# xingyizhou/CenterTrack

Measured on AMD Instinct MI355X. Metric: frames/sec (DLA-34 + DCNv2 CenterTrack hot path: H2D of the frame + forward + decode + D2H + track association), higher is better.
Workload: dtype f32; 1 GPU; mot17_512: mot heads, DLA-34, 512x512, 1 stream(s)/GPU, K=100, flip_test=False, seeded random-init weights; one step = 64 consecutive frames of every stream, each frame uploaded from pinned host memory inside the step (frame t+1 on a copy stream while frame t runs); global_batch=1, parallelism=streams sharded dp1, all-gather of packed detections, hip_graph=True

## Files before the change

### centertrack_amd/_lib.py

```python
import ctypes
import os

_PKG = os.path.dirname(os.path.abspath(__file__))
LIB_PATH = os.environ.get('CENTERTRACK_LIB') or os.path.join(_PKG, 'libcentertrack_hip.so')

c_float_p = ctypes.c_void_p
NUM_HEADS = 11
(HEAD_REG, HEAD_WH, HEAD_TRACKING, HEAD_LTRB, HEAD_LTRB_AMODAL, HEAD_DEP, HEAD_ROT, HEAD_DIM,
 HEAD_AMODEL_OFFSET, HEAD_NUSCENES_ATT, HEAD_VELOCITY) = range(NUM_HEADS)
HEAD_INDEX = {'reg': HEAD_REG, 'wh': HEAD_WH, 'tracking': HEAD_TRACKING, 'ltrb': HEAD_LTRB,
              'ltrb_amodal': HEAD_LTRB_AMODAL, 'dep': HEAD_DEP, 'rot': HEAD_ROT, 'dim': HEAD_DIM,
              'amodel_offset': HEAD_AMODEL_OFFSET, 'nuscenes_att': HEAD_NUSCENES_ATT,
              'velocity': HEAD_VELOCITY}
HEAD_CH = {'reg': 2, 'wh': 2, 'tracking': 2, 'ltrb': 4, 'ltrb_amodal': 4, 'dep': 1, 'rot': 8, 'dim': 3,
           'amodel_offset': 2, 'nuscenes_att': 8, 'velocity': 3}

CT_RELU = 1
CT_OUT_NCHW = 2
CT_DCN_MAIN, CT_DCN_FINISH, CT_DCN_OFFSETS = 1, 2, 4
CT_OK, CT_ERR_ARG, CT_ERR_LAUNCH, CT_ERR_WORKSPACE = 0, 1, 2, 3


class ConvDesc(ctypes.Structure):
    _fields_ = [('x', ctypes.c_void_p), ('N', ctypes.c_int), ('H', ctypes.c_int), ('W', ctypes.c_int),
                ('Cin', ctypes.c_int), ('ldx', ctypes.c_int),
                ('w_packed', ctypes.c_void_p), ('Cout', ctypes.c_int), ('ks', ctypes.c_int),
                ('stride', ctypes.c_int),
                ('scale', ctypes.c_void_p), ('shift', ctypes.c_void_p),
                ('res', ctypes.c_void_p), ('ldr', ctypes.c_int),
                ('y', ctypes.c_void_p), ('ldy', ctypes.c_int),
                ('flags', ctypes.c_int),
                ('sig_lo', ctypes.c_int), ('sig_hi', ctypes.c_int),
                ('dep_lo', ctypes.c_int), ('dep_hi', ctypes.c_int), ('depth_scale', ctypes.c_float),
                ('workspace', ctypes.c_void_p), ('workspace_bytes', ctypes.c_size_t),
                ('split_k', ctypes.c_int), ('algo', ctypes.c_int), ('w_winograd', ctypes.c_void_p),
                ('pool_y', ctypes.c_void_p), ('pool_ld', ctypes.c_int),
                ('proj_w_packed', ctypes.c_void_p), ('proj_scale', ctypes.c_void_p), ('proj_shift', ctypes.c_void_p),
                ('proj_y', ctypes.c_void_p), ('proj_ldy', ctypes.c_int)]


class DcnDesc(ctypes.Structure):
    _fields_ = [('x', ctypes.c_void_p), ('N', ctypes.c_int), ('H', ctypes.c_int), ('W', ctypes.c_int),
                ('Cin', ctypes.c_int), ('ldx', ctypes.c_int),
                ('om', ctypes.c_void_p), ('ldom', ctypes.c_int),
                ('w_packed', ctypes.c_void_p), ('Cout', ctypes.c_int),
                ('scale', ctypes.c_void_p), ('shift', ctypes.c_void_p),
                ('y', ctypes.c_void_p), ('ldy', ctypes.c_int),
                ('flags', ctypes.c_int),
                ('workspace', ctypes.c_void_p), ('workspace_bytes', ctypes.c_size_t),
                ('split_k', ctypes.c_int), ('algo', ctypes.c_int), ('fuse_offset', ctypes.c_int),
                ('w_off_packed', ctypes.c_void_p), ('b_off', ctypes.c_void_p),
                ('up_w', ctypes.c_void_p), ('up_f', ctypes.c_int), ('up_skip', ctypes.c_void_p), ('up_lds', ctypes.c_int),
                ('up_y', ctypes.c_void_p), ('up_ldy', ctypes.c_int),
                ('om_partial', ctypes.c_void_p), ('om_partial_bytes', ctypes.c_size_t),
                ('w_off_winograd', ctypes.c_void_p)]


CT_DCN_BWD_INPUT, CT_DCN_BWD_OFFSET_MASK, CT_DCN_BWD_WEIGHT = 1, 2, 4


class DcnBwdDesc(ctypes.Structure):
    _fields_ = [('x', ctypes.c_void_p), ('N', ctypes.c_int), ('H', ctypes.c_int), ('W', ctypes.c_int),
                ('Cin', ctypes.c_int), ('ldx', ctypes.c_int),
                ('om', ctypes.c_void_p), ('ldom', ctypes.c_int),
                ('gy', ctypes.c_void_p), ('Cout', ctypes.c_int), ('ldgy', ctypes.c_int),
                ('wT_packed', ctypes.c_void_p),
                ('gx', ctypes.c_void_p), ('ldgx', ctypes.c_int),
                ('gom', ctypes.c_void_p), ('ldgom', ctypes.c_int),
                ('gw', ctypes.c_void_p), ('gb', ctypes.c_void_p),
                ('workspace', ctypes.c_void_p), ('workspace_bytes', ctypes.c_size_t),
                ('flags', ctypes.c_int)]


CT_MAX_FUSED_HEADS = 8


class HeadsDesc(ctypes.Structure):
    _fields_ = [('x', ctypes.c_void_p), ('N', ctypes.c_int), ('H', ctypes.c_int), ('W', ctypes.c_int),
                ('Cin', ctypes.c_int), ('ldx', ctypes.c_int),
                ('w0_winograd', ctypes.c_void_p), ('b0', ctypes.c_void_p), ('nheads', ctypes.c_int),
                ('w2', ctypes.c_void_p), ('b2', ctypes.c_void_p),
                ('cout', ctypes.c_int * CT_MAX_FUSED_HEADS), ('coff', ctypes.c_int * CT_MAX_FUSED_HEADS),
                ('out', ctypes.c_void_p), ('ctot', ctypes.c_int),
                ('sig_lo', ctypes.c_int), ('sig_hi', ctypes.c_int), ('dep_lo', ctypes.c_int), ('dep_hi', ctypes.c_int),
                ('depth_scale', ctypes.c_float)]


class SparseHeadsDesc(ctypes.Structure):
    _fields_ = [('feat', ctypes.c_void_p), ('ldf', ctypes.c_int), ('nheads', ctypes.c_int),
                ('head', ctypes.c_int * NUM_HEADS),
                ('w1', ctypes.c_void_p * NUM_HEADS), ('b1', ctypes.c_void_p * NUM_HEADS),
                ('w2', ctypes.c_void_p * NUM_HEADS), ('b2', ctypes.c_void_p * NUM_HEADS),
                ('depth_scale', ctypes.c_float), ('zero_tracking', ctypes.c_int),
                ('flip_B', ctypes.c_int), ('flip_mode', ctypes.c_int * NUM_HEADS)]


class DecodeDesc(ctypes.Structure):
    _fields_ = [('hm', ctypes.c_void_p), ('B', ctypes.c_int), ('C', ctypes.c_int), ('h', ctypes.c_int),
                ('w', ctypes.c_int), ('K', ctypes.c_int),
                ('heads', ctypes.c_void_p * NUM_HEADS),
                ('out', ctypes.c_void_p), ('inds', ctypes.c_void_p),
                ('workspace', ctypes.c_void_p), ('workspace_bytes', ctypes.c_size_t),
                ('hm_batch_stride', ctypes.c_size_t), ('head_batch_stride', ctypes.c_size_t * NUM_HEADS),
                ('out_stride', ctypes.c_int),
                ('host_out', ctypes.c_void_p), ('done_flag', ctypes.c_void_p), ('done_counter', ctypes.c_void_p),
                ('sparse', ctypes.POINTER(SparseHeadsDesc))]


class PoseDesc(ctypes.Structure):
    _fields_ = [('rows', ctypes.c_void_p), ('row_floats', ctypes.c_int), ('box_col', ctypes.c_int),
                ('inds', ctypes.c_void_p),
                ('B', ctypes.c_int), ('h', ctypes.c_int), ('w', ctypes.c_int), ('K', ctypes.c_int),
                ('num_joints', ctypes.c_int),
                ('hps', ctypes.c_void_p), ('hm_hp', ctypes.c_void_p), ('hp_offset', ctypes.c_void_p),
                ('hps_batch_stride', ctypes.c_size_t), ('hm_hp_batch_stride', ctypes.c_size_t),
                ('hp_offset_batch_stride', ctypes.c_size_t),
                ('out', ctypes.c_void_p), ('out_stride', ctypes.c_int),
                ('workspace', ctypes.c_void_p), ('workspace_bytes', ctypes.c_size_t),
                ('box_wh', ctypes.c_void_p), ('box_reg', ctypes.c_void_p), ('box_ltrb', ctypes.c_void_p),
                ('box_wh_batch_stride', ctypes.c_size_t), ('box_reg_batch_stride', ctypes.c_size_t),
                ('box_ltrb_batch_stride', ctypes.c_size_t)]


class FlipHead(ctypes.Structure):
    _fields_ = [('src', ctypes.c_void_p), ('dst', ctypes.c_void_p), ('src_batch_stride', ctypes.c_size_t),
                ('C', ctypes.c_int), ('mode', ctypes.c_int)]


CT_FLIP_AVG, CT_FLIP_NEG_EVEN, CT_FLIP_JOINTS, CT_FLIP_JOINT_OFFSETS = range(4)


class RowLayout(ctypes.Structure):
    _fields_ = [(n, ctypes.c_int) for n in ('score', 'cls', 'cts', 'tracking', 'bbox', 'amodel_offset')]


class Track(ctypes.Structure):
    _fields_ = [('score', ctypes.c_float), ('cls', ctypes.c_int), ('ct', ctypes.c_float * 2),
                ('tracking', ctypes.c_float * 2), ('bbox', ctypes.c_float * 4),
                ('tracking_id', ctypes.c_int), ('age', ctypes.c_int), ('active', ctypes.c_int),
                ('row', ctypes.c_int)]


class PrestageDesc(ctypes.Structure):
    _fields_ = [('enabled', ctypes.c_int), ('N', ctypes.c_int), ('H', ctypes.c_int), ('W', ctypes.c_int),
                ('w_x', ctypes.c_void_p), ('w_img', ctypes.c_void_p), ('scale3', ctypes.c_void_p), ('shift3', ctypes.c_void_p),
                ('partial', ctypes.c_void_p * 3), ('ldp', ctypes.c_int), ('flip_B', ctypes.c_int)]


class FrameLoopDesc(ctypes.Structure):
    _fields_ = [('B', ctypes.c_int), ('K', ctypes.c_int), ('F', ctypes.c_int),
                ('trackers', ctypes.POINTER(ctypes.c_void_p)),
                ('layout', RowLayout),
                ('out_thresh', ctypes.c_float), ('pre_thresh', ctypes.c_float),
                ('inp_w', ctypes.c_int), ('inp_h', ctypes.c_int),
                ('host_rows', ctypes.c_void_p), ('rows_keep', ctypes.c_void_p),
                ('blob_params', ctypes.c_void_p), ('blob_counts', ctypes.c_void_p), ('blob_cap', ctypes.c_int),
                ('nslots', ctypes.c_int),
                ('graphs', ctypes.c_void_p * 3), ('frames', ctypes.c_void_p * 3),
                ('frame_bytes', ctypes.c_size_t),
                ('stream', ctypes.c_void_p),
                ('results', ctypes.c_void_p), ('results_cap', ctypes.c_int), ('done_flag', ctypes.c_void_p),
                ('pre', PrestageDesc)]


class FrameStepArgs(ctypes.Structure):
    _fields_ = [('slot', ctypes.c_int), ('frame_kind', ctypes.c_int),
                ('frame', ctypes.c_void_p), ('next_frame', ctypes.c_void_p),
                ('trans_input', ctypes.c_void_p), ('trans_inv', ctypes.c_void_p)]


CT_FRAME_DEVICE, CT_FRAME_HOST, CT_FRAME_IN_PLACE, CT_FRAME_UPLOADED = range(4)


ABI_VERSION = 103

EXPORTS = ['ct_last_error', 'ct_version', 'ct_set_tuning', 'ct_packed_weight_elems', 'ct_pack_conv_weight',
           'ct_packed_winograd_elems', 'ct_pack_winograd_weight', 'ct_conv2d',
           'ct_conv2d_workspace_bytes', 'ct_heads_fused', 'ct_dcn_v2', 'ct_dcn_v2_workspace_bytes', 'ct_dcn_v2_offsets_bytes', 'ct_dcn_v2_group', 'ct_dcn_v2_group_workspace_bytes', 'ct_dcn_v2_group_plan',
           'ct_dcn_v2_backward', 'ct_dcn_v2_backward_workspace_bytes', 'ct_packed_dcn_weight_t_elems', 'ct_pack_dcn_weight_t', 'ct_stem_forward',
           'ct_maxpool2x2', 'ct_upsample_add', 'ct_nchw_to_nhwc', 'ct_nhwc_to_nchw',
           'ct_decode_row_floats', 'ct_decode_workspace_bytes', 'ct_decode', 'ct_decode_pose_workspace_bytes',
           'ct_decode_pose', 'ct_render_pre_hm',
           'ct_tracker_create', 'ct_tracker_destroy', 'ct_tracker_reset', 'ct_tracker_num_tracks',
           'ct_tracker_id_count', 'ct_tracker_get_tracks', 'ct_tracker_step', 'ct_tracker_prehm_params', 'ct_linear_assignment', 'ct_tracker_set_mode', 'ct_tracker_init_tracks',
           'ct_tracker_step_public', 'ct_tracker_step_dets', 'ct_transform_points',
           'ct_preprocess_image', 'ct_preprocess_lut', 'ct_preprocess_device', 'ct_graph_begin', 'ct_graph_end', 'ct_graph_launch', 'ct_graph_destroy',
           'ct_memcpy_async', 'ct_memset_async', 'ct_stream_synchronize', 'ct_flip_merge', 'ct_flip_images',
           'ct_frame_loop_create', 'ct_frame_loop_destroy', 'ct_frame_loop_submit', 'ct_frame_loop_wait', 'ct_frame_loop_finish',
           'ct_frame_loop_finish_submit', 'ct_frame_loop_upload', 'ct_frame_loop_pending_slot', 'ct_frame_loop_in_flight',
           'ct_frame_loop_forget_upload', 'ct_frame_loop_prestage', 'ct_stem_forward_parts', 'ct_signal_host']

_lib = None


class CTError(RuntimeError):
    pass


def load():
    global _lib
    if _lib is not None:
        return _lib
    if not os.path.exists(LIB_PATH):
        raise CTError('%s not found: build it with `python -c "import __graft_entry__ as g; g.build()"` '
                      '(hipcc --offload-arch=gfx950); there is no CPU fallback' % LIB_PATH)
    import torch
    lib = ctypes.CDLL(LIB_PATH)
    i, p, sz = ctypes.c_int, ctypes.c_void_p, ctypes.c_size_t
    lib.ct_last_error.restype = ctypes.c_char_p
    lib.ct_version.restype = i
    if lib.ct_version() != ABI_VERSION:
        raise CTError('%s is ABI version %d, this binding was written against %d: rebuild it (python -m '
                      'centertrack_amd.build)' % (LIB_PATH, lib.ct_version(), ABI_VERSION))
    lib.ct_set_tuning.argtypes = [ctypes.c_char_p, i]
    lib.ct_packed_weight_elems.restype = sz
    lib.ct_packed_weight_elems.argtypes = [i, i, i]
    lib.ct_pack_conv_weight.argtypes = [p, p, i, i, i, p]
    lib.ct_packed_winograd_elems.restype = sz
    lib.ct_packed_winograd_elems.argtypes = [i, i]
    lib.ct_pack_winograd_weight.argtypes = [p, p, i, i, p]
    lib.ct_conv2d.argtypes = [ctypes.POINTER(ConvDesc), p]
    lib.ct_conv2d_workspace_bytes.restype = sz
    lib.ct_conv2d_workspace_bytes.argtypes = [ctypes.POINTER(ConvDesc)]
    lib.ct_heads_fused.argtypes = [ctypes.POINTER(HeadsDesc), p]
    lib.ct_dcn_v2.argtypes = [ctypes.POINTER(DcnDesc), p]
    lib.ct_dcn_v2_workspace_bytes.restype = sz
    lib.ct_dcn_v2_workspace_bytes.argtypes = [ctypes.POINTER(DcnDesc)]
    lib.ct_dcn_v2_offsets_bytes.restype = sz
    lib.ct_dcn_v2_offsets_bytes.argtypes = [ctypes.POINTER(DcnDesc)]
    lib.ct_dcn_v2_group.argtypes = [ctypes.POINTER(DcnDesc), i, i, p]
    lib.ct_dcn_v2_group_workspace_bytes.restype = sz
    lib.ct_dcn_v2_group_workspace_bytes.argtypes = [ctypes.POINTER(DcnDesc)]
    lib.ct_dcn_v2_group_plan.argtypes = [ctypes.POINTER(DcnDesc), ctypes.POINTER(ctypes.c_size_t), ctypes.POINTER(ctypes.c_int)]
    lib.ct_dcn_v2_backward.argtypes = [ctypes.POINTER(DcnBwdDesc), p]
    lib.ct_dcn_v2_backward_workspace_bytes.restype = sz
    lib.ct_dcn_v2_backward_workspace_bytes.argtypes = [ctypes.POINTER(DcnBwdDesc)]
    lib.ct_packed_dcn_weight_t_elems.restype = sz
    lib.ct_packed_dcn_weight_t_elems.argtypes = [i, i]
    lib.ct_pack_dcn_weight_t.argtypes = [p, p, i, i, p]
    lib.ct_stem_forward.argtypes = [p, p, p, i, i, i, p, p, p, p, p, p, i, p]
    lib.ct_stem_forward_parts.argtypes = [p, p, p, p, i, i, i, i, p, p, p, p, p, p, i, p]
    lib.ct_maxpool2x2.argtypes = [p, i, i, i, i, i, p, i, p]
    lib.ct_upsample_add.argtypes = [p, i, i, i, i, i, p, i, p, i, p, i, p]
    lib.ct_nchw_to_nhwc.argtypes = [p, i, i, i, i, p, i, p]
    lib.ct_nhwc_to_nchw.argtypes = [p, i, i, i, i, i, p, p]
    lib.ct_decode_row_floats.argtypes = [ctypes.POINTER(DecodeDesc)]
    lib.ct_decode_workspace_bytes.restype = sz
    lib.ct_decode_workspace_bytes.argtypes = [ctypes.POINTER(DecodeDesc)]
    lib.ct_decode.argtypes = [ctypes.POINTER(DecodeDesc), p]
    lib.ct_decode_pose_workspace_bytes.restype = sz
    lib.ct_decode_pose_workspace_bytes.argtypes = [ctypes.POINTER(PoseDesc)]
    lib.ct_decode_pose.argtypes = [ctypes.POINTER(PoseDesc), p]
    lib.ct_render_pre_hm.argtypes = [p, p, i, i, i, i, p, i, p]
    lib.ct_tracker_create.restype = p
    lib.ct_tracker_create.argtypes = [ctypes.c_float, i]
    lib.ct_tracker_destroy.restype = None
    lib.ct_tracker_destroy.argtypes = [p]
    lib.ct_tracker_reset.restype = None
    lib.ct_tracker_reset.argtypes = [p]
    lib.ct_tracker_num_tracks.argtypes = [p]
    lib.ct_tracker_id_count.argtypes = [p]
    lib.ct_tracker_get_tracks.argtypes = [p, p, i]
    lib.ct_tracker_step.argtypes = [p, p, i, i, ctypes.POINTER(RowLayout), ctypes.c_float, p, p, i]
    lib.ct_tracker_prehm_params.argtypes = [p, ctypes.c_float, p, i, i, p, i]
    lib.ct_linear_assignment.argtypes = [p, i, i, p, p]
    lib.ct_tracker_set_mode.argtypes = [p, i, i]
    lib.ct_tracker_init_tracks.argtypes = [p, p, i]
    lib.ct_tracker_step_public.argtypes = [p, p, i, i, ctypes.POINTER(RowLayout), ctypes.c_float, p, p, i, p, i]
    lib.ct_tracker_step_dets.argtypes = [p, p, i, p, i, p, i]
    lib.ct_transform_points.argtypes = [p, p, i, p]
    lib.ct_preprocess_image.argtypes = [p, i, i, i, i, p, i, i, p, p, p, i]
    lib.ct_preprocess_lut.argtypes = [p, p, i, p]
    lib.ct_preprocess_device.argtypes = [p, i, i, i, i, p, i, i, p, p, p, p]
    lib.ct_graph_begin.argtypes = [p]
    lib.ct_graph_end.restype = p
    lib.ct_graph_end.argtypes = [p]
    lib.ct_graph_launch.argtypes = [p, p]
    lib.ct_graph_destroy.restype = None
    lib.ct_graph_destroy.argtypes = [p]
    lib.ct_memcpy_async.argtypes = [p, p, sz, i, p]
    lib.ct_stream_synchronize.argtypes = [p]
    lib.ct_memset_async.argtypes = [p, i, sz, p]
    lib.ct_signal_host.argtypes = [p, i, p]
    lib.ct_flip_merge.argtypes = [ctypes.POINTER(FlipHead), i, p, i, i, i, i, p]
    lib.ct_flip_images.argtypes = [p, p, sz, i, p]
    lib.ct_frame_loop_create.restype = p
    lib.ct_frame_loop_create.argtypes = [ctypes.POINTER(FrameLoopDesc)]
    lib.ct_frame_loop_destroy.restype = None
    lib.ct_frame_loop_destroy.argtypes = [p]
    lib.ct_frame_loop_submit.argtypes = [p, ctypes.POINTER(FrameStepArgs)]
    lib.ct_frame_loop_wait.argtypes = [p]
    lib.ct_frame_loop_finish.argtypes = [p, ctypes.POINTER(FrameStepArgs), p]
    lib.ct_frame_loop_finish_submit.argtypes = [p, ctypes.POINTER(FrameStepArgs), p, ctypes.POINTER(FrameStepArgs)]
    lib.ct_frame_loop_upload.argtypes = [p, i, p]
    lib.ct_frame_loop_pending_slot.argtypes = [p]
    lib.ct_frame_loop_prestage.argtypes = [p, i]
    lib.ct_frame_loop_in_flight.argtypes = [p]
    lib.ct_frame_loop_forget_upload.restype = None
    lib.ct_frame_loop_forget_upload.argtypes = [p]
    for kv in filter(None, os.environ.get('CENTERTRACK_TUNE', '').split(',')):
        k, _, v = kv.partition('=')
        if lib.ct_set_tuning(k.strip().encode(), int(v)) != 0:
            raise CTError('CENTERTRACK_TUNE: %s' % lib.ct_last_error().decode())
    _lib = lib
    return lib


def check(rc, what=''):
    if rc != 0:
        raise CTError('%s failed (code %d): %s' % (what or 'libcentertrack_hip call', rc,
                                                  load().ct_last_error().decode()))


def stream_ptr():
    import torch
    return ctypes.c_void_p(torch.cuda.current_stream().cuda_stream)


import contextlib as _contextlib


@_contextlib.contextmanager
def capture_guard(collect=True):
    import gc
    if os.environ.get('CT_NO_CAPTURE_GUARD') == '1':
        yield
        return
    if collect:
        gc.collect()
    was = gc.isenabled()
    gc.disable()
    try:
        yield
    finally:
        if was:
            gc.enable()
```

### centertrack_amd/build.py

```python
import os
import subprocess
import sys

PKG = os.path.dirname(os.path.abspath(__file__))
ROOT = os.path.dirname(PKG)
CSRC = os.path.join(PKG, 'csrc')
LIB = os.path.join(PKG, 'libcentertrack_hip.so')
SOURCES = ['api.cpp', 'runtime.hip', 'conv_mfma.hip', 'wino_mfma.hip', 'dcn_mfma.hip', 'dcn_bwd.hip', 'stem.hip', 'elementwise.hip', 'decode.hip', 'pose.hip', 'host_track.cpp', 'host_preprocess.cpp', 'preprocess.hip', 'flip.hip', 'frame_loop.hip']
FLAGS = ['--offload-arch=gfx950', '-O3', '-std=c++17', '-fPIC', '-I' + os.path.join(ROOT, 'include'), '-I' + CSRC,
         '-Wno-unused-result']


def _stale(target, deps):
    if not os.path.exists(target):
        return True
    t = os.path.getmtime(target)
    return any(os.path.getmtime(d) > t for d in deps)


def build(force=False, verbose=False):
    hipcc = os.environ.get('HIPCC', '/opt/rocm/bin/hipcc')
    objdir = os.path.join(PKG, 'build')
    os.makedirs(objdir, exist_ok=True)
    headers = [os.path.join(CSRC, 'ct_common.h'), os.path.join(CSRC, 'ksplit_core.h'),
               os.path.join(ROOT, 'include', 'centertrack_hip.h')]
    objs = []
    procs = []
    for src in SOURCES:
        sp = os.path.join(CSRC, src)
        if not os.path.exists(sp):
            continue
        obj = os.path.join(objdir, src.rsplit('.', 1)[0] + '.o')
        objs.append(obj)
        if force or _stale(obj, [sp] + headers):
            extra = ['-x', 'hip'] if src.endswith('.hip') else ['-ffp-contract=off']
            cmd = [hipcc] + FLAGS + extra + ['-c', sp, '-o', obj]
            if verbose:
                print(' '.join(cmd))
            procs.append((src, subprocess.Popen(cmd)))
    for src, p in procs:
        if p.wait() != 0:
            raise RuntimeError('hipcc failed on %s' % src)
    if force or _stale(LIB, objs):
        cmd = [hipcc, '--offload-arch=gfx950', '-shared', '-fPIC', '-pthread', '-o', LIB] + objs
        if verbose:
            print(' '.join(cmd))
        subprocess.check_call(cmd)
    return LIB


if __name__ == '__main__':
    print(build(force='--force' in sys.argv, verbose=True))
```

### centertrack_amd/csrc/decode.hip

```cpp
#include "ct_common.h"

namespace {
CT_DEFINE_STAMPS(decode)

constexpr int SEG_MAX = 1024;
constexpr int MAXK = 512;

__device__ __forceinline__ unsigned f2ord(float f)
{
    const unsigned u = __float_as_uint(f);
    return (u & 0x80000000u) ? ~u : (u | 0x80000000u);
}
__device__ __forceinline__ float ord2f(unsigned o)
{
    return __uint_as_float((o & 0x80000000u) ? (o & 0x7fffffffu) : ~o);
}

__device__ __forceinline__ void hist_add(unsigned *hist, unsigned digit, bool active)
{
    unsigned long long todo = __ballot(active);
    const int lane = threadIdx.x & 63;
#pragma unroll 1
    for (int it = 0; it < 4 && todo; ++it) {
        const int leader = __ffsll((long long)todo) - 1;
        const unsigned d0 = __shfl(digit, leader);
        const unsigned long long same = __ballot(active && digit == d0) & todo;
        if (lane == leader) atomicAdd(&hist[d0], (unsigned)__popcll(same));
        todo &= ~same;
    }
    if (active && ((todo >> lane) & 1ull)) atomicAdd(&hist[digit], 1u);
}

template <typename Get>
__device__ unsigned long long radix_select_kth(Get get, int n, int K, unsigned *hist ,
                                               unsigned long long *bcast )
{
    __shared__ int scan_tmp[256];
    __shared__ int wsum[4];
    unsigned long long prefix = 0ull;
    int need = K;
    for (int d = 7; d >= 0; --d) {
        for (int i = threadIdx.x; i < 256; i += blockDim.x) hist[i] = 0u;
        __syncthreads();
        const int sh = d * 8;
        const unsigned long long himask = (d == 7) ? 0ull : (~0ull << (sh + 8));
        const int nround = (n + blockDim.x - 1) / blockDim.x * blockDim.x;
        for (int i = threadIdx.x; i < nround; i += blockDim.x) {
            const unsigned long long k = (i < n) ? get(i) : 0ull;
            hist_add(hist, (unsigned)(k >> sh) & 255u, k != 0ull && (k & himask) == prefix);
        }
        __syncthreads();
        if (threadIdx.x < 256) {
            const int b = threadIdx.x, ln = b & 63;
            const int c = (int)hist[b];
            int suf = c;
#pragma unroll
            for (int o = 1; o < 64; o <<= 1) {
                const int t = __shfl_down(suf, o);
                if (ln + o < 64) suf += t;
            }
            if (ln == 0) wsum[b >> 6] = suf;
            scan_tmp[b] = suf;
        }
        __syncthreads();
        if (threadIdx.x < 256) {
            const int b = threadIdx.x;
            int hi = 0;
            for (int wv = (b >> 6) + 1; wv < 4; ++wv) hi += wsum[wv];
            const int incl = scan_tmp[b] + hi;
            const int above = incl - (int)hist[b];
            if (above < need && incl >= need) {
                bcast[0] = (unsigned long long)b;
                bcast[1] = (incl - above == need - above) ? ~0ull : (unsigned long long)(need - above);
            }
        }
        __syncthreads();
        prefix |= bcast[0] << sh;
        const unsigned long long nd = bcast[1];
        __syncthreads();
        if (nd == ~0ull) break;
        need = (int)nd;
    }
    return prefix;
}

struct Stage1Args {
    const float *hm;
    unsigned long long *cand;
    int B, C, h, w, K, nseg, seg;
    size_t hm_bs;
};

__global__ __launch_bounds__(256) void decode_stage1_kernel(Stage1Args a)
{
    extern __shared__ __attribute__((aligned(16))) unsigned char smem[];
    unsigned long long *keys = reinterpret_cast<unsigned long long *>(smem);
    float *rows = reinterpret_cast<float *>(smem + SEG_MAX * sizeof(unsigned long long));
    __shared__ int npos;

    int bid = blockIdx.x;
    const int seg = bid % a.nseg; bid /= a.nseg;
    const int c = bid % a.C;
    const int b = bid / a.C;
    const int HW = a.h * a.w;
    const int p_lo = seg * a.seg;
    const int p_hi = min(HW, p_lo + a.seg);
    const int nloc = p_hi - p_lo;
    const float *map = a.hm + (size_t)b * a.hm_bs + (size_t)c * HW;

    const int y_lo = p_lo / a.w, y_hi = (p_hi - 1) / a.w;
    const int r_lo = max(0, y_lo - 1), r_hi = min(a.h - 1, y_hi + 1);
    const int nstage = (r_hi - r_lo + 1) * a.w;
    for (int i = threadIdx.x; i < nstage; i += 256) rows[i] = map[r_lo * a.w + i];
    if (threadIdx.x == 0) npos = 0;
    __syncthreads();

    const int lane = threadIdx.x & 63;
    const int nround = (nloc + 255) / 256 * 256;
    for (int i = threadIdx.x; i < nround; i += 256) {
        bool pos = false;
        unsigned long long key = 0ull;
        if (i < nloc) {
            const int p = p_lo + i;
            const int y = p / a.w, x = p - y * a.w;
            const float v = rows[(y - r_lo) * a.w + x];
            float m = v;
#pragma unroll
            for (int dy = -1; dy <= 1; ++dy) {
                const int yy = y + dy;
                if (yy < 0 || yy >= a.h) continue;
#pragma unroll
                for (int dx = -1; dx <= 1; ++dx) {
                    const int xx = x + dx;
                    if (xx < 0 || xx >= a.w) continue;
                    m = fmaxf(m, rows[(yy - r_lo) * a.w + xx]);
                }
            }
            const float s = (m == v) ? v : v * 0.0f;
            pos = s > 0.0f;
            key = ((unsigned long long)f2ord(s) << 32) | (unsigned long long)(0xFFFFFFFFu - (unsigned)p);
        }
        const unsigned long long mask = __ballot(pos);
        int base = 0;
        if (lane == 0 && mask) base = atomicAdd(&npos, (int)__popcll(mask));
        base = __shfl(base, 0);
        if (pos) keys[base + (int)__popcll(mask & ((1ull << lane) - 1ull))] = key;
    }
    __syncthreads();

    const int n = npos;
    unsigned long long *out = a.cand + (size_t)blockIdx.x * a.K;
    if (n <= a.K) {
        for (int i = threadIdx.x; i < a.K; i += 256) out[i] = (i < n) ? keys[i] : 0ull;
    } else {
        for (int i = threadIdx.x; i < n; i += 256) {
            const unsigned long long k = keys[i];
            int r = 0;
            for (int j = 0; j < n; ++j) r += (keys[j] > k) ? 1 : 0;
            if (r < a.K) out[r] = k;
        }
    }
}

struct Stage2Args {
    const unsigned long long *cand;
    const float *hm;
    const float *heads[CT_NUM_HEADS];
    int head_ch[CT_NUM_HEADS];
    size_t head_bs[CT_NUM_HEADS];
    size_t hm_bs;
    float *out;
    long long *inds;
    int B, C, h, w, K, nseg, F;
    int M2;
    int keys_final;
    float *host_out;
    int *done_flag;
    unsigned *done_counter;
    unsigned long long *winners;
    unsigned present;
};

template <typename HV>
__device__ __forceinline__ void emit_row(float *row, float *hrow, unsigned present, float score, int cls, float xs0,
                                         float ys0, HV hv)
{
    constexpr int HCH[CT_NUM_HEADS] = {2, 2, 2, 4, 4, 1, 8, 3, 2, 8, 3};
    auto has = [&](int hd) { return (present >> hd) & 1u; };
    int f = 0;
    auto put = [&](float v) { row[f] = v; if (hrow) hrow[f] = v; ++f; };
    put(score); put((float)cls); put(xs0); put(ys0);
    float xs = xs0 + 0.5f, ys = ys0 + 0.5f;
    if (has(CT_HEAD_REG)) { xs = xs0 + hv(CT_HEAD_REG, 0); ys = ys0 + hv(CT_HEAD_REG, 1); }
    const bool has_box = has(CT_HEAD_WH) || has(CT_HEAD_LTRB) || has(CT_HEAD_LTRB_AMODAL);
    float bb[4] = {0.f, 0.f, 0.f, 0.f};
    if (has(CT_HEAD_WH)) {
        float ww = hv(CT_HEAD_WH, 0), hh = hv(CT_HEAD_WH, 1);
        if (ww < 0.f) ww = 0.f;
        if (hh < 0.f) hh = 0.f;
        bb[0] = xs - ww / 2; bb[1] = ys - hh / 2; bb[2] = xs + ww / 2; bb[3] = ys + hh / 2;
    }
    if (has(CT_HEAD_LTRB)) {
        bb[0] = xs0 + hv(CT_HEAD_LTRB, 0); bb[1] = ys0 + hv(CT_HEAD_LTRB, 1);
        bb[2] = xs0 + hv(CT_HEAD_LTRB, 2); bb[3] = ys0 + hv(CT_HEAD_LTRB, 3);
    }
    float am[4] = {0.f, 0.f, 0.f, 0.f};
    if (has(CT_HEAD_LTRB_AMODAL)) {
        am[0] = xs0 + hv(CT_HEAD_LTRB_AMODAL, 0); am[1] = ys0 + hv(CT_HEAD_LTRB_AMODAL, 1);
        am[2] = xs0 + hv(CT_HEAD_LTRB_AMODAL, 2); am[3] = ys0 + hv(CT_HEAD_LTRB_AMODAL, 3);
        for (int i = 0; i < 4; ++i) bb[i] = am[i];
    }
    if (has_box) for (int i = 0; i < 4; ++i) put(bb[i]);
    if (has(CT_HEAD_LTRB_AMODAL)) for (int i = 0; i < 4; ++i) put(am[i]);
    const int rest[7] = {CT_HEAD_TRACKING, CT_HEAD_DEP, CT_HEAD_ROT, CT_HEAD_DIM, CT_HEAD_AMODEL_OFFSET,
                         CT_HEAD_NUSCENES_ATT, CT_HEAD_VELOCITY};
#pragma unroll
    for (int q = 0; q < 7; ++q) {
        const int hd = rest[q];
        if (!has(hd)) continue;
#pragma unroll
        for (int ch = 0; ch < HCH[hd]; ++ch) put(hv(hd, ch));
    }
}

__device__ __forceinline__ void raise_done_flag(int *done_flag, unsigned *done_counter, int nwg)
{
    __threadfence_system();
    __syncthreads();
    if (threadIdx.x == 0 && nwg == 1) {
        __hip_atomic_store(done_flag, 1, __ATOMIC_RELEASE, __HIP_MEMORY_SCOPE_SYSTEM);
    } else if (threadIdx.x == 0) {
        const unsigned prev = __hip_atomic_fetch_add(done_counter, 1u, __ATOMIC_ACQ_REL, __HIP_MEMORY_SCOPE_SYSTEM);
        if (prev == (unsigned)nwg - 1u) {
            *done_counter = 0u;
            __hip_atomic_store(done_flag, 1, __ATOMIC_RELEASE, __HIP_MEMORY_SCOPE_SYSTEM);
        }
    }
}

__device__ __forceinline__ unsigned long long key_from_map(const float *hm_b, int C, int h, int w, unsigned f)
{
    const int HW = h * w;
    const int cls = (int)(f / (unsigned)HW);
    const int p = (int)(f - (unsigned)cls * (unsigned)HW);
    const int y = p / w, x = p - y * w;
    const float *map = hm_b + (size_t)cls * HW;
    const float v = map[p];
    float m = v;
    for (int dy = -1; dy <= 1; ++dy) {
        const int yy = y + dy;
        if (yy < 0 || yy >= h) continue;
        for (int dx = -1; dx <= 1; ++dx) {
            const int xx = x + dx;
            if (xx < 0 || xx >= w) continue;
            m = fmaxf(m, map[yy * w + xx]);
        }
    }
    const float s = (m == v) ? v : v * 0.0f;
    return ((unsigned long long)f2ord(s) << 32) | (unsigned long long)(0xFFFFFFFFu - f);
}

template <typename F>
__device__ __forceinline__ void scan_cands(const unsigned long long *cand, int M2, int tid, int NT, F f)
{
    constexpr int U = 8;
    for (int i0 = tid; i0 - tid < M2; i0 += NT * U) {
        unsigned long long raw[U];
#pragma unroll
        for (int u = 0; u < U; ++u) {
            const int i = i0 + u * NT;
            raw[u] = (i < M2) ? cand[i] : 0ull;
        }
#pragma unroll
        for (int u = 0; u < U; ++u) f(i0 + u * NT, raw[u]);
    }
}

constexpr int FCAP = 4096;
constexpr int SLICE = 8192;

__device__ __forceinline__ void bitonic_desc(unsigned long long *v, int n, int tid, int NT)
{
    for (int size = 2; size <= n; size <<= 1) {
        for (int stride = size >> 1; stride > 0; stride >>= 1) {
            for (int i = tid; i < (n >> 1); i += NT) {
                const int lo = 2 * i - (i & (stride - 1));
                const int hi = lo + stride;
                const bool desc = ((lo & size) == 0);
                const unsigned long long x = v[lo], y = v[hi];
                if ((x < y) == desc) { v[lo] = y; v[hi] = x; }
            }
            __syncthreads();
        }
    }
}


constexpr int SEL_U = 8;
constexpr int SEL_BINS = 1024;
constexpr int TIECAP = 1024;

struct SelShared {
    unsigned hist[SEL_BINS];
    int wsum[16];
    unsigned long long tie[TIECAP];
    int bstar, need, total, nwin, ntie;
};

__device__ __forceinline__ int sel_bin(unsigned long long k)
{
    const float sc = ord2f((unsigned)(k >> 32));
    const int b = (int)(sc * (float)SEL_BINS);
    return b < 0 ? 0 : (b > SEL_BINS - 1 ? SEL_BINS - 1 : b);
}

__device__ __forceinline__ int select_topk_regs(const unsigned long long (&keys)[SEL_U], int K, SelShared &sh,
                                                unsigned long long *win, bool keep_all)
{
    const int tid = threadIdx.x, lane = tid & 63, wave = tid >> 6;
    sh.hist[tid] = 0u;
    if (tid == 0) { sh.bstar = -1; sh.need = 0; sh.total = 0; sh.nwin = 0; sh.ntie = 0; }
    __syncthreads();
    int bins[SEL_U];
#pragma unroll
    for (int u = 0; u < SEL_U; ++u) {
        bins[u] = sel_bin(keys[u]);
        if (keys[u] != 0ull) atomicAdd(&sh.hist[bins[u]], 1u);
    }
    __syncthreads();
    const int c = (int)sh.hist[tid];
    int suf = c;
#pragma unroll
    for (int o = 1; o < 64; o <<= 1) {
        const int t = __shfl_down(suf, o);
        if (lane + o < 64) suf += t;
    }
    if (lane == 0) sh.wsum[wave] = suf;
    __syncthreads();
    int hi = 0;
    for (int w = wave + 1; w < 16; ++w) hi += sh.wsum[w];
    const int incl = suf + hi, above = incl - c;
    if (tid == 0) sh.total = incl;
    if (above < K && incl >= K) { sh.bstar = tid; sh.need = K - above; }
    __syncthreads();
    const int total = sh.total;
    if (total < K) {
        if (keep_all) {
#pragma unroll
            for (int u = 0; u < SEL_U; ++u) {
                const bool hit = keys[u] != 0ull;
                const unsigned long long mask = __ballot(hit);
                int base = 0;
                if (mask) {
                    const int leader = __ffsll((long long)mask) - 1;
                    if (lane == leader) base = atomicAdd(&sh.nwin, (int)__popcll(mask));
                    base = __shfl(base, leader);
                }
                if (hit) win[base + (int)__popcll(mask & ((1ull << lane) - 1ull))] = keys[u];
            }
            __syncthreads();
        }
        return -1;
    }
    const int bstar = sh.bstar, need = sh.need;
    unsigned hitm = 0u, tiem = 0u;
#pragma unroll
    for (int u = 0; u < SEL_U; ++u) {
        const bool live = keys[u] != 0ull;
        hitm |= (live && bins[u] > bstar) ? (1u << u) : 0u;
        tiem |= (live && bins[u] == bstar) ? (1u << u) : 0u;
    }
    const int packed = __popc(hitm) | (__popc(tiem) << 16);
    int pre = packed;
#pragma unroll
    for (int o = 1; o < 64; o <<= 1) {
        const int t = __shfl_up(pre, o);
        if (lane >= o) pre += t;
    }
    const int tot = __shfl(pre, 63);
    int bh = 0, bt = 0;
    if (lane == 63) {
        if (tot & 0xffff) bh = atomicAdd(&sh.nwin, tot & 0xffff);
        if (tot >> 16) bt = atomicAdd(&sh.ntie, tot >> 16);
    }
    int sw = __shfl(bh, 63) + ((pre - packed) & 0xffff);
    int st = __shfl(bt, 63) + ((pre - packed) >> 16);
#pragma unroll
    for (int u = 0; u < SEL_U; ++u) {
        if ((hitm >> u) & 1u) win[sw++] = keys[u];
        if ((tiem >> u) & 1u) {
            if (st < TIECAP) sh.tie[st] = keys[u];
            ++st;
        }
    }
    __syncthreads();
    const int m = sh.ntie;
    if (m > TIECAP) return -2;
    const int first = K - need;
    for (int i = tid; i < m; i += 1024) {
        const unsigned long long k = sh.tie[i];
        int r = 0;
        for (int j = 0; j < m; ++j) r += (sh.tie[j] > k) ? 1 : 0;
        if (r < need) win[first + r] = k;
    }
    __syncthreads();
    return K;
}

struct Stage2aArgs {
    const unsigned long long *cand;
    unsigned long long *cand2;
    int M2, G, K, per_class, HW;
};

__global__ __launch_bounds__(1024) void decode_stage2a_kernel(Stage2aArgs a)
{
    __shared__ SelShared sh;
    __shared__ unsigned long long win[MAXK];
    __shared__ unsigned rhist[256];
    __shared__ unsigned long long rbcast[2];
    __shared__ int rslot;
    const int b = blockIdx.x / a.G, g = blockIdx.x - b * a.G;
    const int tid = threadIdx.x, NT = blockDim.x;
    const int lo = g * SLICE, n = min(SLICE, a.M2 - lo);
    const unsigned long long *cand = a.cand + (size_t)b * a.M2 + lo;
    unsigned long long keys[SEL_U];
#pragma unroll
    for (int u = 0; u < SEL_U; ++u) {
        const int i = tid + u * NT;
        unsigned long long k = (i < n) ? cand[i] : 0ull;
        if (k != 0ull) {
            const unsigned cls = (unsigned)((lo + i) / a.per_class);
            const unsigned p = 0xFFFFFFFFu - (unsigned)(k & 0xFFFFFFFFull);
            k = (k & 0xFFFFFFFF00000000ull) | (unsigned long long)(0xFFFFFFFFu - (cls * (unsigned)a.HW + p));
        }
        keys[u] = k;
    }
    for (int i = tid; i < a.K; i += NT) win[i] = 0ull;
    __syncthreads();
    unsigned long long *out = a.cand2 + ((size_t)b * a.G + g) * a.K;
    const int rc = select_topk_regs(keys, a.K, sh, win, true);
    if (rc != -2) {
        for (int i = tid; i < a.K; i += NT) out[i] = win[i];
        return;
    }
    auto get = [&](int i) -> unsigned long long {
        unsigned long long k = cand[i];
        if (k != 0ull) {
            const unsigned cls = (unsigned)((lo + i) / a.per_class);
            const unsigned p = 0xFFFFFFFFu - (unsigned)(k & 0xFFFFFFFFull);
            k = (k & 0xFFFFFFFF00000000ull) | (unsigned long long)(0xFFFFFFFFu - (cls * (unsigned)a.HW + p));
        }
        return k;
    };
    if (tid == 0) rslot = 0;
    __syncthreads();
    const unsigned long long T = radix_select_kth(get, n, a.K, rhist, rbcast);
#pragma unroll
    for (int u = 0; u < SEL_U; ++u)
        if (keys[u] >= T && keys[u] != 0ull) {
            const int sl = atomicAdd(&rslot, 1);
            if (sl < a.K) out[sl] = keys[u];
        }
}

__global__ __launch_bounds__(1024) void decode_stage2_kernel(Stage2Args a)
{
    __shared__ unsigned hist[256];
    __shared__ unsigned long long bcast[2];
    __shared__ unsigned long long win[MAXK];
    __shared__ unsigned long long lmax[1024];
    __shared__ unsigned long long filt[FCAP];
    __shared__ SelShared sel;
    __shared__ unsigned long long Lsh;
    __shared__ int slot, total, nf;
    const int b = blockIdx.x;
    const int tid = threadIdx.x, NT = blockDim.x, lane = tid & 63;
    const int HW = a.h * a.w;
    const int M2 = a.M2;
    CT_STAMP_RT(0);
    CT_STAMP(1);
    const unsigned long long *cand = a.cand + (size_t)b * M2;
    const int per_class = a.nseg * a.K;

    auto key2 = [&](int i, unsigned long long k) -> unsigned long long {
        if (k == 0ull || a.keys_final) return k;
        const unsigned cls = (unsigned)(i / per_class);
        const unsigned p = 0xFFFFFFFFu - (unsigned)(k & 0xFFFFFFFFull);
        return (k & 0xFFFFFFFF00000000ull) | (unsigned long long)(0xFFFFFFFFu - (cls * (unsigned)HW + p));
    };
    auto get = [&](int i) -> unsigned long long { return key2(i, cand[i]); };
    const bool in_regs = M2 <= SEL_U * 1024 && NT == 1024;
    unsigned long long keys[SEL_U];
    if (in_regs) {
#pragma unroll
        for (int u = 0; u < SEL_U; ++u) {
            const int i = tid + u * NT;
            keys[u] = (i < M2) ? cand[i] : 0ull;
        }
    }
    int KP = 1;
    while (KP < a.K) KP <<= 1;
    for (int i = tid; i < KP; i += NT) win[i] = 0ull;
    if (tid == 0) { slot = 0; total = 0; nf = 0; Lsh = 1ull; }
    __syncthreads();
    bool need_sort = true;
    bool selected = false;
    if (in_regs) {
#pragma unroll
        for (int u = 0; u < SEL_U; ++u) keys[u] = key2(tid + u * NT, keys[u]);
        CT_STAMP(2);
        const int rc = select_topk_regs(keys, a.K, sel, filt, false);
        CT_STAMP(3);
        if (rc == a.K) {
            for (int i0 = 0; i0 < a.K; i0 += NT / 8) {
                const int i = i0 + (tid >> 3), part = tid & 7;
                const unsigned long long k = (i < a.K) ? filt[i] : 0ull;
                int r = 0;
                for (int j = part; j < a.K; j += 8) r += (filt[j] > k) ? 1 : 0;
                r += __shfl_xor(r, 1);
                r += __shfl_xor(r, 2);
                r += __shfl_xor(r, 4);
                if (i < a.K && part == 0) win[r] = k;
            }
            need_sort = false;
            selected = true;
        } else if (rc == -1) {
            if (tid == 0) total = sel.total;
            selected = true;
        }
        __syncthreads();
    }
    if (!selected) {
    scan_cands(cand, M2, tid, NT, [&](int i, unsigned long long raw) {
        const unsigned long long k = key2(i, raw);
        const bool hit = k != 0ull;
        const unsigned long long mask = __ballot(hit);
        int base = 0;
        if (mask) {
            const int leader = __ffsll((long long)mask) - 1;
            if (lane == leader) base = atomicAdd(&total, (int)__popcll(mask));
            base = __shfl(base, leader);
        }
        if (hit) {
            const int sl = base + (int)__popcll(mask & ((1ull << lane) - 1ull));
            if (sl < FCAP) filt[sl] = k;
        }
    });
    __syncthreads();
    }
    if (selected && need_sort == false) {
    } else if (!selected && total >= a.K && total <= FCAP) {
        int NP = KP;
        while (NP < total) NP <<= 1;
        for (int i = total + tid; i < NP; i += NT) filt[i] = 0ull;
        __syncthreads();
        bitonic_desc(filt, NP, tid, NT);
        for (int i = tid; i < a.K; i += NT) win[i] = filt[i];
        need_sort = false;
    } else if (!selected && total >= a.K) {
        {
            unsigned long long mx = 0ull;
            scan_cands(cand, M2, tid, NT, [&](int i, unsigned long long raw) {
                const unsigned long long k = key2(i, raw);
                mx = (k > mx) ? k : mx;
            });
            lmax[tid] = mx;
        }
        __syncthreads();
        if (tid < 256) {
            const int G = NT < 256 ? NT : 256;
            const unsigned long long my = lmax[tid];
            int r = 0;
            for (int j = 0; j < G; ++j) r += (lmax[j] > my) ? 1 : 0;
            if (my != 0ull && r == a.K - 1) Lsh = my;
        }
        __syncthreads();
        const unsigned long long L = Lsh;
        scan_cands(cand, M2, tid, NT, [&](int i, unsigned long long raw) {
            const unsigned long long k = key2(i, raw);
            const bool hit = k >= L && k != 0ull;
            const unsigned long long mask = __ballot(hit);
            int base = 0;
            if (mask) {
                const int leader = __ffsll((long long)mask) - 1;
                if (lane == leader) base = atomicAdd(&nf, (int)__popcll(mask));
                base = __shfl(base, leader);
            }
            if (hit) {
                const int sl = base + (int)__popcll(mask & ((1ull << lane) - 1ull));
                if (sl < FCAP) filt[sl] = k;
            }
        });
        __syncthreads();
        const int n = nf;
        if (n <= FCAP) {
            for (int i = tid; i < n; i += NT) {
                const unsigned long long k = filt[i];
                int r = 0;
                for (int j = 0; j < n; ++j) r += (filt[j] > k) ? 1 : 0;
                if (r < a.K) win[r] = k;
            }
            need_sort = false;
        } else {
            const unsigned long long T = radix_select_kth(get, M2, a.K, hist, bcast);
            for (int i = tid; i < M2; i += NT) {
                const unsigned long long k = get(i);
                if (k >= T && k != 0ull) {
                    const int s = atomicAdd(&slot, 1);
                    if (s < a.K) win[s] = k;
                }
            }
        }
    } else {
        const float *hm_b = a.hm + (size_t)b * a.hm_bs;
        const int NALL = a.C * HW;
        auto getall = [&](int i) -> unsigned long long { return key_from_map(hm_b, a.C, a.h, a.w, (unsigned)i); };
        const unsigned long long T = radix_select_kth(getall, NALL, a.K, hist, bcast);
        for (int i = tid; i < NALL; i += NT) {
            const unsigned long long k = getall(i);
            if (k >= T) {
                const int s = atomicAdd(&slot, 1);
                if (s < a.K) win[s] = k;
            }
        }
    }
    __syncthreads();
    CT_STAMP(4);
    if (need_sort) bitonic_desc(win, KP, tid, NT);
    if (a.winners) {
        for (int r = threadIdx.x; r < a.K; r += blockDim.x) {
            const unsigned long long k = win[r];
            a.winners[(size_t)b * a.K + r] = k;
            if (a.inds) a.inds[(size_t)b * a.K + r] = (int)((0xFFFFFFFFu - (unsigned)(k & 0xFFFFFFFFull)) % (unsigned)HW);
        }
        CT_STAMP(5);
        CT_STAMP(6);
        CT_STAMP(7);
        CT_STAMP_RT(8);
        return;
    }
    for (int r = threadIdx.x; r < a.K; r += blockDim.x) {
        const unsigned long long k = win[r];
        const float score = ord2f((unsigned)(k >> 32));
        const unsigned flat = 0xFFFFFFFFu - (unsigned)(k & 0xFFFFFFFFull);
        const int cls = (int)(flat / (unsigned)HW);
        const int p = (int)(flat - (unsigned)cls * (unsigned)HW);
        const float ys0 = (float)(p / a.w), xs0 = (float)(p % a.w);
        float *row = a.out + ((size_t)b * a.K + r) * a.F;
        float *hrow = a.host_out ? a.host_out + ((size_t)b * a.K + r) * a.F : nullptr;
        if (a.inds) a.inds[(size_t)b * a.K + r] = p;
        constexpr int HCH[CT_NUM_HEADS] = {2, 2, 2, 4, 4, 1, 8, 3, 2, 8, 3};
        float hval[CT_NUM_HEADS][8];
#pragma unroll
        for (int hd = 0; hd < CT_NUM_HEADS; ++hd) {
            const float *hp = a.heads[hd];
            const bool on = hp != nullptr;
            const float *base = on ? hp + (size_t)b * a.head_bs[hd] + p : a.hm;
#pragma unroll
            for (int ch = 0; ch < HCH[hd]; ++ch) hval[hd][ch] = base[on ? (size_t)ch * HW : 0];
        }
        emit_row(row, hrow, a.present, score, cls, xs0, ys0, [&](int hd, int ch) { return hval[hd][ch]; });
    }
    CT_STAMP(5);
    if (a.done_flag) {
        raise_done_flag(a.done_flag, a.done_counter, a.B);
        CT_STAMP(6);
    }
    CT_STAMP(7);
    CT_STAMP_RT(8);
}

constexpr int SP_HID = 256;

struct SparseArgs {
    const float *feat; int ldf; size_t feat_bs;
    int nheads;
    int head[CT_NUM_HEADS];
    const float *w1[CT_NUM_HEADS], *b1[CT_NUM_HEADS], *w2[CT_NUM_HEADS], *b2[CT_NUM_HEADS];
    float depth_scale;
    int zero_tracking;
    int flip_B;
    int flip_mode[CT_NUM_HEADS];
    const unsigned long long *winners;
    float *partial;
    float *out, *host_out;
    int *done_flag; unsigned *done_counter;
    int B, h, w, K, F, tiles;
    unsigned present;
};

__global__ __launch_bounds__(256) __attribute__((amdgpu_waves_per_eu(2, 2))) void sparse_heads_kernel(SparseArgs a)
{
    __shared__ __attribute__((aligned(16))) float A[36 * 256];
    __shared__ __attribute__((aligned(16))) float Hd[16 * 68];
    __shared__ int wy[16], wx[16];
    constexpr int HCH[CT_NUM_HEADS] = {2, 2, 2, 4, 4, 1, 8, 3, 2, 8, 3};
    const int tid = threadIdx.x, lane = tid & 63;
    const int wave = __builtin_amdgcn_readfirstlane(tid >> 6);
    int bid = blockIdx.x;
    const int quarter = bid & 3; bid >>= 2;
    const int hi = bid % a.nheads; bid /= a.nheads;
    const int tile = bid;
    const int b = tile / a.tiles, t = tile - b * a.tiles;
    const int HW = a.h * a.w;
    const int hd = a.head[hi];
    const int cout = HCH[hd];
    const float *wp = a.w1[hi] + ((size_t)(quarter * 4 + wave) << 8) + (lane << 2);
    f32x4 bq[36];
#pragma unroll
    for (int st = 0; st < 36; ++st) bq[st] = *reinterpret_cast<const f32x4 *>(wp + (size_t)st * (16 << 8));
    const int li = lane & 15, lg = lane >> 4;
    const float bias1 = a.b1[hi][quarter * 64 + wave * 16 + li];
    if (tid < 16) {
        const int r = t * 16 + tid;
        int y = -4, x = -4;
        if (r < a.K) {
            const unsigned long long k = a.winners[(size_t)b * a.K + r];
            const unsigned flat = 0xFFFFFFFFu - (unsigned)(k & 0xFFFFFFFFull);
            const int p = (int)(flat % (unsigned)HW);
            y = p / a.w; x = p - y * a.w;
        }
        wy[tid] = y; wx[tid] = x;
    }
    __syncthreads();
    const int npass = (a.flip_B > 0 && a.flip_mode[hi] != 0) ? 2 : 1;
    for (int pass = 0; pass < npass; ++pass) {
    {
        const float *fb = a.feat + (size_t)(pass ? a.flip_B + b : b) * a.feat_bs;
        f32x4 pv[9];
#pragma unroll
        for (int j = 0; j < 9; ++j) {
            const int it = tid + 256 * j;
            const int m = it / 144, rem = it - m * 144;
            const int tap = rem >> 4, q = rem & 15;
            const int cx = pass ? a.w - 1 - wx[m] : wx[m];
            const int y = wy[m] + tap / 3 - 1, x = cx + tap % 3 - 1;
            const bool ok = y >= 0 && y < a.h && x >= 0 && x < a.w && wy[m] >= 0;
            const f32x4 v = *reinterpret_cast<const f32x4 *>(fb + (ok ? ((size_t)y * a.w + x) * a.ldf + q * 4 : 0));
            pv[j] = ok ? v : f32x4{0.f, 0.f, 0.f, 0.f};
        }
        if (pass) __syncthreads();
#pragma unroll
        for (int j = 0; j < 9; ++j) {
            const int it = tid + 256 * j;
            const int m = it / 144, rem = it - m * 144;
            const int tap = rem >> 4, q = rem & 15;
            *reinterpret_cast<f32x4 *>(A + (tap * 4 + (q >> 2)) * 256 + m * 16 + (((q & 3) ^ ((m >> 1) & 2)) << 2)) = pv[j];
        }
    }
    __syncthreads();
    {
        const int aoff = li * 16 + ((lg ^ ((li >> 1) & 2)) << 2);
        f32x4 acc = f32x4{0.f, 0.f, 0.f, 0.f};
#pragma unroll
        for (int st = 0; st < 36; ++st) {
            const f32x4 af = *reinterpret_cast<const f32x4 *>(A + st * 256 + aoff);
#pragma unroll
            for (int e = 0; e < 4; ++e) acc = __builtin_amdgcn_mfma_f32_16x16x4f32(af[e], bq[st][e], acc, 0, 0, 0);
        }
#pragma unroll
        for (int e = 0; e < 4; ++e) Hd[(lg * 4 + e) * 68 + wave * 16 + li] = fmaxf(acc[e] + bias1, 0.0f);
    }
    __syncthreads();
    {
        const int pair = tid >> 1, part = tid & 1;
        const int m = pair >> 3, c = pair & 7;
        float sum = 0.f;
        if (c < cout) {
            const float *w2 = a.w2[hi] + c * SP_HID + quarter * 64 + part * 32;
            const float *hh = Hd + m * 68 + part * 32;
#pragma unroll
            for (int j = 0; j < 32; ++j) sum += hh[j] * w2[j];
        }
        sum += __shfl_xor(sum, 1);
        if (part == 0) a.partial[(((((size_t)tile * a.nheads + hi) * 2 + pass) * 4 + quarter) * 16 + m) * 8 + c] = sum;
    }
    }
}

__global__ __launch_bounds__(128) void sparse_rows_kernel(SparseArgs a)
{
    constexpr int HCH[CT_NUM_HEADS] = {2, 2, 2, 4, 4, 1, 8, 3, 2, 8, 3};
    const int b = blockIdx.x;
    const int HW = a.h * a.w;
    for (int r = threadIdx.x; r < a.K; r += blockDim.x) {
        const unsigned long long k = a.winners[(size_t)b * a.K + r];
        const unsigned flat = 0xFFFFFFFFu - (unsigned)(k & 0xFFFFFFFFull);
        const int cls = (int)(flat / (unsigned)HW);
        const int p = (int)(flat - (unsigned)cls * (unsigned)HW);
        const int y = p / a.w, x = p - y * a.w;
        const float score = ord2f((unsigned)(k >> 32));
        const int tile = b * a.tiles + (r >> 4), m = r & 15;
        float V[CT_NUM_HEADS][8];
#pragma unroll
        for (int hd = 0; hd < CT_NUM_HEADS; ++hd)
#pragma unroll
            for (int c = 0; c < 8; ++c) V[hd][c] = 0.f;
        for (int h2 = 0; h2 < a.nheads; ++h2) {
            const int hd2 = a.head[h2];
            const bool both = a.flip_B > 0 && a.flip_mode[h2] != 0;
#pragma unroll
            for (int c = 0; c < 8; ++c) {
                if (c >= HCH[hd2]) continue;
                auto value = [&](int pass) {
                    const float *pp = a.partial + ((((size_t)tile * a.nheads + h2) * 2 + pass) * 4 * 16 + m) * 8 + c;
                    float v = pp[0];
                    v += pp[128];
                    v += pp[256];
                    v += pp[384];
                    v += a.b2[h2][c];
                    if (hd2 == CT_HEAD_DEP) v = (1.0f / (1.0f / (1.0f + expf(-v)) + 1e-6f) - 1.0f) * a.depth_scale;
                    return v;
                };
                float v = value(0);
                if (both) {
                    const float v1 = value(1);
                    v = (v + ((a.flip_mode[h2] == 2 && !(c & 1)) ? -v1 : v1)) / 2;
                }
                if (hd2 == CT_HEAD_TRACKING && a.zero_tracking) v = 0.0f;
#pragma unroll
                for (int hd = 0; hd < CT_NUM_HEADS; ++hd)
                    if (hd == hd2) V[hd][c] = v;
            }
        }
        float *row = a.out + ((size_t)b * a.K + r) * a.F;
        float *hrow = a.host_out ? a.host_out + ((size_t)b * a.K + r) * a.F : nullptr;
        emit_row(row, hrow, a.present, score, cls, (float)x, (float)y, [&](int hd3, int ch) { return V[hd3][ch]; });
    }
    if (a.done_flag) raise_done_flag(a.done_flag, a.done_counter, a.B);
}

const int kHeadCh[CT_NUM_HEADS] = {2, 2, 2, 4, 4, 1, 8, 3, 2, 8, 3};

int check(const ct_decode_desc *d, const char *who)
{
    if (!d || !d->hm) CT_FAIL_ARG("%s: null heat-map", who);
    if (d->B <= 0 || d->C <= 0 || d->h <= 0 || d->w <= 0) CT_FAIL_ARG("%s: bad shape", who);
    if (d->K <= 0 || d->K > MAXK) CT_FAIL_ARG("%s: K=%d out of range (1..%d)", who, d->K, MAXK);
    if ((long)d->h * d->w < d->K) CT_FAIL_ARG("%s: h*w=%ld < K=%d (torch.topk would raise too)", who, (long)d->h * d->w, d->K);
    if ((double)d->C * d->h * d->w >= 4294967295.0) CT_FAIL_ARG("%s: C*h*w too large", who);
    if (const ct_sparse_heads_desc *sp = d->sparse) {
        if (sp->nheads < 1 || sp->nheads > CT_NUM_HEADS || !sp->feat || sp->ldf < 64 || (sp->ldf & 3) || ((uintptr_t)sp->feat & 15))
            CT_FAIL_ARG("%s: sparse heads need 1..%d heads and a 16-byte aligned NHWC feature view of >= 64 channels", who, CT_NUM_HEADS);
        for (int i = 0; i < sp->nheads; ++i) {
            if (sp->head[i] < 0 || sp->head[i] >= CT_NUM_HEADS || !sp->w1[i] || !sp->b1[i] || !sp->w2[i] || !sp->b2[i])
                CT_FAIL_ARG("%s: sparse head %d is incomplete", who, i);
            if (d->heads[sp->head[i]]) CT_FAIL_ARG("%s: head %d is both dense and sparse", who, sp->head[i]);
        }
        if (sp->flip_B < 0 || (sp->flip_B > 0 && sp->flip_B != d->B)) CT_FAIL_ARG("%s: sparse flip_B must be 0 or B (feat then holds 2 * B images)", who);
    }
    return CT_OK;
}

}

static unsigned present_mask(const ct_decode_desc *d)
{
    unsigned m = 0;
    for (int i = 0; i < CT_NUM_HEADS; ++i)
        if (d->heads[i]) m |= 1u << i;
    if (d->sparse)
        for (int i = 0; i < d->sparse->nheads && i < CT_NUM_HEADS; ++i)
            if (d->sparse->head[i] >= 0 && d->sparse->head[i] < CT_NUM_HEADS) m |= 1u << d->sparse->head[i];
    return m;
}

extern "C" int ct_decode_row_floats(const ct_decode_desc *d)
{
    if (!d) return 0;
    if (d->sparse && (d->sparse->nheads < 1 || d->sparse->nheads > CT_NUM_HEADS)) {
        ct_set_error("ct_decode_row_floats: sparse nheads=%d out of range (1..%d)", d->sparse->nheads, CT_NUM_HEADS);
        return 0;
    }
    const unsigned m = present_mask(d);
    auto has = [&](int hd) { return (m >> hd) & 1u; };
    int f = 4;
    if (has(CT_HEAD_WH) || has(CT_HEAD_LTRB) || has(CT_HEAD_LTRB_AMODAL)) f += 4;
    if (has(CT_HEAD_LTRB_AMODAL)) f += 4;
    const int rest[7] = {CT_HEAD_TRACKING, CT_HEAD_DEP, CT_HEAD_ROT, CT_HEAD_DIM, CT_HEAD_AMODEL_OFFSET,
                         CT_HEAD_NUSCENES_ATT, CT_HEAD_VELOCITY};
    for (int q = 0; q < 7; ++q)
        if (has(rest[q])) f += kHeadCh[rest[q]];
    return f;
}

static int pick_seg(const ct_decode_desc *d)
{
    const long HW = (long)d->h * d->w;
    int seg = SEG_MAX;
    while (seg > 256 && (long)d->B * d->C * ((HW + seg - 1) / seg) < 256) seg >>= 1;
    return seg;
}

static int pick_groups(const ct_decode_desc *d, int seg, int nseg)
{
    const long M2 = (long)d->C * nseg * d->K;
    (void)seg;
    if (M2 <= SLICE) return 0;
    const long G = (M2 + SLICE - 1) / SLICE;
    return (int)G;
}

static size_t sparse_bytes(const ct_decode_desc *d)
{
    if (!d->sparse) return 0;
    const size_t tiles = (size_t)d->B * ct_cdiv(d->K, 16);
    return (size_t)d->B * d->K * 8 + tiles * (size_t)d->sparse->nheads * 2 * 4 * 16 * 8 * sizeof(float);
}

extern "C" size_t ct_decode_workspace_bytes(const ct_decode_desc *d)
{
    if (check(d, "ct_decode_workspace_bytes") != CT_OK) return 0;
    const int seg = pick_seg(d);
    const int nseg = ct_cdiv(d->h * d->w, seg);
    const long M2 = (long)d->C * nseg * d->K;
    return ((size_t)d->B * M2 + (size_t)d->B * pick_groups(d, seg, nseg) * d->K) * sizeof(unsigned long long) + sparse_bytes(d);
}

extern "C" int ct_decode(const ct_decode_desc *d, void *stream)
{
    int rc = check(d, "ct_decode");
    if (rc != CT_OK) return rc;
    if (!d->out) CT_FAIL_ARG("ct_decode: null output");
    if (d->done_flag && (!d->done_counter || !d->host_out)) CT_FAIL_ARG("ct_decode: done_flag needs host_out and done_counter");
    const int seg = pick_seg(d);
    const int nseg = ct_cdiv(d->h * d->w, seg);
    const long M2 = (long)d->C * nseg * d->K;
    const int G = pick_groups(d, seg, nseg);
    const size_t need = ((size_t)d->B * M2 + (size_t)d->B * G * d->K) * sizeof(unsigned long long) + sparse_bytes(d);
    const ct_sparse_heads_desc *sp = d->sparse;
    if (!d->workspace || d->workspace_bytes < need) {
        ct_set_error("ct_decode: needs %zu workspace bytes, got %zu", need, d->workspace_bytes);
        return CT_ERR_WORKSPACE;
    }
    if (d->w > 4096) CT_FAIL_ARG("ct_decode: w=%d > 4096 unsupported", d->w);
    hipStream_t s = (hipStream_t)stream;
    Stage1Args a1;
    a1.hm = d->hm; a1.cand = (unsigned long long *)d->workspace;
    a1.B = d->B; a1.C = d->C; a1.h = d->h; a1.w = d->w; a1.K = d->K; a1.nseg = nseg; a1.seg = seg;
    const size_t HWs = (size_t)d->h * d->w;
    a1.hm_bs = d->hm_batch_stride ? (size_t)d->hm_batch_stride : (size_t)d->C * HWs;
    const int max_rows = ct_cdiv(seg, d->w) + 3;
    const size_t lds1 = SEG_MAX * sizeof(unsigned long long) + (size_t)max_rows * d->w * sizeof(float);
    static bool attr_set = false;
    if (!attr_set) {
        (void)hipFuncSetAttribute(reinterpret_cast<const void *>(decode_stage1_kernel),
                                  hipFuncAttributeMaxDynamicSharedMemorySize, 96 * 1024);
        attr_set = true;
    }
    if (lds1 > 96 * 1024) CT_FAIL_ARG("ct_decode: stage-1 LDS %zu too large", lds1);
    hipLaunchKernelGGL(decode_stage1_kernel, dim3((unsigned)(d->B * d->C * nseg)), dim3(256), lds1, s, a1);
    CT_CHECK_LAUNCH("ct_decode(stage 1)");
    Stage2Args a2;
    a2.cand = a1.cand; a2.hm = d->hm;
    for (int i = 0; i < CT_NUM_HEADS; ++i) {
        a2.heads[i] = d->heads[i]; a2.head_ch[i] = kHeadCh[i];
        a2.head_bs[i] = d->head_batch_stride[i] ? (size_t)d->head_batch_stride[i] : (size_t)kHeadCh[i] * HWs;
    }
    a2.hm_bs = a1.hm_bs;
    a2.out = d->out; a2.inds = (long long *)d->inds;
    a2.B = d->B; a2.C = d->C; a2.h = d->h; a2.w = d->w; a2.K = d->K; a2.nseg = nseg;
    a2.F = d->out_stride ? d->out_stride : ct_decode_row_floats(d);
    if (a2.F < ct_decode_row_floats(d)) CT_FAIL_ARG("ct_decode: out_stride %d < row floats", d->out_stride);
    a2.M2 = (int)M2; a2.keys_final = 0;
    a2.host_out = d->host_out; a2.done_flag = d->done_flag; a2.done_counter = d->done_counter;
    a2.present = present_mask(d);
    a2.winners = sp ? (unsigned long long *)d->workspace + (size_t)d->B * M2 + (size_t)d->B * G * d->K : nullptr;
    if (G > 0) {
        Stage2aArgs aa;
        aa.cand = a1.cand; aa.cand2 = a1.cand + (size_t)d->B * M2;
        aa.M2 = (int)M2; aa.G = G; aa.K = d->K; aa.per_class = nseg * d->K; aa.HW = d->h * d->w;
        hipLaunchKernelGGL(decode_stage2a_kernel, dim3((unsigned)(d->B * G)), dim3(1024), 0, s, aa);
        CT_CHECK_LAUNCH("ct_decode(stage 2a)");
        a2.cand = aa.cand2; a2.M2 = G * d->K; a2.keys_final = 1;
    }
    hipLaunchKernelGGL(decode_stage2_kernel, dim3((unsigned)d->B), dim3(1024), 0, s, a2);
    CT_CHECK_LAUNCH("ct_decode(stage 2)");
    if (sp) {
        SparseArgs sa;
        sa.feat = sp->feat; sa.ldf = sp->ldf; sa.feat_bs = (size_t)d->h * d->w * sp->ldf;
        sa.nheads = sp->nheads;
        for (int i = 0; i < CT_NUM_HEADS; ++i) {
            const bool on = i < sp->nheads;
            sa.head[i] = on ? sp->head[i] : 0;
            sa.w1[i] = on ? sp->w1[i] : nullptr; sa.b1[i] = on ? sp->b1[i] : nullptr;
            sa.w2[i] = on ? sp->w2[i] : nullptr; sa.b2[i] = on ? sp->b2[i] : nullptr;
        }
        sa.depth_scale = sp->depth_scale; sa.zero_tracking = sp->zero_tracking;
        sa.flip_B = sp->flip_B;
        for (int i = 0; i < CT_NUM_HEADS; ++i) sa.flip_mode[i] = (i < sp->nheads) ? sp->flip_mode[i] : 0;
        sa.partial = (float *)(a2.winners + (size_t)d->B * d->K);
        sa.winners = a2.winners; sa.out = d->out; sa.host_out = d->host_out;
        sa.done_flag = d->done_flag; sa.done_counter = d->done_counter;
        sa.B = d->B; sa.h = d->h; sa.w = d->w; sa.K = d->K; sa.F = a2.F; sa.tiles = ct_cdiv(d->K, 16);
        sa.present = a2.present;
        hipLaunchKernelGGL(sparse_heads_kernel, dim3((unsigned)(d->B * sa.tiles * sp->nheads * 4)), dim3(256), 0, s, sa);
        CT_CHECK_LAUNCH("ct_decode(sparse heads)");
        hipLaunchKernelGGL(sparse_rows_kernel, dim3((unsigned)d->B), dim3(128), 0, s, sa);
        CT_CHECK_LAUNCH("ct_decode(sparse rows)");
    }
    return CT_OK;
}
```

### centertrack_amd/csrc/elementwise.hip

```cpp
#include "ct_common.h"

namespace {

__global__ __launch_bounds__(256) void maxpool2x2_kernel(const float *x, int N, int H, int W, int C, int ldx,
                                                         float *y, int ldy)
{
    const int Ho = H >> 1, Wo = W >> 1, C4 = C >> 2;
    const size_t total = (size_t)N * Ho * Wo * C4;
    for (size_t idx = (size_t)blockIdx.x * 256 + threadIdx.x; idx < total; idx += (size_t)gridDim.x * 256) {
        const int c4 = (int)(idx % C4);
        size_t p = idx / C4;
        const int ox = (int)(p % Wo); p /= Wo;
        const int oy = (int)(p % Ho);
        const int n = (int)(p / Ho);
        const float *src = x + (((size_t)n * H + 2 * oy) * W + 2 * ox) * ldx + c4 * 4;
        const f32x4 a = *reinterpret_cast<const f32x4 *>(src);
        const f32x4 b = *reinterpret_cast<const f32x4 *>(src + ldx);
        const f32x4 c = *reinterpret_cast<const f32x4 *>(src + (size_t)W * ldx);
        const f32x4 d = *reinterpret_cast<const f32x4 *>(src + (size_t)W * ldx + ldx);
        f32x4 m;
#pragma unroll
        for (int i = 0; i < 4; ++i) m[i] = fmaxf(fmaxf(a[i], b[i]), fmaxf(c[i], d[i]));
        *reinterpret_cast<f32x4 *>(y + (((size_t)n * Ho + oy) * Wo + ox) * ldy + c4 * 4) = m;
    }
}

__global__ __launch_bounds__(256) void upsample_add_kernel(const float *x, int N, int H, int W, int C, int ldx,
                                                           const float *w, int f, const float *skip, int lds,
                                                           float *y, int ldy)
{
    const int Ho = H * f, Wo = W * f, C4 = C >> 2, kw = 2 * f, p = f >> 1;
    const size_t total = (size_t)N * Ho * Wo * C4;
    for (size_t idx = (size_t)blockIdx.x * 256 + threadIdx.x; idx < total; idx += (size_t)gridDim.x * 256) {
        const int c = (int)(idx % C4) * 4;
        size_t q = idx / C4;
        const int ox = (int)(q % Wo); q /= Wo;
        const int oy = (int)(q % Ho);
        const int n = (int)(q / Ho);
        const int iy = (oy + p) / f, ky = (oy + p) - iy * f;
        const int ix = (ox + p) / f, kx = (ox + p) - ix * f;
        const size_t opix = ((size_t)n * Ho + oy) * Wo + ox;
        f32x4 acc = *reinterpret_cast<const f32x4 *>(skip + opix * lds + c);
#pragma unroll
        for (int jy = 0; jy < 2; ++jy) {
            const int yy = iy - jy;
            if (yy < 0 || yy >= H) continue;
#pragma unroll
            for (int jx = 0; jx < 2; ++jx) {
                const int xx = ix - jx;
                if (xx < 0 || xx >= W) continue;
                const f32x4 v = *reinterpret_cast<const f32x4 *>(x + (((size_t)n * H + yy) * W + xx) * ldx + c);
                const int widx = (ky + f * jy) * kw + (kx + f * jx);
                const f32x4 wv = *reinterpret_cast<const f32x4 *>(w + (size_t)widx * C + c);
#pragma unroll
                for (int i = 0; i < 4; ++i) acc[i] += v[i] * wv[i];
            }
        }
        *reinterpret_cast<f32x4 *>(y + opix * ldy + c) = acc;
    }
}

__global__ __launch_bounds__(256) void nchw_to_nhwc_kernel(const float *x, int C, int HW, float *y, int ldy)
{
    __shared__ float tile[32][33];
    const int n = blockIdx.z;
    const int c0 = blockIdx.y * 32, p0 = blockIdx.x * 32;
    const int tx = threadIdx.x & 31, ty = threadIdx.x >> 5;
    const float *src = x + (size_t)n * C * HW;
    float *dst = y + (size_t)n * HW * ldy;
    for (int r = ty; r < 32; r += 8) {
        const int c = c0 + r, p = p0 + tx;
        tile[r][tx] = (c < C && p < HW) ? src[(size_t)c * HW + p] : 0.0f;
    }
    __syncthreads();
    for (int r = ty; r < 32; r += 8) {
        const int p = p0 + r, c = c0 + tx;
        if (p < HW && c < C) dst[(size_t)p * ldy + c] = tile[tx][r];
    }
}

__global__ __launch_bounds__(256) void nhwc_to_nchw_kernel(const float *x, int C, int HW, int ldx, float *y)
{
    __shared__ float tile[32][33];
    const int n = blockIdx.z;
    const int c0 = blockIdx.y * 32, p0 = blockIdx.x * 32;
    const int tx = threadIdx.x & 31, ty = threadIdx.x >> 5;
    const float *src = x + (size_t)n * HW * ldx;
    float *dst = y + (size_t)n * C * HW;
    for (int r = ty; r < 32; r += 8) {
        const int p = p0 + r, c = c0 + tx;
        tile[r][tx] = (p < HW && c < C) ? src[(size_t)p * ldx + c] : 0.0f;
    }
    __syncthreads();
    for (int r = ty; r < 32; r += 8) {
        const int c = c0 + r, p = p0 + tx;
        if (c < C && p < HW) dst[(size_t)c * HW + p] = tile[tx][r];
    }
}

constexpr int PHM_TW = 32, PHM_TH = 8, PHM_CAP = 256;
__global__ __launch_bounds__(256) void render_pre_hm_kernel(const int *params, const int *counts, int cap, int B,
                                                            int H, int W, float *out, int also_flipped)
{
    __shared__ int blob[PHM_CAP * 3];
    __shared__ int nblob;
    const int tilesX = (W + PHM_TW - 1) / PHM_TW, tilesY = (H + PHM_TH - 1) / PHM_TH;
    int bid = blockIdx.x;
    const int tx = bid % tilesX; bid /= tilesX;
    const int ty = bid % tilesY;
    const int b = bid / tilesY;
    const int x0 = tx * PHM_TW, y0 = ty * PHM_TH;
    const int n = min(counts[b], cap);
    const int *p = params + (size_t)b * cap * 3;
    const int lane = threadIdx.x & 63;
    const int x = x0 + (threadIdx.x & (PHM_TW - 1)), y = y0 + (threadIdx.x / PHM_TW);
    float v = 0.0f;
    for (int c0 = 0; c0 == 0 || c0 < n; c0 += PHM_CAP) {
        const int c1 = min(n, c0 + PHM_CAP);
        if (threadIdx.x == 0) nblob = 0;
        __syncthreads();
        for (int i0 = c0; i0 < c1; i0 += 256) {
            const int i = i0 + threadIdx.x;
            int cx = 0, cy = 0, r = -1;
            if (i < c1) { cx = p[3 * i]; cy = p[3 * i + 1]; r = p[3 * i + 2]; }
            const bool hit = i < c1 && r >= 0 && cx + r >= x0 && cx - r < x0 + PHM_TW && cy + r >= y0 && cy - r < y0 + PHM_TH;
            const unsigned long long mask = __ballot(hit);
            int base = 0;
            if (mask) {
                const int leader = __ffsll((long long)mask) - 1;
                if (lane == leader) base = atomicAdd(&nblob, (int)__popcll(mask));
                base = __shfl(base, leader);
            }
            if (hit) {
                const int s = base + (int)__popcll(mask & ((1ull << lane) - 1ull));
                blob[3 * s] = cx; blob[3 * s + 1] = cy; blob[3 * s + 2] = r;
            }
        }
        __syncthreads();
        const int m = nblob;
        for (int i = 0; i < m; ++i) {
            const int cx = blob[3 * i], cy = blob[3 * i + 1], r = blob[3 * i + 2];
            const int dx = x - cx, dy = y - cy;
            if (dx < -r || dx > r || dy < -r || dy > r) continue;
            const double sigma = (double)(2 * r + 1) / 6.0;
            const double g = exp(-(double)(dx * dx + dy * dy) / (2.0 * sigma * sigma));
            v = fmaxf(v, (float)g);
        }
        __syncthreads();
    }
    if (x >= W || y >= H) return;
    out[((size_t)b * H + y) * W + x] = v;
    if (also_flipped) out[((size_t)(B + b) * H + y) * W + (W - 1 - x)] = v;
}

unsigned grid_for(size_t total)
{
    size_t b = (total + 255) / 256;
    if (b > 256 * 16) b = 256 * 16;
    if (b < 1) b = 1;
    return (unsigned)b;
}

}

extern "C" int ct_maxpool2x2(const float *x, int N, int H, int W, int C, int ldx, float *y, int ldy, void *stream)
{
    if (!x || !y) CT_FAIL_ARG("ct_maxpool2x2: null pointer");
    if (C % 4 || ldx % 4 || ldy % 4 || ((uintptr_t)x & 15) || ((uintptr_t)y & 15))
        CT_FAIL_ARG("ct_maxpool2x2: C/ld must be multiples of 4 and pointers 16-byte aligned");
    if (H < 2 || W < 2 || N <= 0) CT_FAIL_ARG("ct_maxpool2x2: bad shape");
    const size_t total = (size_t)N * (H / 2) * (W / 2) * (C / 4);
    hipLaunchKernelGGL(maxpool2x2_kernel, dim3(grid_for(total)), dim3(256), 0, (hipStream_t)stream, x, N, H, W, C, ldx,
                       y, ldy);
    CT_CHECK_LAUNCH("ct_maxpool2x2");
    return CT_OK;
}

extern "C" int ct_upsample_add(const float *x, int N, int H, int W, int C, int ldx, const float *w, int f,
                               const float *skip, int lds, float *y, int ldy, void *stream)
{
    if (!x || !w || !skip || !y) CT_FAIL_ARG("ct_upsample_add: null pointer");
    if (f != 2 && f != 4 && f != 8) CT_FAIL_ARG("ct_upsample_add: f=%d unsupported", f);
    if (C % 4 || ldx % 4 || lds % 4 || ldy % 4 || ((uintptr_t)x & 15) || ((uintptr_t)skip & 15) || ((uintptr_t)y & 15))
        CT_FAIL_ARG("ct_upsample_add: C/ld must be multiples of 4 and pointers 16-byte aligned");
    const size_t total = (size_t)N * H * f * W * f * (C / 4);
    hipLaunchKernelGGL(upsample_add_kernel, dim3(grid_for(total)), dim3(256), 0, (hipStream_t)stream, x, N, H, W, C,
                       ldx, w, f, skip, lds, y, ldy);
    CT_CHECK_LAUNCH("ct_upsample_add");
    return CT_OK;
}

extern "C" int ct_nchw_to_nhwc(const float *x, int N, int C, int H, int W, float *y, int ldy, void *stream)
{
    if (!x || !y || ldy < C) CT_FAIL_ARG("ct_nchw_to_nhwc: bad arguments");
    const int HW = H * W;
    hipLaunchKernelGGL(nchw_to_nhwc_kernel, dim3(ct_cdiv(HW, 32), ct_cdiv(C, 32), N), dim3(256), 0,
                       (hipStream_t)stream, x, C, HW, y, ldy);
    CT_CHECK_LAUNCH("ct_nchw_to_nhwc");
    return CT_OK;
}

extern "C" int ct_nhwc_to_nchw(const float *x, int N, int C, int H, int W, int ldx, float *y, void *stream)
{
    if (!x || !y || ldx < C) CT_FAIL_ARG("ct_nhwc_to_nchw: bad arguments");
    const int HW = H * W;
    hipLaunchKernelGGL(nhwc_to_nchw_kernel, dim3(ct_cdiv(HW, 32), ct_cdiv(C, 32), N), dim3(256), 0,
                       (hipStream_t)stream, x, C, HW, ldx, y);
    CT_CHECK_LAUNCH("ct_nhwc_to_nchw");
    return CT_OK;
}

extern "C" int ct_render_pre_hm(const int *params, const int *counts, int cap, int B, int H, int W, float *out,
                                int also_flipped, void *stream)
{
    if (!params || !counts || !out || cap <= 0 || B <= 0 || H <= 0 || W <= 0) CT_FAIL_ARG("ct_render_pre_hm: bad arguments");
    const long blocks = (long)B * ((H + PHM_TH - 1) / PHM_TH) * ((W + PHM_TW - 1) / PHM_TW);
    hipLaunchKernelGGL(render_pre_hm_kernel, dim3((unsigned)blocks), dim3(256), 0, (hipStream_t)stream, params, counts,
                       cap, B, H, W, out, also_flipped);
    CT_CHECK_LAUNCH("ct_render_pre_hm");
    return CT_OK;
}
```

### centertrack_amd/csrc/stem.hip

```cpp
#include "ct_common.h"

namespace {

constexpr int ST_TW = 32;
constexpr int ST_PW = 40;
template <int TH> struct StCfg {
    static constexpr int PH = TH + 6;
    static constexpr int PS = PH * ST_PW;
    static constexpr int NPV = (3 * PH * 38 + 255) / 256;
    static constexpr int HALVES = TH / 8;
};
__host__ __device__ constexpr int st_k4(int s) { return s == 2 ? 52 : 148; }
__host__ __device__ constexpr int st_koff(int s) { return s * 148; }
constexpr int ST_KTOT = 348;
constexpr int ST_WLP = 16;

CT_DEFINE_STAMPS(stem)

struct StemArgs {
    const float *in[3];
    const float *w[3];
    const float *scale;
    const float *shift;
    const float *add;
    float *y;
    int N, H, W, ldy, ldadd, tilesX, tilesY;
};

constexpr int ST_NWV = 10;

template <int TH>
__attribute__((amdgpu_waves_per_eu(TH == 16 ? 2 : 1)))
__global__ __launch_bounds__(256) void stem_kernel(StemArgs a)
{
    using SC = StCfg<TH>;
    constexpr int ST_TH = TH, ST_PH = SC::PH, ST_PS = SC::PS, ST_NPV = SC::NPV, MT = 4, HV = SC::HALVES;
    __shared__ __attribute__((aligned(16))) float planes[7 * ST_PS];
    __shared__ __attribute__((aligned(16))) float wl[ST_KTOT * ST_WLP];
    __shared__ int tab[ST_KTOT];
    CT_STAMP_RT(0);
    CT_STAMP(1);
    CT_STAMP_HW(8);

    const int tid = threadIdx.x;
    const int lane = tid & 63, wave = __builtin_amdgcn_readfirstlane(tid >> 6);
    const int li = lane & 15, lg = lane >> 4;
    int bid = blockIdx.x;
    const int tx = bid % a.tilesX; bid /= a.tilesX;
    const int ty = bid % a.tilesY; bid /= a.tilesY;
    const int n = bid;
    const int oy0 = ty * ST_TH, ox0 = tx * ST_TW;
    const size_t HW = (size_t)a.H * a.W;

    for (int k = tid; k < ST_KTOT; k += 256) {
        const int s = (k >= 296) ? 2 : ((k >= 148) ? 1 : 0);
        const int kk = k - st_koff(s);
        const int cin = (s == 2) ? 1 : 3;
        int off = 0;
        if (kk < cin * 49) {
            const int c = kk / 49, r = kk - c * 49;
            off = (3 * s + c) * ST_PS + (r / 7) * ST_PW + (r % 7);
        }
        tab[k] = off;
    }

    float pv[ST_NPV], wv[ST_NWV];
    auto stage_load = [&](int s) {
        const int cin = (s == 2) ? 1 : 3;
        const int K = cin * 49;
        const float *src = a.in[s] + (size_t)n * cin * HW;
        const float *w = a.w[s];
        const int np = cin * ST_PH * 38, nw = st_k4(s) * 16;
#pragma unroll
        for (int i = 0; i < ST_NPV; ++i) {
            const int it = tid + 256 * i;
            const int c = it / (ST_PH * 38);
            const int r = it - c * (ST_PH * 38);
            const int py = r / 38, px = r - py * 38;
            const int iy = oy0 - 3 + py, ix = ox0 - 3 + px;
            const bool ok = it < np && iy >= 0 && iy < a.H && ix >= 0 && ix < a.W;
            const float v = src[ok ? ((size_t)c * HW + (size_t)iy * a.W + ix) : 0];
            pv[i] = ok ? v : 0.0f;
        }
#pragma unroll
        for (int i = 0; i < ST_NWV; ++i) {
            const int it = tid + 256 * i;
            const int k = it >> 4, j = it & 15;
            const bool ok = it < nw && k < K;
            const float v = w[ok ? (j * K + k) : 0];
            wv[i] = ok ? v : 0.0f;
        }
    };
    auto stage_store = [&](int s) {
        const int cin = (s == 2) ? 1 : 3;
        const int np = cin * ST_PH * 38, nw = st_k4(s) * 16;
#pragma unroll
        for (int i = 0; i < ST_NPV; ++i) {
            const int it = tid + 256 * i;
            if (it < np) {
                const int c = it / (ST_PH * 38);
                const int r = it - c * (ST_PH * 38);
                const int py = r / 38, px = r - py * 38;
                planes[(3 * s + c) * ST_PS + py * ST_PW + px] = pv[i];
            }
        }
#pragma unroll
        for (int i = 0; i < ST_NWV; ++i) {
            const int it = tid + 256 * i;
            if (it < nw) wl[st_koff(s) * 16 + it] = wv[i];
        }
    };

    int pbase[MT];
#pragma unroll
    for (int mt = 0; mt < MT; ++mt) pbase[mt] = (2 * wave + (mt >> 1)) * ST_PW + (mt & 1) * 16 + li;

    f32x4 out[HV][MT];
#pragma unroll
    for (int h = 0; h < HV; ++h)
#pragma unroll
    for (int mt = 0; mt < MT; ++mt) {
        out[h][mt] = f32x4{0.f, 0.f, 0.f, 0.f};
        if (a.add) {
            const int oy = oy0 + 8 * h + 2 * wave + (mt >> 1);
#pragma unroll
            for (int e = 0; e < 4; ++e) {
                const int ox = ox0 + (mt & 1) * 16 + lg * 4 + e;
                if (oy < a.H && ox < a.W) out[h][mt][e] = a.add[(((size_t)n * a.H + oy) * a.W + ox) * a.ldadd + li];
            }
        }
    }

    const int first = a.in[0] ? 0 : (a.in[1] ? 1 : 2);
    stage_load(first);
    CT_STAMP(2);
    stage_store(first);
    __syncthreads();
    CT_STAMP(3);
#pragma unroll
    for (int s = 0; s < 3; ++s) {
        if (s < first) continue;
        const int nxt = (s < 1 && a.in[1]) ? 1 : ((s < 2 && a.in[2]) ? 2 : 3);
        const bool have_next = a.in[s] != nullptr && nxt < 3;
        if (have_next) stage_load(nxt);
        if (a.in[s]) {
            const float sc = a.scale[s * 16 + li], sh = a.shift[s * 16 + li];
#pragma unroll
            for (int h = 0; h < HV; ++h) {
                f32x4 acc[MT];
#pragma unroll
                for (int mt = 0; mt < MT; ++mt) acc[mt] = f32x4{0.f, 0.f, 0.f, 0.f};
                const int nsteps = st_k4(s) / 4;
#pragma unroll 4
                for (int st = 0; st < nsteps; ++st) {
                    const int k = st_koff(s) + 4 * st + lg;
                    const int off = tab[k] + 8 * h * ST_PW;
                    const float b = wl[k * ST_WLP + li];
#pragma unroll
                    for (int mt = 0; mt < MT; ++mt)
                        acc[mt] = __builtin_amdgcn_mfma_f32_16x16x4f32(planes[off + pbase[mt]], b, acc[mt], 0, 0, 0);
                }
#pragma unroll
                for (int mt = 0; mt < MT; ++mt)
#pragma unroll
                    for (int e = 0; e < 4; ++e) out[h][mt][e] += fmaxf(acc[mt][e] * sc + sh, 0.0f);
            }
        }
        if (have_next) stage_store(nxt);
        if (s < 2) __syncthreads();
        if (s == 0) CT_STAMP(4);
        if (s == 1) CT_STAMP(5);
    }
    CT_STAMP(9);

#pragma unroll
    for (int h = 0; h < HV; ++h)
#pragma unroll
    for (int mt = 0; mt < MT; ++mt) {
        const int oy = oy0 + 8 * h + 2 * wave + (mt >> 1);
        if (oy >= a.H) continue;
#pragma unroll
        for (int e = 0; e < 4; ++e) {
            const int ox = ox0 + (mt & 1) * 16 + lg * 4 + e;
            if (ox < a.W) a.y[(((size_t)n * a.H + oy) * a.W + ox) * a.ldy + li] = out[h][mt][e];
        }
    }
    CT_STAMP(6);
    CT_STAMP_RT(7);
}

}

extern "C" int ct_stem_forward(const float *x, const float *pre_img, const float *pre_hm, int N, int H, int W,
                               const float *w_x, const float *w_img, const float *w_hm, const float *scale3,
                               const float *shift3, float *y, int ldy, void *stream)
{
    if (!x) CT_FAIL_ARG("ct_stem_forward: null pointer");
    return ct_stem_forward_parts(x, pre_img, pre_hm, nullptr, 0, N, H, W, w_x, w_img, w_hm, scale3, shift3, y, ldy, stream);
}

extern "C" int ct_stem_forward_parts(const float *x, const float *pre_img, const float *pre_hm, const float *add, int ldadd,
                                     int N, int H, int W, const float *w_x, const float *w_img, const float *w_hm,
                                     const float *scale3, const float *shift3, float *y, int ldy, void *stream)
{
    if (!scale3 || !shift3 || !y) CT_FAIL_ARG("ct_stem_forward: null pointer");
    if (!x && !pre_img && !pre_hm) CT_FAIL_ARG("ct_stem_forward_parts: no stem selected");
    if ((x && !w_x) || (pre_img && !w_img) || (pre_hm && !w_hm)) CT_FAIL_ARG("ct_stem_forward: input given without its weights");
    if (N <= 0 || H <= 0 || W <= 0 || ldy < 16 || (add && ldadd < 16)) CT_FAIL_ARG("ct_stem_forward: bad shape");
    StemArgs a;
    a.in[0] = x; a.in[1] = pre_img; a.in[2] = pre_hm;
    a.w[0] = w_x; a.w[1] = w_img; a.w[2] = w_hm;
    a.scale = scale3; a.shift = shift3; a.y = y; a.add = add; a.ldadd = ldadd;
    a.N = N; a.H = H; a.W = W; a.ldy = ldy;
    a.tilesX = ct_cdiv(W, ST_TW);
    const long blocks8 = (long)N * a.tilesX * ct_cdiv(H, 8);
    const int want = ct_tune_get(CT_TUNE_STEM_ROWS);
    const bool rows16 = want == 16 || (want == 0 && blocks8 > 768 && blocks8 <= 1536);
    a.tilesY = ct_cdiv(H, rows16 ? 16 : 8);
    const long blocks = (long)N * a.tilesX * a.tilesY;
    if (blocks > 0x7fffffffL) CT_FAIL_ARG("ct_stem_forward: grid too large");
    if (rows16) hipLaunchKernelGGL(stem_kernel<16>, dim3((unsigned)blocks), dim3(256), 0, (hipStream_t)stream, a);
    else hipLaunchKernelGGL(stem_kernel<8>, dim3((unsigned)blocks), dim3(256), 0, (hipStream_t)stream, a);
    CT_CHECK_LAUNCH("ct_stem_forward");
    return CT_OK;
}
```

### centertrack_amd/detector.py

```python
import ctypes
import math
import os
import time

import numpy as np
import torch

from . import _lib, fast_track, ops
NATIVE_LOOP = os.environ.get('CENTERTRACK_NATIVE_LOOP', '1') != '0'
SPLIT_STEM_MAX = int(os.environ.get('CENTERTRACK_SPLIT_STEM_MAX', '0'))
HOST_FLAG = os.environ.get('CENTERTRACK_HOST_FLAG', '1') != '0'
HOST_ROWS = os.environ.get('CENTERTRACK_HOST_ROWS', '1') != '0'
from .image import (affine_transform, draw_umich_gaussian, gaussian_radius, get_affine_transform, make_meta)
from .model import create_model, load_model
from .post_process import generic_post_process
from .tracker import Tracker

MEAN = np.array([0.40789654, 0.44719302, 0.47026115], dtype=np.float32).reshape(1, 1, 3)
STD = np.array([0.28863828, 0.27408164, 0.27809835], dtype=np.float32).reshape(1, 1, 3)
REST_FOCAL_LENGTH = {'nuscenes': 1200, 'kitti': 721.5377, 'kitti_tracking': 721.5377}
AVERAGE_FLIPS = ('hm', 'wh', 'dep', 'dim')
NEG_AVERAGE_FLIPS = ('amodel_offset',)
COCO_FLIP_IDX = [[1, 2], [3, 4], [5, 6], [7, 8], [9, 10], [11, 12], [13, 14], [15, 16]]


def trans_bbox(bbox, trans, width, height):
    bbox = np.array(bbox, dtype=np.float32).copy()
    bbox[:2] = affine_transform(bbox[:2], trans)
    bbox[2:] = affine_transform(bbox[2:], trans)
    bbox[[0, 2]] = np.clip(bbox[[0, 2]], 0, width - 1)
    bbox[[1, 3]] = np.clip(bbox[[1, 3]], 0, height - 1)
    return bbox


def render_pre_hm(tracks, meta, pre_thresh, out=None, with_hm=True):
    inp_w, inp_h = meta['inp_width'], meta['inp_height']
    out_w, out_h = meta['out_width'], meta['out_height']
    hm = np.zeros((inp_h, inp_w), np.float32) if out is None else out
    if out is not None:
        hm[...] = 0
    inds = []
    for det in tracks:
        if det['score'] < pre_thresh or det['active'] == 0:
            continue
        bbox = trans_bbox(det['bbox'], meta['trans_input'], inp_w, inp_h)
        bbox_out = trans_bbox(det['bbox'], meta['trans_output'], out_w, out_h)
        h, w = bbox[3] - bbox[1], bbox[2] - bbox[0]
        if h > 0 and w > 0:
            radius = max(0, int(gaussian_radius((math.ceil(h), math.ceil(w)))))
            ct = np.array([(bbox[0] + bbox[2]) / 2, (bbox[1] + bbox[3]) / 2], dtype=np.float32)
            if with_hm:
                draw_umich_gaussian(hm, ct.astype(np.int32), radius)
            ct_out = np.array([(bbox_out[0] + bbox_out[2]) / 2, (bbox_out[1] + bbox_out[3]) / 2], dtype=np.int32)
            inds.append(int(ct_out[1] * out_w + ct_out[0]))
    return hm, inds


def imread_bgr(path):
    try:
        import cv2
        img = cv2.imread(str(path))
        if img is None:
            raise _lib.CTError('cannot read image %r' % (path,))
        return img
    except ImportError:
        pass
    try:
        from PIL import Image
    except ImportError:
        raise _lib.CTError('reading image files needs cv2 or Pillow; pass the decoded uint8 BGR array instead')
    from PIL import ImageOps
    with Image.open(path) as im:
        im = ImageOps.exif_transpose(im)
        return np.ascontiguousarray(np.asarray(im.convert('RGB'))[:, :, ::-1])


class _HipGraph(object):

    def __init__(self, fn, collect=True):
        lib = _lib.load()
        side = torch.cuda.Stream()
        side.wait_stream(torch.cuda.current_stream())
        sp = ctypes.c_void_p(side.cuda_stream)
        with _lib.capture_guard(collect=collect), torch.cuda.stream(side):
            _lib.check(lib.ct_graph_begin(sp), 'ct_graph_begin')
            try:
                fn()
            finally:
                self.exec = lib.ct_graph_end(sp)
        torch.cuda.current_stream().wait_stream(side)
        if not self.exec:
            raise _lib.CTError('ct_graph_end failed: %s' % lib.ct_last_error().decode())
        self._lib = lib

    def replay(self, sp=None):
        rc = self._lib.ct_graph_launch(self.exec, sp if sp is not None else _lib.stream_ptr())
        if rc:
            _lib.check(rc, 'ct_graph_launch')

    def __del__(self):
        try:
            self._lib.ct_graph_destroy(self.exec)
        except Exception:
            pass


class StreamDetector(object):
    supports_prefetch = True

    def __init__(self, opt, model=None, num_streams=1, use_graph=True, native_host=True):
        if not torch.cuda.is_available():
            raise _lib.CTError('centertrack_amd needs an MI355X (no CPU fallback)')
        _lib.load()
        self.opt = opt
        self.device = torch.device('cuda', torch.cuda.current_device())
        opt.device = self.device
        if model is None:
            model = create_model(opt.arch, opt.heads, opt.head_conv, opt=opt)
            if getattr(opt, 'load_model', ''):
                model = load_model(model, opt.load_model, opt)
        self.model = model.to(self.device).eval()
        self.B = num_streams
        self.flip = bool(getattr(opt, 'flip_test', False))
        self.sparse = bool(getattr(opt, 'sparse_heads', False)) and not ({'hps', 'hm_hp'} & set(opt.heads))
        self.use_graph = use_graph
        self.trackers = [Tracker(opt) for _ in range(self.B)]
        self.native = bool(native_host and getattr(opt, 'tracking', False) and 'tracking' in opt.heads
                           and not getattr(opt, 'zero_pre_hm', False))
        self.fast = [fast_track.FastTracker(opt.new_thresh, getattr(opt, 'max_age', -1), opt.K,
                                            hungarian=getattr(opt, 'hungarian', False),
                                            public_det=getattr(opt, 'public_det', False))
                     for _ in range(self.B)] if self.native else None
        self._last_dets = None
        self._prefetched = None
        self.started = [False] * self.B
        lut = np.empty((3, 256), np.float32)
        mean, std = np.ascontiguousarray(MEAN.reshape(-1)), np.ascontiguousarray(STD.reshape(-1))
        _lib.check(_lib.load().ct_preprocess_lut(mean.ctypes.data, std.ctypes.data, 3, lut.ctypes.data), 'ct_preprocess_lut')
        self._lut = torch.from_numpy(lut).to(self.device)
        self._raw_bufs = {}
        self._carried = {}
        self.gather_fn = None
        self._rows_free = None
        self._ctx = None

    def __del__(self):
        try:
            ctx = self._ctx
            if ctx is not None and ctx.get('loop') is not None:
                if os.environ.get('CT_NO_CAPTURE_GUARD') != '1' and torch.cuda.is_current_stream_capturing():
                    return
                torch.cuda.synchronize()
                _lib.load().ct_frame_loop_destroy(ctx['loop'])
                ctx['loop'] = None
        except Exception:
            pass

    def _context(self, H, W):
        if self._ctx is not None and self._ctx['hw'] == (H, W):
            return self._ctx
        if self._ctx is not None and self._ctx.get('loop') is not None:
            torch.cuda.synchronize()
            _lib.load().ct_frame_loop_destroy(self._ctx['loop'])
            self._ctx['loop'] = None
        opt = self.opt
        NB = self.B * (2 if self.flip else 1)
        with_img = bool(getattr(opt, 'tracking', False)) and bool(getattr(opt, 'pre_img', True))
        with_hm = bool(getattr(opt, 'tracking', False)) and bool(getattr(opt, 'pre_hm', False))
        plan = self.model.get_plan(NB, H, W, with_img, with_hm, True, self.sparse)
        x_in, img_in, hm_in = plan['inputs']
        outs = plan['outputs']
        ctx = {'hw': (H, W), 'plan': plan, 'NB': NB}
        if self.flip:
            modes = {'hps': _lib.CT_FLIP_JOINT_OFFSETS, 'hm_hp': _lib.CT_FLIP_JOINTS}
            modes.update({k: _lib.CT_FLIP_AVG for k in AVERAGE_FLIPS})
            modes.update({k: _lib.CT_FLIP_NEG_EVEN for k in NEG_AVERAGE_FLIPS})
            merged, fl = {}, []
            for k, v in outs.items():
                if k in modes:
                    merged[k] = torch.empty((self.B,) + tuple(v.shape[1:]), device=self.device)
                    fl.append((v, merged[k], modes[k]))
                else:
                    merged[k] = v[:self.B]
            heads_arr = (_lib.FlipHead * len(fl))()
            for i, (v, m, mode) in enumerate(fl):
                assert v.stride(3) == 1 and v.stride(2) == v.shape[3] and v.stride(1) == v.shape[2] * v.shape[3]
                heads_arr[i].src, heads_arr[i].dst = v.data_ptr(), m.data_ptr()
                heads_arr[i].src_batch_stride, heads_arr[i].C, heads_arr[i].mode = v.stride(0), v.shape[1], mode
            pairs = np.ascontiguousarray(getattr(opt, 'flip_idx', COCO_FLIP_IDX), np.int32).reshape(-1, 2)
            hm0 = outs['hm']
            ctx['flip_call'] = (heads_arr, len(fl), pairs, int(hm0.shape[2]), int(hm0.shape[3]))
        else:
            merged = outs
        ctx['merged'] = merged
        dec_heads = {k: v for k, v in merged.items() if k != 'hm'}
        ctx['done_flag'] = torch.zeros((16,), dtype=torch.int32).pin_memory()
        sparse = plan.get('sparse')
        if sparse is not None:
            sparse = dict(sparse, zero_tracking=bool(getattr(opt, 'zero_tracking', False)), flip=self.flip)
        F = ops.Decoder.row_floats(dec_heads, [n for n, *_ in sparse['heads']] if sparse else None)
        ctx['host_out'] = torch.zeros((merged['hm'].shape[0], opt.K, F), dtype=torch.float32).pin_memory()
        direct = HOST_FLAG and HOST_ROWS
        ctx['decoder'] = ops.Decoder(merged['hm'], dec_heads, opt.K, host_out=ctx['host_out'] if direct else None,
                                     done_flag=ctx['done_flag'] if direct else None, sparse=sparse)
        assert tuple(ctx['decoder'].out.shape) == tuple(ctx['host_out'].shape)
        ctx['host_rows'] = ctx['host_out'].numpy()
        ctx['host_hm'] = torch.zeros((NB, 1, H, W), dtype=torch.float32).pin_memory() if (with_hm and not self.native) else None
        render = self.native and with_hm
        if render:
            nblob = ctx['max_blobs'] = fast_track.max_blobs(opt.K)
            nprm = self.B * nblob * 3
            ctx['pc_host'] = torch.zeros((nprm + self.B,), dtype=torch.int32).pin_memory()
            ctx['pc_dev'] = torch.zeros((nprm + self.B,), dtype=torch.int32, device=self.device)
            ctx['prm_host'] = ctx['pc_host'][:nprm].view(self.B, nblob, 3)
            ctx['cnt_host'] = ctx['pc_host'][nprm:]
            ctx['prm_dev'] = ctx['pc_dev'][:nprm]
            ctx['cnt_dev'] = ctx['pc_dev'][nprm:]
        if self.native:
            ctx['row_layout'] = fast_track.row_layout(ctx['decoder'].layout)
        nslots = 3 if img_in is not None else 2
        ctx['nslots'] = nslots
        ctx['frames'] = [torch.zeros_like(x_in) for _ in range(nslots)]
        ctx['slot'] = 0
        ctx['graphs'] = [None] * nslots
        ctx['raw'] = False
        ctx['loop'] = None
        ctx['launched'] = None
        ctx['copy_stream'] = None
        split = img_in is not None and hm_in is not None and 0 < NB <= SPLIT_STEM_MAX
        ctx['partial'] = [ops.new_view(NB, H, W, 16, self.device) for _ in range(nslots)] if split else None

        def pre_stage(slot):
            if not split:
                return
            cur, prev = ctx['frames'][slot], ctx['frames'][(slot - 1) % nslots]
            if self.flip:
                _lib.check(_lib.load().ct_flip_images(cur.data_ptr(), cur[self.B:].data_ptr(), self.B * 3 * H, W,
                                                      _lib.stream_ptr()), 'ct_flip_images')
            self.model.run_stem_partial(cur, prev, ctx['partial'][slot])
        ctx['pre_stage'] = pre_stage

        def device_frame(slot=0, with_copies=False):
            cur = ctx['frames'][slot]
            prev = ctx['frames'][(slot - 1) % nslots] if img_in is not None else None
            if with_copies and render:
                _lib.check(_lib.load().ct_memcpy_async(ctx['pc_dev'].data_ptr(), ctx['pc_host'].data_ptr(),
                                                       ctx['pc_host'].numel() * 4, 1, _lib.stream_ptr()), 'H2D')
            lib = _lib.load()
            if render:
                _lib.check(lib.ct_render_pre_hm(ctx['prm_dev'].data_ptr(), ctx['cnt_dev'].data_ptr(),
                                                ctx['max_blobs'], self.B, H, W, hm_in.data_ptr(),
                                                1 if self.flip else 0, _lib.stream_ptr()), 'ct_render_pre_hm')
            if self.flip and not split:
                _lib.check(lib.ct_flip_images(cur.data_ptr(), cur[self.B:].data_ptr(), self.B * 3 * H, W,
                                              _lib.stream_ptr()), 'ct_flip_images')
            self.model._run_plan(plan, inputs=(cur, prev, hm_in), stem_partial=ctx['partial'][slot] if split else None)
            if self.flip:
                arr, n, pairs, h, w = ctx['flip_call']
                _lib.check(lib.ct_flip_merge(arr, n, pairs.ctypes.data, len(pairs), self.B, h, w, _lib.stream_ptr()),
                           'ct_flip_merge')
            if getattr(opt, 'zero_tracking', False) and 'tracking' in merged:
                t = merged['tracking']
                for b in range(t.shape[0]):
                    _lib.check(lib.ct_memset_async(t[b].data_ptr(), 0, t[b].numel() * 4, _lib.stream_ptr()), 'memset')
            ctx['decoder'].run()
            if with_copies and not ctx['decoder'].direct:
                _lib.check(_lib.load().ct_memcpy_async(ctx['host_out'].data_ptr(), ctx['decoder'].out.data_ptr(),
                                                       ctx['host_out'].numel() * 4, 2, _lib.stream_ptr()), 'D2H')
                if HOST_FLAG:
                    _lib.check(_lib.load().ct_signal_host(ctx['done_flag'].data_ptr(), 1, _lib.stream_ptr()), 'ct_signal_host')

        ctx['device_frame'] = device_frame
        if self.use_graph:
            try:
                torch.cuda.synchronize()
                side = torch.cuda.Stream()
                side.wait_stream(torch.cuda.current_stream())
                with torch.cuda.stream(side):
                    pre_stage(0)
                    device_frame(0)
                torch.cuda.current_stream().wait_stream(side)
                torch.cuda.synchronize()
                raw = os.environ.get('CENTERTRACK_RAW_GRAPH', '1') != '0'
                for sl in range(nslots):
                    if raw:
                        g = _HipGraph(lambda: device_frame(sl, True), collect=(sl == 0))
                    else:
                        g = torch.cuda.CUDAGraph()
                        with _lib.capture_guard(collect=False), torch.cuda.graph(g):
                            device_frame(sl)
                    ctx['graphs'][sl] = g
                ctx['raw'] = raw
            except Exception as e:
                if os.environ.get('CENTERTRACK_GRAPH_FALLBACK', '0') != '1':
                    raise _lib.CTError('HIP graph capture of the frame failed (%s); pass use_graph=False or set '
                                       'CENTERTRACK_GRAPH_FALLBACK=1 to run eager launches' % (e,))
                import warnings
                warnings.warn('centertrack_amd: HIP graph capture failed (%s); using eager launches' % (e,))
                ctx['graphs'] = [None] * nslots
                torch.cuda.synchronize()
        ctx['graph'] = ctx['graphs'][0]
        if ctx['raw'] and self.native and NATIVE_LOOP:
            self._make_loop(ctx, H, W, render)
        self._ctx = ctx
        return ctx

    def _make_loop(self, ctx, H, W, render):
        lib = _lib.load()
        B, K, F = ctx['decoder'].out.shape
        d = _lib.FrameLoopDesc()
        d.B, d.K, d.F = int(B), int(K), int(F)
        ctx['loop_trackers'] = (ctypes.c_void_p * self.B)(*[f.h for f in self.fast])
        d.trackers = ctypes.cast(ctx['loop_trackers'], ctypes.POINTER(ctypes.c_void_p))
        d.layout = ctx['row_layout']
        d.out_thresh, d.pre_thresh = float(self.opt.out_thresh), float(self.opt.pre_thresh)
        d.inp_w, d.inp_h = int(W), int(H)
        d.host_rows = ctx['host_out'].data_ptr()
        ctx['rows_keep'] = np.zeros(tuple(ctx['decoder'].out.shape), np.float32)
        d.rows_keep = ctx['rows_keep'].ctypes.data
        if render:
            d.blob_params, d.blob_counts = ctx['prm_host'].data_ptr(), ctx['cnt_host'].data_ptr()
            d.blob_cap = ctx['max_blobs']
        d.nslots = ctx['nslots']
        for i in range(ctx['nslots']):
            d.graphs[i] = ctx['graphs'][i].exec
            d.frames[i] = ctx['frames'][i].data_ptr()
        d.frame_bytes = self.B * 3 * H * W * 4
        ctx['loop_stream'] = torch.cuda.current_stream()
        d.stream = ctx['loop_stream'].cuda_stream
        if ctx['partial'] is not None:
            P = self.model._prepare()
            d.pre.enabled = 1
            d.pre.N, d.pre.H, d.pre.W = ctx['NB'], int(H), int(W)
            d.pre.w_x, d.pre.w_img = P['stem_w'][0].data_ptr(), P['stem_w'][1].data_ptr()
            d.pre.scale3, d.pre.shift3 = P['stem_scale'].data_ptr(), P['stem_shift'].data_ptr()
            for i in range(ctx['nslots']):
                d.pre.partial[i] = ctx['partial'][i].ptr
            d.pre.ldp = ctx['partial'][0].ld
            d.pre.flip_B = self.B if self.flip else 0
        ctx['res_cap'] = self.fast[0].cap
        ctx['res_buf'] = np.zeros((self.B, ctx['res_cap']), fast_track.TRACK_DTYPE)
        d.results, d.results_cap = ctx['res_buf'].ctypes.data, ctx['res_cap']
        d.done_flag = ctx['done_flag'].data_ptr() if HOST_FLAG else None
        h = lib.ct_frame_loop_create(ctypes.byref(d))
        if not h:
            raise _lib.CTError('ct_frame_loop_create: %s' % lib.ct_last_error().decode())
        ctx['loop'] = ctypes.c_void_p(h)
        ctx['loop_desc'] = d
        ctx['counts'] = np.zeros(self.B, np.int32)
        ctx['tin'] = np.zeros((self.B, 6), np.float64)
        ctx['tinv'] = np.zeros((self.B, 6), np.float32)
        ctx['args'] = [_lib.FrameStepArgs(), _lib.FrameStepArgs()]
        for a in ctx['args']:
            a.trans_input, a.trans_inv = ctx['tin'].ctypes.data, ctx['tinv'].ctypes.data

    def _warp_frame(self, s, image, meta, frames, H, W):
        lib = _lib.load()
        if image.dtype != np.uint8 or image.ndim != 3 or image.shape[2] != 3:
            raise _lib.CTError('raw frames must be uint8 HxWx3 (got %s %s)' % (image.dtype, image.shape))
        h, w, c = image.shape
        if (int(meta['inp_height']), int(meta['inp_width'])) != (H, W):
            raise _lib.CTError('all streams of a step must share the network input size')
        need = h * w * c
        bufs = self._raw_bufs.get(s)
        if bufs is None or bufs[0].numel() < need:
            bufs = (torch.empty(need, dtype=torch.uint8).pin_memory(),
                    torch.empty(need, dtype=torch.uint8, device=self.device))
            self._raw_bufs[s] = bufs
        host, dev = bufs
        host.numpy()[:need].reshape(h, w, c)[...] = image
        st = _lib.stream_ptr()
        _lib.check(lib.ct_memcpy_async(dev.data_ptr(), host.data_ptr(), need, 1, st), 'H2D')
        trans = np.ascontiguousarray(meta['trans_input'], np.float64)
        _lib.check(lib.ct_preprocess_device(dev.data_ptr(), h, w, w * c, c, trans.ctypes.data, W, H,
                                            self._lut.data_ptr(), frames[s].data_ptr(),
                                            frames[self.B + s].data_ptr() if self.flip else None, st),
                   'ct_preprocess_device')

    def _meta_transforms(self, m):
        cached = m.get('_trans_inv')
        c_, s_ = m['c'], m['s']
        ident = (float(c_[0]), float(c_[1]), float(s_) if np.ndim(s_) == 0 else tuple(np.ravel(s_).tolist()),
                 m['out_width'], m['out_height'])
        if cached is None or cached[0] != ident:
            tinv = np.ascontiguousarray(get_affine_transform(
                m['c'], m['s'], 0, (m['out_width'], m['out_height']), inv=1).astype(np.float32))
            m['_trans_inv'] = cached = (ident, tinv)
        return cached[1]

    def _checked_submit(self, ctx, rc, what):
        if rc == 0:
            return
        lib = _lib.load()
        msg = lib.ct_last_error().decode('utf-8', 'replace')
        lib.ct_frame_loop_wait(ctx['loop'])
        lib.ct_frame_loop_forget_upload(ctx['loop'])
        ctx['launched'] = None
        self._prefetched = None
        raise _lib.CTError('%s failed (%d): %s' % (what, rc, msg))

    def _drop_launched(self, ctx):
        if ctx.get('loop') is not None and ctx['launched'] is not None:
            _lib.check(_lib.load().ct_frame_loop_wait(ctx['loop']), 'ct_frame_loop_wait')
            _lib.load().ct_frame_loop_forget_upload(ctx['loop'])
            ctx['slot'] = (ctx['slot'] - 1) % ctx['nslots']
            ctx['launched'] = None

    def _step_native(self, ctx, images, metas, timers, prefetch, prefetch_metas):
        cs = torch.cuda.current_stream()
        ls = ctx['loop_stream']
        if cs != ls:
            ls.wait_stream(cs)
            try:
                with torch.cuda.stream(ls):
                    return self._step_native_on_loop_stream(ctx, images, metas, timers, prefetch, prefetch_metas)
            finally:
                cs.wait_stream(ls)
        return self._step_native_on_loop_stream(ctx, images, metas, timers, prefetch, prefetch_metas)

    def _step_native_on_loop_stream(self, ctx, images, metas, timers, prefetch, prefetch_metas):
        lib = _lib.load()
        t0 = time.time()
        B, n = self.B, ctx['nslots']
        loop = ctx['loop']
        launched = ctx['launched']
        ahead = launched is not None and launched[0] is images and launched[1] == images._version
        if launched is not None and not ahead:
            self._drop_launched(ctx)
        cur, nxt = ctx['args']
        if ahead:
            if any(a is not b for a, b in zip(launched[2], metas)) and [self._meta_transforms(m).tobytes() for m in metas] != launched[3]:
                raise _lib.CTError('step(): the metas of this frame differ from the prefetch_metas promised for it')
            ctx['launched'] = None
            slot = (ctx['slot'] - 1) % n
        else:
            slot = ctx['slot']
            tin, tinv = ctx['tin'], ctx['tinv']
            for s_ in range(B):
                tinv[s_] = self._meta_transforms(metas[s_]).reshape(-1)
                tin[s_] = np.asarray(metas[s_]['trans_input'], np.float64).reshape(-1)
            pf = self._prefetched
            self._prefetched = None
            cur.slot, cur.frame, cur.next_frame = slot, None, None
            if pf is not None and pf[0] is images and pf[1] == images._version and pf[2] == slot:
                cur.frame_kind = _lib.CT_FRAME_UPLOADED
            elif images.dtype == torch.float32 and images.is_contiguous():
                cur.frame_kind = _lib.CT_FRAME_DEVICE if images.device.type == 'cuda' else _lib.CT_FRAME_HOST
                cur.frame = images.data_ptr()
            else:
                if pf is not None:
                    lib.ct_frame_loop_forget_upload(loop)
                    pf = None
                ctx['frames'][slot][:B].copy_(images)
                cur.frame_kind = _lib.CT_FRAME_IN_PLACE
            if pf is not None and cur.frame_kind != _lib.CT_FRAME_UPLOADED:
                lib.ct_frame_loop_forget_upload(loop)
        can_prefetch = (prefetch is not None and torch.is_tensor(prefetch) and prefetch.device.type == 'cpu'
                        and prefetch.dtype == torch.float32 and prefetch.is_contiguous()
                        and tuple(prefetch.shape) == tuple(images.shape))
        t1 = time.time()
        if ahead:
            if can_prefetch:
                _lib.check(lib.ct_frame_loop_upload(loop, (slot + 1) % n, prefetch.data_ptr()), 'ct_frame_loop_upload')
        else:
            if can_prefetch:
                cur.next_frame = prefetch.data_ptr()
            if self._rows_free is not None:
                ctx['loop_stream'].wait_event(self._rows_free)
                self._rows_free = None
            self._checked_submit(ctx, lib.ct_frame_loop_submit(loop, ctypes.byref(cur)), 'ct_frame_loop_submit')
            ctx['slot'] = (slot + 1) % n
        if can_prefetch:
            self._prefetched = (prefetch, prefetch._version, (slot + 1) % n)
        if self.gather_fn is not None:
            ev = self.gather_fn(ctx['decoder'].out)
            if isinstance(ev, torch.cuda.Event):
                ctx['loop_stream'].wait_event(ev)
        counts = ctx['counts']
        early = (can_prefetch and prefetch_metas is not None
                 and all(a is b for a, b in zip(prefetch_metas, metas)))
        if early:
            nxt.slot, nxt.frame_kind, nxt.frame, nxt.next_frame = (slot + 1) % n, _lib.CT_FRAME_UPLOADED, None, None
            ctx['slot'] = (slot + 1) % n
            self._checked_submit(ctx, lib.ct_frame_loop_finish_submit(loop, ctypes.byref(cur), counts.ctypes.data,
                                                                      ctypes.byref(nxt)), 'ct_frame_loop_finish_submit')
            ctx['slot'] = (slot + 2) % n
            ctx['launched'] = (prefetch, prefetch._version, list(metas),
                               [self._meta_transforms(m).tobytes() for m in metas])
            self._prefetched = None
        else:
            _lib.check(lib.ct_frame_loop_finish(loop, ctypes.byref(cur), counts.ctypes.data), 'ct_frame_loop_finish')
        t2 = time.time()
        self._last_dets = None
        res, cap = ctx['res_buf'], ctx['res_cap']
        out = []
        for s_ in range(B):
            k = int(counts[s_])
            if k > cap:
                tmp = np.zeros(k, fast_track.TRACK_DTYPE)
                got = lib.ct_tracker_get_tracks(self.fast[s_].h, tmp.ctypes.data, k)
                out.append(tmp[:min(got, k)])
            else:
                out.append(res[s_, :k].copy())
        if timers is not None:
            timers.update({'pre': t1 - t0, 'net': t2 - t1, 'dec': 0.0, 'post': 0.0, 'merge': 0.0,
                           'track': time.time() - t2})
        return out

    def step(self, images, metas, timers=None, prefetch=None, prefetch_metas=None):
        opt = self.opt
        t0 = time.time()
        B = self.B
        raw_frames = isinstance(images, (list, tuple))
        if not raw_frames and self.flip and images.shape[0] == 2 * B:
            images = images[:B]
        assert len(images) == B and len(metas) == B
        if raw_frames:
            H, W = int(metas[0]['inp_height']), int(metas[0]['inp_width'])
        else:
            H, W = int(images.shape[2]), int(images.shape[3])
        ctx = self._context(H, W)
        x_in, img_in, hm_in = ctx['plan']['inputs']
        lib = _lib.load()
        if (ctx['loop'] is not None and not raw_frames and all(self.started) and tuple(images.shape) == (B, 3, H, W)
                and not getattr(opt, 'public_det', False) and not getattr(opt, 'zero_tracking', False)):
            return self._step_native(ctx, images, metas, timers, prefetch, prefetch_metas)
        self._drop_launched(ctx)
        cur = torch.cuda.current_stream()
        sp = ctypes.c_void_p(cur.cuda_stream)
        n = ctx['nslots']
        slot = ctx['slot']
        fr = ctx['frames'][slot]
        pf = self._prefetched
        self._prefetched = None
        if raw_frames:
            self._forget_upload(ctx, pf)
            for s in range(B):
                self._warp_frame(s, images[s], metas[s], fr, H, W)
        else:
            if tuple(images.shape) != (B, 3, H, W):
                raise _lib.CTError('step() expects [%d,3,%d,%d] frames, got %s' % (B, H, W, tuple(images.shape)))
            if pf is not None and pf[0] is images and pf[1] == images._version and pf[2] == slot:
                if ctx['loop'] is not None:
                    self._forget_upload(ctx, pf)
                else:
                    cur.wait_event(ctx['frame_ready'])
            else:
                self._forget_upload(ctx, pf)
                if images.dtype == torch.float32 and images.is_contiguous():
                    kind = 0 if images.device.type == 'cuda' else 1
                    _lib.check(lib.ct_memcpy_async(fr.data_ptr(), images.data_ptr(), images.numel() * 4, kind, sp),
                               'frame copy')
                else:
                    fr[:B].copy_(images)
        tracking = bool(getattr(opt, 'tracking', False))
        if tracking:
            for s in range(B):
                if not self.started[s]:
                    pre_dets = metas[s].get('pre_dets', [])
                    if self.native and len(pre_dets) > 0:
                        self.fast[s].init_tracks(pre_dets)
                    if not self.native:
                        self.trackers[s].init_track(pre_dets)
            if img_in is not None:
                prev = ctx['frames'][(slot - 1) % n]
                fresh = [s for s in range(B) if not self.started[s]]
                if fresh and self.flip:
                    _lib.check(lib.ct_flip_images(fr.data_ptr(), fr[B:].data_ptr(), B * 3 * H, W, sp), 'ct_flip_images')
                if len(fresh) == B:
                    prev.copy_(fr)
                else:
                    for s in fresh:
                        prev[s].copy_(fr[s])
                        if self.flip:
                            prev[B + s].copy_(fr[B + s])
            if hm_in is not None and self.native:
                ph, ch = ctx['prm_host'].numpy(), ctx['cnt_host'].numpy()
                for s in range(B):
                    m = metas[s]
                    ch[s], _ = self.fast[s].prehm_params(opt.pre_thresh, m['trans_input'], m['inp_width'],
                                                         m['inp_height'], out=ph[s])
                if not ctx['raw']:
                    ctx['pc_dev'].copy_(ctx['pc_host'], non_blocking=True)
            elif hm_in is not None:
                hh = ctx['host_hm']
                for s in range(B):
                    render_pre_hm(self.trackers[s].tracks, metas[s], opt.pre_thresh, out=hh[s, 0].numpy(),
                                  with_hm=not getattr(opt, 'zero_pre_hm', False))
                    if self.flip:
                        hh[B + s, 0].copy_(torch.flip(hh[s, 0], [1]))
                hm_in.copy_(hh, non_blocking=True)
            for s in range(B):
                self.started[s] = True
        t1 = time.time()
        if self._rows_free is not None:
            cur.wait_event(self._rows_free)
            self._rows_free = None
        if ctx['partial'] is not None:
            if ctx['loop'] is not None:
                _lib.check(lib.ct_frame_loop_prestage(ctx['loop'], slot), 'ct_frame_loop_prestage')
            else:
                ctx['pre_stage'](slot)
        if ctx['raw']:
            ctx['graphs'][slot].replay(sp)
        elif ctx['graphs'][slot] is not None:
            ctx['graphs'][slot].replay()
        else:
            ctx['device_frame'](slot)
        ctx['slot'] = (slot + 1) % n
        if (prefetch is not None and torch.is_tensor(prefetch) and prefetch.device.type == 'cpu'
                and prefetch.dtype == torch.float32 and prefetch.is_contiguous() and tuple(prefetch.shape) == (B, 3, H, W)):
            ns = (slot + 1) % n
            if ctx['loop'] is not None:
                _lib.check(lib.ct_frame_loop_upload(ctx['loop'], ns, prefetch.data_ptr()), 'ct_frame_loop_upload')
            else:
                if ctx['copy_stream'] is None:
                    ctx['copy_stream'] = torch.cuda.Stream(device=self.device)
                    ctx['frame_ready'] = torch.cuda.Event()
                    ctx['copy_sp'] = ctypes.c_void_p(ctx['copy_stream'].cuda_stream)
                _lib.check(lib.ct_memcpy_async(ctx['frames'][ns].data_ptr(), prefetch.data_ptr(), prefetch.numel() * 4, 1,
                                               ctx['copy_sp']), 'prefetch')
                ctx['frame_ready'].record(ctx['copy_stream'])
            self._prefetched = (prefetch, prefetch._version, ns)
        if self.gather_fn is not None:
            ev = self.gather_fn(ctx['decoder'].out)
            self._rows_free = ev if isinstance(ev, torch.cuda.Event) else None
        if ctx['raw']:
            _lib.check(lib.ct_stream_synchronize(sp), 'ct_stream_synchronize')
        else:
            ctx['host_out'].copy_(ctx['decoder'].out, non_blocking=True)
            cur.synchronize()
        t2 = time.time()
        rows = ctx['host_rows']
        if ctx.get('rows_keep') is not None:
            ctx['rows_keep'][...] = rows
        self._last_dets = None
        all_results = []
        t_post = t_track = 0.0
        if self.native:
            ta = time.time()
            for s in range(B):
                m = metas[s]
                tinv = self._meta_transforms(m)
                pub = m['cur_dets'] if getattr(opt, 'public_det', False) else None
                all_results.append(self.fast[s].step(rows[s], ctx['row_layout'], opt.out_thresh, tinv, pub).copy())
            t_track = time.time() - ta
        dets = None if self.native else self.last_dets
        for s in (range(B) if not self.native else []):
            ta = time.time()
            meta = metas[s]
            one = {k: v[s:s + 1] for k, v in dets.items()}
            res = generic_post_process(opt, one, [meta['c']], [meta['s']], meta['out_height'], meta['out_width'],
                                       opt.num_classes, [meta['calib']], meta['height'], meta['width'])[0]
            res = [r for r in res if r['score'] > opt.out_thresh]
            tb = time.time()
            if tracking:
                public_det = meta['cur_dets'] if getattr(opt, 'public_det', False) else None
                res = self.trackers[s].step(res, public_det)
            tc = time.time()
            t_post += tb - ta
            t_track += tc - tb
            all_results.append(res)
        if timers is not None:
            timers.update({'pre': t1 - t0, 'net': t2 - t1, 'dec': 0.0, 'post': t_post, 'merge': 0.0,
                           'track': t_track})
        return all_results

    def _forget_upload(self, ctx, pf):
        if pf is None:
            return
        if ctx['loop'] is not None:
            _lib.load().ct_frame_loop_forget_upload(ctx['loop'])
        if ctx['copy_stream'] is not None:
            ctx['copy_stream'].synchronize()

    @property
    def last_dets(self):
        if self._last_dets is None and self._ctx is not None:
            keep = self._ctx.get('rows_keep')
            self._last_dets = self._ctx['decoder'].unpack((keep if keep is not None else self._ctx['host_rows']).copy())
        return self._last_dets

    def reset_tracking(self, stream=None):
        if self._ctx is not None:
            self._drop_launched(self._ctx)
            self._forget_upload(self._ctx, self._prefetched)
        for s in (range(self.B) if stream is None else [stream]):
            self.trackers[s].reset()
            if self.fast is not None:
                self.fast[s].reset()
            self._carried.pop(s, None)
            self.started[s] = False
        self._prefetched = None

    def results_as_dicts(self, results, stream=0, meta=None):
        if isinstance(results, np.ndarray):
            carried = self._carried.setdefault(stream, {})
            tinv = meta['_trans_inv'][1] if (meta is not None and '_trans_inv' in meta) else None
            return fast_track.as_dicts(results, self.last_dets, stream, None if meta is None else meta.get('calib'),
                                       carried, tinv)
        return results


class Detector(object):

    def __init__(self, opt, model=None, use_graph=True, native_host=True):
        if not hasattr(opt, 'device'):
            opt.device = torch.device('cuda')
        self._init_host(opt)
        self.impl = StreamDetector(opt, model=model, num_streams=1, use_graph=use_graph, native_host=native_host)
        self.model = self.impl.model

    def _init_host(self, opt):
        scales = list(getattr(opt, 'test_scales', [1.0]))
        if len(scales) != 1:
            raise _lib.CTError('centertrack_amd.Detector supports one test scale (got test_scales=%s): multi-scale '
                               'testing (detector.py:78, merge_outputs) is not part of the accelerated path' % scales)
        self.opt = opt
        self.mean, self.std = MEAN, STD
        self.pause = not getattr(opt, 'no_pause', True)
        self.rest_focal_length = (REST_FOCAL_LENGTH.get(getattr(opt, 'dataset', ''), 1200)
                                  if getattr(opt, 'test_focal_length', -1) < 0 else opt.test_focal_length)
        self.cnt = 0

    @property
    def tracker(self):
        return self.impl.fast[0] if self.impl.native else self.impl.trackers[0]

    def pre_process(self, image, scale, input_meta={}):
        import ctypes
        opt = self.opt
        image = np.ascontiguousarray(image)
        height, width, ch = image.shape
        meta = self.frame_meta(image, input_meta)
        inp_h, inp_w = meta['inp_height'], meta['inp_width']
        flip = bool(getattr(opt, 'flip_test', False))
        out = np.empty((2 if flip else 1, ch, inp_h, inp_w), np.float32)
        trans = np.ascontiguousarray(meta['trans_input'], np.float64)
        mean = np.ascontiguousarray(self.mean.reshape(-1)[:ch], np.float32)
        std = np.ascontiguousarray(self.std.reshape(-1)[:ch], np.float32)
        _lib.check(_lib.load().ct_preprocess_image(
            image.ctypes.data_as(ctypes.c_void_p), height, width, image.strides[0], ch,
            trans.ctypes.data_as(ctypes.c_void_p), inp_w, inp_h, mean.ctypes.data_as(ctypes.c_void_p),
            std.ctypes.data_as(ctypes.c_void_p), out.ctypes.data_as(ctypes.c_void_p), 1 if flip else 0),
            'ct_preprocess_image')
        return torch.from_numpy(out), meta

    def frame_meta(self, image, input_meta={}):
        opt = self.opt
        if image.dtype != np.uint8 or image.ndim != 3:
            raise _lib.CTError('pre_process expects a uint8 HxWxC image (got %s %s)' % (image.dtype, image.shape))
        height, width = image.shape[:2]
        meta = make_meta(getattr(opt, 'input_h', -1), getattr(opt, 'input_w', -1), height, width,
                         down_ratio=getattr(opt, 'down_ratio', 4), calib=input_meta.get('calib'),
                         focal_length=self.rest_focal_length, fix_res=bool(getattr(opt, 'fix_res', True)),
                         fix_short=getattr(opt, 'fix_short', 0), pad=getattr(opt, 'pad', 31))
        if 'pre_dets' in input_meta:
            meta['pre_dets'] = input_meta['pre_dets']
        if 'cur_dets' in input_meta:
            meta['cur_dets'] = input_meta['cur_dets']
        return meta

    def run(self, image_or_path_or_tensor, meta={}):
        start = time.time()
        x = image_or_path_or_tensor
        if isinstance(x, dict):
            images, meta = self.parse_prefetched(x)
        elif torch.is_tensor(x):
            images = x
        elif isinstance(x, (str, os.PathLike)) or isinstance(x, np.ndarray):
            if not isinstance(x, np.ndarray):
                x = imread_bgr(x)
            if getattr(self.opt, 'device_pre_process', True) and x.ndim == 3 and x.shape[2] == 3:
                images, meta = [x], self.frame_meta(x, meta)
            else:
                images, meta = self.pre_process(x, 1.0, meta)
        else:
            raise _lib.CTError('run() takes an image path, a uint8 image array, a normalised tensor + meta, or a '
                               'pre-processed dict (got %s)' % type(x).__name__)
        loaded = time.time()
        timers = {}
        results = self.impl.results_as_dicts(self.impl.step(images, [meta], timers)[0], 0, meta)
        self.cnt += 1
        end = time.time()
        ret = {'results': results, 'tot': end - start, 'load': loaded - start, 'display': 0.0}
        ret.update(timers)
        return ret

    def parse_prefetched(self, x):
        scale = self.opt.test_scales[0] if hasattr(self.opt, 'test_scales') else 1.0
        images = x['images'][scale][0]
        meta = {k: (v.numpy()[0] if torch.is_tensor(v) else v) for k, v in x['meta'][scale].items()}
        for k in ('pre_dets', 'cur_dets'):
            if k in x['meta']:
                meta[k] = x['meta'][k]
        return images, meta

    def reset_tracking(self):
        self.impl.reset_tracking()


def default_opt(heads, **kw):
    import types
    o = types.SimpleNamespace(
        arch='dla_34', heads=heads, head_conv=256, dla_node='dcn', head_kernel=3, load_model='',
        tracking=True, pre_img=True, pre_hm=True, zero_pre_hm=False, flip_test=False, K=100,
        track_thresh=0.3, out_thresh=-1.0, pre_thresh=-1.0, new_thresh=0.3, max_age=-1, hungarian=False,
        public_det=False, zero_tracking=False, depth_scale=1.0, down_ratio=4, num_classes=heads['hm'],
        test_scales=[1.0], model_output_list=False, no_pause=True, dataset='', test_focal_length=-1,
        input_h=512, input_w=512, fix_res=True, fix_short=0, pad=31)
    for k, v in kw.items():
        setattr(o, k, v)
    if o.tracking:
        o.out_thresh = max(o.track_thresh, o.out_thresh)
        o.pre_thresh = max(o.track_thresh, o.pre_thresh)
        o.new_thresh = max(o.track_thresh, o.new_thresh)
    return o
```

### centertrack_amd/model.py

```python
import ctypes
import os
from collections import OrderedDict

import torch

from . import _lib, autotune, ops
from .ops import View
from .weights import CHANNELS, LEVELS, dla34_param_shapes

BN_EPS = 1e-5
SMALL_SLOT_WGS = 600
FUSE_OFFSET = os.environ.get('CENTERTRACK_FUSE_OFFSET', '1') != '0'
WINOGRAD = os.environ.get('CENTERTRACK_WINOGRAD', '1') != '0'
FUSE_HEADS = os.environ.get('CENTERTRACK_FUSE_HEADS', '1') != '0'
FOLD_POOL = os.environ.get('CENTERTRACK_FOLD_POOL', '1') != '0'
FUSE_PROJ = os.environ.get('CENTERTRACK_FUSE_PROJ', '1') != '0'


def _fold_bn(sd, p):
    scale = sd[p + '.weight'].double() / torch.sqrt(sd[p + '.running_var'].double() + BN_EPS)
    shift = sd[p + '.bias'].double() - sd[p + '.running_mean'].double() * scale
    return scale.float().contiguous(), shift.float().contiguous()


class _Launch(object):
    __slots__ = ('fn', 'args', 'name', 'keep', 'us', 'ws_need')

    def __init__(self, name, fn, args, keep=(), reads=(), writes=(), us=5.0, ws_need=0):
        self.name, self.fn, self.args, self.keep = name, fn, args, keep
        self.us, self.ws_need = us, ws_need


class _DcnLayer(object):
    __slots__ = ('name', 'x', 'cout', 'out', 'up', 'main', 'finish', 'desc', 'fused', 'splits', 'use_ws', 'nkk')

    def __init__(self, name, x, cout, out, up):
        self.name, self.x, self.cout, self.out, self.up = name, x, cout, out, up


class DLASegHIP(torch.nn.Module):

    def __init__(self, heads, head_conv=256, pre_img=True, pre_hm=True, depth_scale=1.0,
                 model_output_list=False):
        super().__init__()
        self.heads = OrderedDict(heads)
        if isinstance(head_conv, dict):
            vals = {tuple(v) if isinstance(v, (list, tuple)) else (v,) for v in head_conv.values()}
            assert len(vals) == 1 and len(next(iter(vals))) == 1, 'only one head-conv layer is supported'
            head_conv = next(iter(vals))[0]
        self.head_conv = head_conv
        self.pre_img, self.pre_hm = pre_img, pre_hm
        self.depth_scale = depth_scale
        self.model_output_list = model_output_list
        self._names = []
        for key, shape, kind in dla34_param_shapes(self.heads, head_conv, pre_img, pre_hm):
            if kind == 'bn':
                for suf, val in (('weight', 1.0), ('bias', 0.0), ('running_mean', 0.0), ('running_var', 1.0)):
                    self._reg(key + '.' + suf, torch.full(shape, val))
                self._reg(key + '.num_batches_tracked', torch.tensor(0, dtype=torch.long))
            else:
                self._reg(key, torch.zeros(shape))
        self._prepared = None
        self._plans = {}

    def _reg(self, name, t):
        self.register_buffer(name.replace('.', '__'), t)
        self._names.append(name)

    def state_dict(self, *a, **k):
        return OrderedDict((n, getattr(self, n.replace('.', '__'))) for n in self._names)

    def load_state_dict(self, sd, strict=True):
        missing = [n for n in self._names if n not in sd]
        unexpected = [k for k in sd if k not in set(self._names)]
        if strict and (missing or unexpected):
            raise RuntimeError('missing %s unexpected %s' % (missing[:5], unexpected[:5]))
        for n in self._names:
            if n in sd:
                buf = getattr(self, n.replace('.', '__'))
                if tuple(buf.shape) != tuple(sd[n].shape):
                    raise RuntimeError('shape mismatch for %s: %s vs %s' % (n, tuple(buf.shape), tuple(sd[n].shape)))
                buf.copy_(sd[n])
        self._prepared = None
        self._plans = {}
        return missing, unexpected

    def _prepare(self):
        if self._prepared is not None:
            return self._prepared
        dev = next(self.buffers()).device
        if dev.type != 'cuda':
            raise _lib.CTError('DLASegHIP runs on an MI355X only: call .to("cuda") first (no CPU fallback)')
        _lib.load()
        sd = {k: v.to(dev) for k, v in self.state_dict().items()}
        P = {}

        def wino(w):
            ok = WINOGRAD and w.shape[2] == 3 and w.shape[1] % 64 == 0
            return ops.pack_winograd(w) if ok else None

        def conv_bn(wkey, bnkey):
            sc, sh = _fold_bn(sd, bnkey)
            return ops.pack_weight(sd[wkey]), sc, sh, wino(sd[wkey])

        P['stem_w'] = [sd['base.base_layer.0.weight'].contiguous(),
                       sd['base.pre_img_layer.0.weight'].contiguous() if self.pre_img else None,
                       sd['base.pre_hm_layer.0.weight'].contiguous() if self.pre_hm else None]
        sc3 = torch.ones(3, 16, device=dev)
        sh3 = torch.zeros(3, 16, device=dev)
        for i, (name, on) in enumerate((('base_layer', True), ('pre_img_layer', self.pre_img),
                                        ('pre_hm_layer', self.pre_hm))):
            if on:
                sc3[i], sh3[i] = _fold_bn(sd, 'base.%s.1' % name)
        P['stem_scale'], P['stem_shift'] = sc3.contiguous(), sh3.contiguous()
        P['level0'] = conv_bn('base.level0.0.weight', 'base.level0.1')
        P['level1'] = conv_bn('base.level1.0.weight', 'base.level1.1')

        def leaf(p, cin, cout):
            d = {'c11': conv_bn(p + '.tree1.conv1.weight', p + '.tree1.bn1'),
                 'c12': conv_bn(p + '.tree1.conv2.weight', p + '.tree1.bn2'),
                 'c21': conv_bn(p + '.tree2.conv1.weight', p + '.tree2.bn1'),
                 'c22': conv_bn(p + '.tree2.conv2.weight', p + '.tree2.bn2'),
                 'root': conv_bn(p + '.root.conv.weight', p + '.root.bn')}
            if cin != cout:
                d['proj'] = conv_bn(p + '.project.0.weight', p + '.project.1')
            return d

        for i in range(2, 6):
            p = 'base.level%d' % i
            if LEVELS[i] == 1:
                P[p] = leaf(p, CHANNELS[i - 1], CHANNELS[i])
            else:
                P[p + '.tree1'] = leaf(p + '.tree1', CHANNELS[i - 1], CHANNELS[i])
                P[p + '.tree2'] = leaf(p + '.tree2', CHANNELS[i], CHANNELS[i])

        def deform(p):
            sc, sh = _fold_bn(sd, p + '.actf.0')
            sh = (sd[p + '.conv.bias'].double() * sc.double() + sh.double()).float().contiguous()
            return {'w': ops.pack_weight(sd[p + '.conv.weight']), 'scale': sc, 'shift': sh,
                    'w_off': ops.pack_weight(sd[p + '.conv.conv_offset_mask.weight']),
                    'w_off_wino': wino(sd[p + '.conv.conv_offset_mask.weight']),
                    'b_off': sd[p + '.conv.conv_offset_mask.bias'].contiguous()}

        for p, n in (('dla_up.ida_0', 1), ('dla_up.ida_1', 2), ('dla_up.ida_2', 3), ('ida_up', 2)):
            for k in range(1, n + 1):
                P['%s.proj_%d' % (p, k)] = deform('%s.proj_%d' % (p, k))
                P['%s.node_%d' % (p, k)] = deform('%s.node_%d' % (p, k))
                P['%s.up_%d' % (p, k)] = ops.upsample_weight(sd['%s.up_%d.weight' % (p, k)])
        hc = self.head_conv
        small = ([h for h, c in self.heads.items() if c <= 8 and h != 'hm_hp']
                 if (FUSE_HEADS and WINOGRAD and hc == 256) else [])
        small = small[:_lib.CT_MAX_FUSED_HEADS]
        P['heads_small'] = small
        def fused(names):
            w0s = torch.cat([sd[h + '.0.weight'] for h in names], 0)
            w2s = torch.zeros((len(names), 8, hc), device=dev)
            b2s = torch.zeros((len(names), 8), device=dev)
            for i, h in enumerate(names):
                c = self.heads[h]
                w2s[i, :c] = sd[h + '.2.weight'].reshape(c, hc)
                b2s[i, :c] = sd[h + '.2.bias']
            return (ops.pack_winograd(w0s), torch.cat([sd[h + '.0.bias'] for h in names], 0).contiguous(),
                    w2s.contiguous(), b2s.contiguous())

        if small:
            P['hs:' + ','.join(small)] = fused(small)
            if 'hm' in small and small != ['hm']:
                P['hs:hm'] = fused(['hm'])
        big = [h for h in self.heads if h not in small]
        P['heads_big'] = big
        if small and big:
            w0b = torch.cat([sd[h + '.0.weight'] for h in big], 0)
            P['hb_w'], P['hb_ww'] = ops.pack_weight(w0b), wino(w0b)
            P['hb_b'] = torch.cat([sd[h + '.0.bias'] for h in big], 0).contiguous()
        w0 = torch.cat([sd[h + '.0.weight'] for h in self.heads], 0)
        P['head0_w'] = ops.pack_weight(w0)
        P['head0_ww'] = wino(w0)
        P['head0_b'] = torch.cat([sd[h + '.0.bias'] for h in self.heads], 0).contiguous()
        hc = self.head_conv
        ctot = sum(self.heads.values())
        w2 = torch.zeros((ctot, hc * len(self.heads), 1, 1), device=dev)
        c0 = 0
        for j, (h, c) in enumerate(self.heads.items()):
            w2[c0:c0 + c, hc * j:hc * (j + 1)] = sd[h + '.2.weight']
            c0 += c
        P['head2_w'] = ops.pack_weight(w2)
        P['head2_b'] = torch.cat([sd[h + '.2.bias'] for h in self.heads], 0).contiguous()
        for h in self.heads:
            P[h + '.2'] = (ops.pack_weight(sd[h + '.2.weight']), sd[h + '.2.bias'].contiguous())
        if hc == 256:
            for h, c in self.heads.items():
                if h in _lib.HEAD_INDEX:
                    P['sparse.' + h] = (ops.pack_weight(sd[h + '.0.weight']), sd[h + '.0.bias'].contiguous(),
                                        sd[h + '.2.weight'].reshape(c, hc).contiguous(), sd[h + '.2.bias'].contiguous())
        self._prepared = P
        return P

    def _build_plan(self, N, H, W, with_img, with_hm, fuse_sigmoid, sparse_heads=False):
        P = self._prepare()
        lib = _lib.load()
        dev = next(self.buffers()).device
        if H % 32 or W % 32:
            raise _lib.CTError('input %dx%d must be a multiple of 32 (reference pads to 32 too, opts.py:297)' % (H, W))
        plan = {'launches': [], 'ws_need': 0}
        L = plan['launches']
        tune = autotune.enabled()

        def alloc(h, w, c):
            return ops.new_view(N, h, w, c, dev)

        def add_conv(name, x, pk, cout, ks, stride=1, relu=True, res=None, out=None, **kw):
            wp, sc, sh, ww = pk
            d = ops.make_conv_desc(x, wp, cout, ks, stride, scale=sc, shift=sh, res=res, relu=relu, out=out,
                                   w_wino=(ww if stride == 1 else None), **kw)
            us = autotune.tune_conv(d, dev)[2] if tune else 10.0
            L.append(_Launch(name, 'conv', d, (x, res, out, pk, kw.get('out_nchw'), kw.get('pool'), kw.get('proj')), reads=(x, res),
                             writes=(out, kw.get('out_nchw')), us=us,
                             ws_need=lib.ct_conv2d_workspace_bytes(ctypes.byref(d))))
            return out

        x_in = torch.zeros((N, 3, H, W), device=dev)
        img_in = torch.zeros((N, 3, H, W), device=dev) if with_img else None
        hm_in = torch.zeros((N, 1, H, W), device=dev) if with_hm else None
        plan['inputs'] = (x_in, img_in, hm_in)
        s0 = alloc(H, W, 16)
        L.append(_Launch('stem', 'stem', (x_in, img_in, hm_in, s0), (), reads=(x_in, img_in, hm_in), writes=(s0,), us=46.0))
        l0 = add_conv('level0', s0, P['level0'], 16, 3, out=alloc(H, W, 16))
        l1 = add_conv('level1', l0, P['level1'], 32, 3, stride=2, out=alloc(H // 2, W // 2, 32))

        def leaf(name, x, pk, cin, cout, stride, R, out, bottom=None, level_root=False, make_bottom=False):
            h, w = x.H // stride, x.W // stride
            fold = None
            fuse_proj = FUSE_PROJ and stride == 2 and cin != cout
            if stride > 1 and bottom is None:
                if level_root:
                    bottom = R.slice(2 * cout, cin)
                    make_bottom = True
                elif not fuse_proj:
                    bottom = alloc(h, w, cin)
                    make_bottom = True
            elif stride == 1:
                bottom = x
            if stride > 1 and make_bottom:
                if FOLD_POOL:
                    fold = bottom
                else:
                    L.append(_Launch(name + '.pool', 'pool', (x, bottom), reads=(x,), writes=(bottom,)))
            t = alloc(h, w, cout)
            x1 = R.slice(cout, cout)
            x2 = R.slice(0, cout)
            if fuse_proj:
                residual = alloc(h, w, cout)
                add_conv(name + '.t1.conv1+project', x, pk['c11'], cout, 3, stride=stride, out=t, pool=fold,
                         proj=(pk['proj'][0], pk['proj'][1], pk['proj'][2], residual))
            else:
                add_conv(name + '.t1.conv1', x, pk['c11'], cout, 3, stride=stride, out=t, pool=fold)
                if cin != cout:
                    residual = add_conv(name + '.project', bottom, pk['proj'], cout, 1, relu=False, out=alloc(h, w, cout))
                else:
                    residual = bottom
            add_conv(name + '.t1.conv2', t, pk['c12'], cout, 3, res=residual, out=x1)
            add_conv(name + '.t2.conv1', x1, pk['c21'], cout, 3, out=t)
            add_conv(name + '.t2.conv2', t, pk['c22'], cout, 3, res=x1, out=x2)
            add_conv(name + '.root', View(R.buf, R.c0, R.C), pk['root'], cout, 1, out=out)
            return out

        feats = [l0, l1]
        x = l1
        for i in range(2, 6):
            p = 'base.level%d' % i
            cin, cout = CHANNELS[i - 1], CHANNELS[i]
            h, w = x.H // 2, x.W // 2
            out = alloc(h, w, cout)
            level_root = i >= 3
            if LEVELS[i] == 1:
                R = alloc(h, w, 2 * cout + (cin if level_root else 0))
                leaf(p, x, P[p], cin, cout, 2, R, out, level_root=level_root)
            else:
                R2 = alloc(h, w, 3 * cout + cin)
                bottom = R2.slice(2 * cout, cin)
                x1 = R2.slice(2 * cout + cin, cout)
                R1 = alloc(h, w, 2 * cout)
                leaf(p + '.tree1', x, P[p + '.tree1'], cin, cout, 2, R1, x1, bottom=bottom, make_bottom=True)
                leaf(p + '.tree2', x1, P[p + '.tree2'], cout, cout, 1, R2, out)
            feats.append(out)
            x = out

        dcn_layers = []

        def deform(name, x, cout, out, up=None):
            dcn_layers.append(_DcnLayer(name, x, cout, out, up))
            return out

        def ida(p, layers, startp, endp, o, up_f):
            for i in range(startp + 1, endp):
                k = i - startp
                f = up_f[k]
                xi = layers[i]
                up = alloc(xi.H * f, xi.W * f, o)
                deform('%s.proj_%d' % (p, k), xi, o, alloc(xi.H, xi.W, o),
                       up=(P['%s.up_%d' % (p, k)], f, layers[i - 1], up))
                layers[i] = deform('%s.node_%d' % (p, k), up, o, alloc(up.H, up.W, o))

        layers = list(feats)
        outs = [layers[-1]]
        ida('dla_up.ida_0', layers, 4, 6, 256, [1, 2]); outs.insert(0, layers[-1])
        ida('dla_up.ida_1', layers, 3, 6, 128, [1, 2, 2]); outs.insert(0, layers[-1])
        ida('dla_up.ida_2', layers, 2, 6, 64, [1, 2, 2, 2]); outs.insert(0, layers[-1])
        y = [outs[0], outs[1], outs[2]]
        ida('ida_up', y, 0, 3, 64, [1, 2, 4])
        feat = y[-1]
        plan['feat'] = feat
        produced0 = {id(f_.buf): 0 for f_ in feats}
        knobs, dcn_launches = self._tune_dcn_schedule(dcn_layers, produced0, N, H, W, dev, tune)
        plan['dcn_knobs'] = knobs
        plan['dcn_layers'] = {ly.name: (ly.up[3] if ly.up is not None else ly.out) for ly in dcn_layers}
        L.extend(dcn_launches)

        small, big = P['heads_small'], P['heads_big']
        plan['sparse'] = None
        if sparse_heads:
            sp = [h for h in self.heads if ('sparse.' + h) in P]
            if {'ltrb', 'ltrb_amodal'} & set(self.heads):
                sp = [h for h in sp if h not in ('reg', 'wh')]
            if not sp or 'hm' not in self.heads or {'hps', 'hm_hp'} & set(self.heads) or not fuse_sigmoid:
                raise _lib.CTError('sparse heads need an hm head, regression heads with head_conv 256, no pose heads '
                                   'and the detector\'s fused epilogues')
            plan['sparse'] = {'feat': feat, 'heads': [(h,) + P['sparse.' + h] for h in sp], 'depth_scale': self.depth_scale}
            small = [h for h in small if ('sparse.' + h) not in P]
            if any(('sparse.' + h) in P for h in big):
                raise _lib.CTError('sparse heads: %s do not fit the fused-heads launch' % [h for h in big if ('sparse.' + h) in P])
        if small or plan['sparse'] is not None:
            outputs = self._plan_heads_fused(plan, L, P, feat, N, dev, tune, fuse_sigmoid, small, big)
        else:
            nh = len(self.heads)
            hc = self.head_conv
            mid = alloc(feat.H, feat.W, hc * nh)
            d = ops.make_conv_desc(feat, P['head0_w'], hc * nh, 3, 1, shift=P['head0_b'], relu=True, out=mid,
                                   w_wino=P['head0_ww'])
            us = autotune.tune_conv(d, dev)[2] if tune else 200.0
            L.append(_Launch('heads.0', 'conv', d, (feat, mid), reads=(feat,), writes=(mid,), us=us,
                             ws_need=lib.ct_conv2d_workspace_bytes(ctypes.byref(d))))
            ctot = sum(self.heads.values())
            comb = torch.empty((N, ctot, feat.H, feat.W), device=dev)
            sig, dep = (0, 0), (0, 0)
            c0 = 0
            outputs = OrderedDict()
            for hname, c in self.heads.items():
                if fuse_sigmoid and hname == 'hm':
                    sig = (c0, c0 + c)
                if fuse_sigmoid and hname == 'dep':
                    dep = (c0, c0 + c)
                outputs[hname] = comb[:, c0:c0 + c]
                c0 += c
            if ctot <= 32 and 'hm_hp' not in self.heads:
                d = ops.make_conv_desc(mid, P['head2_w'], ctot, 1, 1, shift=P['head2_b'], out_nchw=comb, sig=sig, dep=dep,
                                       depth_scale=self.depth_scale)
                us = autotune.tune_conv(d, dev)[2] if tune else 20.0
                L.append(_Launch('heads.2', 'conv', d, (mid, comb), reads=(mid,), writes=(comb,), us=us,
                                 ws_need=lib.ct_conv2d_workspace_bytes(ctypes.byref(d))))
            else:
                outputs = OrderedDict()
                for j, (hname, c) in enumerate(self.heads.items()):
                    o = torch.empty((N, c, feat.H, feat.W), device=dev)
                    wp, b = P[hname + '.2']
                    hsig = (0, c) if (fuse_sigmoid and hname in ('hm', 'hm_hp')) else (0, 0)
                    hdep = (0, c) if (fuse_sigmoid and hname == 'dep') else (0, 0)
                    d = ops.make_conv_desc(mid.slice(hc * j, hc), wp, c, 1, 1, shift=b, out_nchw=o, sig=hsig, dep=hdep,
                                           depth_scale=self.depth_scale)
                    us = autotune.tune_conv(d, dev)[2] if tune else 7.0
                    L.append(_Launch('heads.%s.2' % hname, 'conv', d, (mid, o), reads=(mid.slice(hc * j, hc),), writes=(o,),
                                     us=us, ws_need=lib.ct_conv2d_workspace_bytes(ctypes.byref(d))))
                    outputs[hname] = o
        plan['outputs'] = outputs
        need = max([l.ws_need for l in L if l.fn == 'conv'] + [16])
        ws = torch.empty(need // 4, dtype=torch.float32, device=dev)
        plan['ws'] = [ws]
        for l in L:
            if l.fn == 'conv':
                l.args.workspace, l.args.workspace_bytes = ws.data_ptr(), ws.numel() * 4
        plan['ws_need'] = ws.numel() * 4
        return plan

    def _plan_heads_fused(self, plan, L, P, feat, N, dev, tune, fuse_sigmoid, small, big):
        lib = _lib.load()
        hc = self.head_conv
        outputs = {}
        if small:
            ctot = sum(self.heads[h] for h in small)
            comb = torch.empty((N, ctot, feat.H, feat.W), device=dev)
            hd = _lib.HeadsDesc()
            hd.x, hd.N, hd.H, hd.W, hd.Cin, hd.ldx = feat.ptr, N, feat.H, feat.W, feat.C, feat.ld
            hs_w0, hs_b0, hs_w2, hs_b2 = P['hs:' + ','.join(small)]
            hd.w0_winograd, hd.b0, hd.nheads = hs_w0.data_ptr(), hs_b0.data_ptr(), len(small)
            hd.w2, hd.b2, hd.out, hd.ctot = hs_w2.data_ptr(), hs_b2.data_ptr(), comb.data_ptr(), ctot
            hd.depth_scale = self.depth_scale
            c0 = 0
            for i, h in enumerate(small):
                c = self.heads[h]
                hd.cout[i], hd.coff[i] = c, c0
                if fuse_sigmoid and h == 'hm':
                    hd.sig_lo, hd.sig_hi = c0, c0 + c
                if fuse_sigmoid and h == 'dep':
                    hd.dep_lo, hd.dep_hi = c0, c0 + c
                outputs[h] = comb[:, c0:c0 + c]
                c0 += c
            L.append(_Launch('heads.fused[%s]' % ' + '.join(small), 'heads', hd, (feat, comb, hs_w0, hs_b0, hs_w2, hs_b2),
                             us=100.0))
        if big:
            mid = ops.new_view(N, feat.H, feat.W, hc * len(big), dev)
            d = ops.make_conv_desc(feat, P['hb_w'], hc * len(big), 3, 1, shift=P['hb_b'], relu=True, out=mid, w_wino=P['hb_ww'])
            us = autotune.tune_conv(d, dev)[2] if tune else 100.0
            L.append(_Launch('heads.0', 'conv', d, (feat, mid), us=us, ws_need=lib.ct_conv2d_workspace_bytes(ctypes.byref(d))))
            for j, h in enumerate(big):
                c = self.heads[h]
                o = torch.empty((N, c, feat.H, feat.W), device=dev)
                wp, b = P[h + '.2']
                hsig = (0, c) if (fuse_sigmoid and h in ('hm', 'hm_hp')) else (0, 0)
                hdep = (0, c) if (fuse_sigmoid and h == 'dep') else (0, 0)
                d = ops.make_conv_desc(mid.slice(hc * j, hc), wp, c, 1, 1, shift=b, out_nchw=o, sig=hsig, dep=hdep,
                                       depth_scale=self.depth_scale)
                us = autotune.tune_conv(d, dev)[2] if tune else 7.0
                L.append(_Launch('heads.%s.2' % h, 'conv', d, (mid, o), us=us,
                                 ws_need=lib.ct_conv2d_workspace_bytes(ctypes.byref(d))))
                outputs[h] = o
        return OrderedDict((h, outputs[h]) for h in self.heads if h in outputs)

    def run_stem_partial(self, x, pre_img, out):
        P = self._prepare()
        lib = _lib.load()
        w = P['stem_w']
        rc = lib.ct_stem_forward_parts(x.data_ptr(), ops._p(pre_img), None, None, 0, x.shape[0], x.shape[2], x.shape[3],
                                       w[0].data_ptr(), ops._p(w[1]) if pre_img is not None else None, None,
                                       P['stem_scale'].data_ptr(), P['stem_shift'].data_ptr(), out.ptr, out.ld,
                                       _lib.stream_ptr())
        if rc != 0:
            _lib.check(rc, 'stem (x / pre_img terms)')

    def _run_plan(self, plan, inputs=None, stem_partial=None, launches=None):
        P = self._prepared
        lib = _lib.load()
        st = _lib.stream_ptr()
        for l in (plan['launches'] if launches is None else launches):
            if l.fn == 'conv':
                rc = lib.ct_conv2d(ctypes.byref(l.args), st)
            elif l.fn == 'dcn_group':
                arr, n, phases = l.args
                rc = lib.ct_dcn_v2_group(arr, n, phases, st)
            elif l.fn == 'heads':
                rc = lib.ct_heads_fused(ctypes.byref(l.args), st)
            elif l.fn == 'pool':
                x, y = l.args
                rc = lib.ct_maxpool2x2(x.ptr, x.N, x.H, x.W, x.C, x.ld, y.ptr, y.ld, st)
            elif l.fn == 'stem':
                x, img, hm, y = l.args
                if inputs is not None:
                    x, img, hm = inputs
                w = P['stem_w']
                if stem_partial is not None:
                    if hm is None:
                        raise _lib.CTError('a split stem needs the pre_hm input')
                    rc = lib.ct_stem_forward_parts(None, None, hm.data_ptr(), stem_partial.ptr, stem_partial.ld,
                                                   x.shape[0], x.shape[2], x.shape[3], None, None, w[2].data_ptr(),
                                                   P['stem_scale'].data_ptr(), P['stem_shift'].data_ptr(), y.ptr, y.ld, st)
                    if rc != 0:
                        _lib.check(rc, l.name)
                    continue
                rc = lib.ct_stem_forward(x.data_ptr(), ops._p(img), ops._p(hm), x.shape[0], x.shape[2], x.shape[3],
                                         w[0].data_ptr(), ops._p(w[1]) if img is not None else None,
                                         ops._p(w[2]) if hm is not None else None,
                                         P['stem_scale'].data_ptr(), P['stem_shift'].data_ptr(), y.ptr, y.ld, st)
            else:
                raise AssertionError(l.fn)
            if rc != 0:
                _lib.check(rc, l.name)

    def _schedule_dcn(self, layers, produced0, N, dev, knobs, tune=True):
        lib = _lib.load()
        P = self._prepared
        fuse_max_cin, cps, nkk = knobs[:3]
        split_offsets = knobs[3] if len(knobs) > 3 else 1
        cps_small = knobs[4] if len(knobs) > 4 else 0
        small_unfuse = knobs[5] if len(knobs) > 5 else 0
        persist = knobs[6] if len(knobs) > 6 else 0
        slot_cps = {}
        sizes, mains = self._dcn_slot_sizes(layers, produced0, N, cps, with_mains=True)
        if cps_small and cps_small < cps:
            for t, wgs in sizes.items():
                if wgs < SMALL_SLOT_WGS:
                    slot_cps[t] = cps_small
        unfuse_slots = set()
        if small_unfuse == 2:
            unfuse_slots = {m for ly, m in zip(layers, mains) if not (ly.x.C % 64 == 0 and ly.x.C <= fuse_max_cin and FUSE_OFFSET)}
        time_of = dict(produced0)

        def t_of(view):
            return time_of.get(id(view.buf), 0)

        slots = {}
        convs = {}
        offs = {}
        for ly in layers:
            pk = P[ly.name]
            nchunks = ly.x.C // 32
            ly.main = t_of(ly.x) // 2 + 1
            c = slot_cps.get(ly.main, cps)
            ly.fused = (ly.x.C % 64 == 0 and ly.x.C <= fuse_max_cin and FUSE_OFFSET
                        and not (small_unfuse and ly.main in slot_cps) and ly.main not in unfuse_slots)
            ly.nkk = 2 if (c == 1 or ly.x.C % 64) else nkk
            ly.splits = max(1, nchunks // c)
            om = part = None
            raw = False
            if not ly.fused and split_offsets == 2 and ly.x.C % 64 == 0 and pk['w_off_wino'] is not None:
                raw = True
                omv = ops.new_view(N, ly.x.H, ly.x.W, 32, dev)
                part = omv.buf
                d = ops.make_conv_desc(ly.x, pk['w_off'], 27, 3, 1, out=omv, w_wino=pk['w_off_wino'])
                if tune:
                    autotune.tune_conv(d, dev)
                convs.setdefault(ly.main, []).append(
                    _Launch(ly.name + '.offset', 'conv', d, (ly.x, omv, pk),
                            ws_need=lib.ct_conv2d_workspace_bytes(ctypes.byref(d))))
            elif not ly.fused and split_offsets and ly.x.C % 64 == 0:
                part = torch.empty((ly.x.C // 64) * N * ly.x.H * ly.x.W * 32, dtype=torch.float32, device=dev)
                offs.setdefault(ly.main, []).append(ly)
            elif not ly.fused:
                om = ops.new_view(N, ly.x.H, ly.x.W, 32, dev)
                d = ops.make_conv_desc(ly.x, pk['w_off'], 27, 3, 1, shift=pk['b_off'], out=om, sig=(18, 27))
                if tune:
                    autotune.tune_conv(d, dev)
                convs.setdefault(ly.main, []).append(
                    _Launch(ly.name + '.offset', 'conv', d, (ly.x, om, pk),
                            ws_need=lib.ct_conv2d_workspace_bytes(ctypes.byref(d))))
            own = ly.fused or part is not None
            dd = ops.make_dcn_desc(ly.x, om, pk['w'], ly.cout, pk['scale'], pk['shift'], True, ly.out, up=ly.up,
                                   split_k=ly.splits, algo=3264, om_partial=part, raw_offsets=raw,
                                   w_off=pk['w_off'] if own else None, b_off=pk['b_off'] if own else None,
                                   w_off_wino=pk['w_off_wino'] if (split_offsets == 3 and not ly.fused) else None)
            need_c = ctypes.c_size_t(0)
            _lib.check(lib.ct_dcn_v2_group_plan(ctypes.byref(dd), ctypes.byref(need_c), None), 'DCN layer ' + ly.name)
            need = need_c.value
            ly.use_ws = need > 0
            keep = [ly.x, om, part, ly.out, pk, ly.up]
            if need:
                ws = torch.empty(need // 4, dtype=torch.float32, device=dev)
                dd.workspace, dd.workspace_bytes = ws.data_ptr(), need
                keep.append(ws)
            ly.desc = (dd, keep)
            if ly.use_ws:
                ly.finish = max(ly.main, (t_of(ly.up[2]) + 1) // 2) if ly.up is not None else ly.main
                done = 2 * ly.finish + 1
            else:
                ly.finish = None
                done = 2 * ly.main
            time_of[id((ly.up[3] if ly.up is not None else ly.out).buf)] = done
            slots.setdefault(ly.main, {'main': [], 'finish': []})['main'].append(ly)
            if ly.finish is not None:
                slots.setdefault(ly.finish, {'main': [], 'finish': []})['finish'].append(ly)
        out = []

        def group(lys, phases, tag):
            if phases == _lib.CT_DCN_MAIN:
                lys = sorted(lys, key=lambda ly: -((ly.x.C // 32 + ly.splits - 1) // ly.splits))
            for i in range(0, len(lys), 4):
                part = lys[i:i + 4]
                arr = (_lib.DcnDesc * len(part))()
                keep = []
                def can_persist(ly):
                    cpsplit = -(-(ly.x.C // 32) // ly.splits)
                    return (not ly.fused and (ly.x.C // 32) % cpsplit == 0
                            and cpsplit % (4 if ly.nkk == 4 else 2) == 0)
                pers = bool(persist) and phases == _lib.CT_DCN_MAIN and all(can_persist(ly) for ly in part)
                for j, ly in enumerate(part):
                    ctypes.memmove(ctypes.byref(arr[j]), ctypes.byref(ly.desc[0]), ctypes.sizeof(_lib.DcnDesc))
                    arr[j].algo = (43264 if ly.nkk == 4 else 3264) + (20000 if pers and ly.nkk == 4 else 50000 if pers else 0)
                    keep.append(ly.desc[1])
                name = '%s[%s]' % (tag, ' + '.join(ly.name for ly in part))
                out.append(_Launch(name, 'dcn_group', (arr, len(part), phases), keep))

        for t in sorted(slots):
            out.extend(convs.get(t, []))
            if offs.get(t):
                group(offs[t], _lib.CT_DCN_OFFSETS, 'dcn.offsets')
            lys = slots[t]['main']
            if lys:
                group(lys, _lib.CT_DCN_MAIN, 'dcn')
            if slots[t]['finish']:
                group(slots[t]['finish'], _lib.CT_DCN_FINISH, 'dcn.finish')
        return out

    @staticmethod
    def _dcn_slot_sizes(layers, produced0, N, cps, with_mains=False):
        time_of = dict(produced0)
        sizes = {}
        mains = []
        for ly in layers:
            main = time_of.get(id(ly.x.buf), 0) // 2 + 1
            mains.append(main)
            splits = max(1, (ly.x.C // 32) // cps)
            use_ws = splits > 1 or ly.up is not None
            if use_ws:
                fin = max(main, (time_of.get(id(ly.up[2].buf), 0) + 1) // 2) if ly.up is not None else main
                done = 2 * fin + 1
            else:
                done = 2 * main
            time_of[id((ly.up[3] if ly.up is not None else ly.out).buf)] = done
            tiles = N * ((ly.x.H + 1) // 2) * ((ly.x.W + 15) // 16) * ((ly.cout + 63) // 64)
            sizes[main] = sizes.get(main, 0) + tiles * splits
        return (sizes, mains) if with_mains else sizes

    def _time_launches(self, launches, reps=10):
        plan = {'launches': launches}
        need = max([l.ws_need for l in launches if l.fn == 'conv'] + [16])
        dev = next(self.buffers()).device
        ws = torch.empty(need // 4, dtype=torch.float32, device=dev)
        for l in launches:
            if l.fn == 'conv':
                l.args.workspace, l.args.workspace_bytes = ws.data_ptr(), ws.numel() * 4
        side = torch.cuda.Stream()
        side.wait_stream(torch.cuda.current_stream())
        with torch.cuda.stream(side):
            self._run_plan(plan)
        torch.cuda.current_stream().wait_stream(side)
        torch.cuda.synchronize()
        g = torch.cuda.CUDAGraph()
        with _lib.capture_guard(collect=False), torch.cuda.graph(g):
            for _ in range(reps):
                self._run_plan(plan)
        g.replay()
        torch.cuda.synchronize()
        best = None
        e0, e1 = torch.cuda.Event(enable_timing=True), torch.cuda.Event(enable_timing=True)
        for _ in range(2):
            e0.record()
            g.replay()
            e1.record()
            torch.cuda.synchronize()
            t = e0.elapsed_time(e1) * 1e3 / reps
            best = t if best is None else min(best, t)
        del g
        return best

    def _tune_dcn_schedule(self, layers, produced0, N, H, W, dev, tune):
        env = os.environ.get('CENTERTRACK_DCN_KNOBS', '')
        if env:
            knobs = tuple(int(v) for v in env.split(','))
            return knobs, self._schedule_dcn(layers, produced0, N, dev, knobs, tune)
        default = (128, 4, 2, 1, 0, 0, 0)
        if not tune:
            return default, self._schedule_dcn(layers, produced0, N, dev, default, tune)
        key = 'dcnplan5:%d,%d,%d' % (N, H, W)
        key4 = 'dcnplan4:%d,%d,%d' % (N, H, W)
        key3 = 'dcnplan3:%d,%d,%d' % (N, H, W)
        autotune._load_file()
        retune = os.environ.get('CENTERTRACK_DCN_RETUNE', '0') == '1'
        if key in autotune._CACHE and not retune:
            knobs = tuple(int(v) for v in autotune._CACHE[key][:-1])
            return knobs, self._schedule_dcn(layers, produced0, N, dev, knobs)
        if key4 in autotune._CACHE and not retune:
            knobs = tuple(int(v) for v in autotune._CACHE[key4][:-1]) + (0,)
            return knobs, self._schedule_dcn(layers, produced0, N, dev, knobs)
        if key3 in autotune._CACHE and not retune:
            knobs = tuple(int(v) for v in autotune._CACHE[key3][:4]) + (0, 0, 0)
            return knobs, self._schedule_dcn(layers, produced0, N, dev, knobs)
        best = None
        tried = []
        for fuse_max in (0, 64, 128, 256):
            for cps in (2, 4, 8):
                for nkk in (2, 4):
                    for so in ((1, 2, 3) if fuse_max < 256 else (1,)):
                        small = [t for t, w in self._dcn_slot_sizes(layers, produced0, N, cps).items() if w < SMALL_SLOT_WGS]
                        for cs, un in (((0, 0), (0, 2)) + tuple((c, u) for c in (2, 1) if c < cps for u in (0, 1, 2)) if small
                                       else ((0, 0), (0, 2))):
                            knobs = (fuse_max, cps, nkk, so, cs, un, 0)
                            launches = self._schedule_dcn(layers, produced0, N, dev, knobs)
                            us = self._time_launches(launches)
                            if os.environ.get('CENTERTRACK_TUNE_VERBOSE'):
                                print('dcn schedule N=%d %dx%d knobs %s: %d launches, %.1f us' % (N, H, W, knobs, len(launches), us))
                            tried.append((us, knobs))
                            if best is None or us < best[0]:
                                best = (us, knobs)
                            del launches
        tried.sort()
        stage2 = os.environ.get('CENTERTRACK_DCN_TUNE_PERSIST', '0') == '1'
        for us0, k0 in (tried[:5] + [t for t in tried[5:] if t[1][0] == 0 and t[1][5] == 0]) if stage2 else ():
            knobs = k0[:6] + (1,)
            launches = self._schedule_dcn(layers, produced0, N, dev, knobs)
            if any(l.fn == 'dcn_group' and int(l.args[0][0].algo) >= 50000 for l in launches):
                us = self._time_launches(launches)
                if os.environ.get('CENTERTRACK_TUNE_VERBOSE'):
                    print('dcn schedule N=%d %dx%d knobs %s: %d launches, %.1f us (%.1f without)' % (N, H, W, knobs, len(launches), us, us0))
                if us < best[0]:
                    best = (us, knobs)
            del launches
        autotune._CACHE[key] = tuple(best[1]) + (round(best[0], 1),)
        autotune._save_file()
        return best[1], self._schedule_dcn(layers, produced0, N, dev, best[1])

    @staticmethod
    def plan_signature(plan):
        parts = ['dcn_knobs=%s' % (tuple(plan.get('dcn_knobs', ())),)]
        for l in plan['launches']:
            if l.fn == 'conv':
                parts.append('%s:conv:%d:%d' % (l.name, int(l.args.algo), int(l.args.split_k)))
            elif l.fn == 'dcn_group':
                arr, n, phases = l.args
                parts.append('%s:dcn:%d:%s' % (l.name, phases, ','.join(
                    '%d/%d/%d' % (int(arr[j].algo), int(arr[j].split_k), int(arr[j].fuse_offset)) for j in range(n))))
            else:
                parts.append('%s:%s' % (l.name, l.fn))
        return ';'.join(parts)

    def get_plan(self, N, H, W, with_img, with_hm, fuse_sigmoid=False, sparse_heads=False):
        key = (N, H, W, with_img, with_hm, fuse_sigmoid, sparse_heads)
        if key not in self._plans:
            self._plans[key] = self._build_plan(*key)
        return self._plans[key]

    def forward_plan(self, plan, x, pre_img=None, pre_hm=None):
        xi, ii, hi = plan['inputs']
        xi.copy_(x)
        if ii is not None:
            ii.copy_(pre_img)
        if hi is not None:
            hi.copy_(pre_hm)
        self._run_plan(plan)
        return plan['outputs']

    @torch.no_grad()
    def forward(self, x, pre_img=None, pre_hm=None, fuse_sigmoid=False):
        if pre_img is not None and not self.pre_img:
            raise _lib.CTError('model was built with pre_img=False')
        if pre_hm is not None and not self.pre_hm:
            raise _lib.CTError('model was built with pre_hm=False')
        N, _, H, W = x.shape
        plan = self.get_plan(N, H, W, pre_img is not None, pre_hm is not None, fuse_sigmoid)
        out = self.forward_plan(plan, x, pre_img, pre_hm)
        z = OrderedDict((k, v.clone()) for k, v in out.items())
        if self.model_output_list:
            return [[z[h] for h in sorted(self.heads)]]
        return [z]


def create_model(arch, head, head_conv, opt=None):
    if arch != 'dla_34':
        raise ValueError('centertrack_amd implements arch "dla_34" only (got %r)' % arch)
    if opt is not None and getattr(opt, 'dla_node', 'dcn') != 'dcn':
        raise ValueError('only dla_node="dcn" is implemented')
    if opt is not None and getattr(opt, 'head_kernel', 3) != 3:
        raise ValueError('only head_kernel=3 is implemented')
    return DLASegHIP(head, head_conv,
                     pre_img=getattr(opt, 'pre_img', True) if opt is not None else True,
                     pre_hm=getattr(opt, 'pre_hm', True) if opt is not None else True,
                     depth_scale=getattr(opt, 'depth_scale', 1.0) if opt is not None else 1.0,
                     model_output_list=getattr(opt, 'model_output_list', False) if opt is not None else False)


def load_model(model, model_path, opt=None, optimizer=None):
    ckpt = torch.load(model_path, map_location='cpu')
    sd_in = ckpt['state_dict'] if 'state_dict' in ckpt else ckpt
    if 'epoch' in ckpt:
        print('loaded {}, epoch {}'.format(model_path, ckpt['epoch']))
    sd = {}
    for k, v in sd_in.items():
        sd[k[7:] if k.startswith('module') and not k.startswith('module_list') else k] = v
    own = model.state_dict()
    reset_hm = bool(getattr(opt, 'reset_hm', False))
    reuse_hm = bool(getattr(opt, 'reuse_hm', False))
    keep = {}
    for k, v in sd.items():
        if k in own:
            mismatch = tuple(v.shape) != tuple(own[k].shape)
            if mismatch or (reset_hm and k.startswith('hm') and v.shape[0] in (80, 1)):
                if reuse_hm and tuple(v.shape[1:]) == tuple(own[k].shape[1:]):
                    print('Reusing parameter {}, required shape{}, loaded shape{}.'.format(
                        k, tuple(own[k].shape), tuple(v.shape)))
                    n = min(v.shape[0], own[k].shape[0])
                    merged = own[k].clone()
                    merged[:n] = v[:n]
                    keep[k] = merged
                else:
                    print('Skip loading parameter {}, required shape{}, loaded shape{}.'.format(
                        k, tuple(own[k].shape), tuple(v.shape)))
            else:
                keep[k] = v
        else:
            print('Drop parameter {}.'.format(k))
    for k in own:
        if k not in keep:
            print('No param {}.'.format(k))
    model.load_state_dict(keep, strict=False)
    return model
```

### include/centertrack_hip.h

```cpp
#ifndef CENTERTRACK_HIP_H
#define CENTERTRACK_HIP_H

#include <stddef.h>
#include <stdint.h>

#ifdef __cplusplus
extern "C" {
#endif

#define CT_OK 0
#define CT_ERR_ARG 1
#define CT_ERR_LAUNCH 2
#define CT_ERR_WORKSPACE 3

#define CT_RELU 1
#define CT_OUT_NCHW 2

#define CT_ABI_VERSION 103

const char *ct_last_error(void);
int ct_version(void);
int ct_set_tuning(const char *key, int value);

size_t ct_packed_weight_elems(int Cout, int Cin, int ks);
int ct_pack_conv_weight(const float *w_oihw, float *packed, int Cout, int Cin, int ks, void *stream);
size_t ct_packed_winograd_elems(int Cout, int Cin);
int ct_pack_winograd_weight(const float *w_oihw, float *packed, int Cout, int Cin, void *stream);

typedef struct ct_conv_desc {
    const float *x; int N, H, W, Cin, ldx;
    const float *w_packed; int Cout, ks, stride;
    const float *scale; const float *shift;
    const float *res; int ldr;
    float *y; int ldy;
    int flags;
    int sig_lo, sig_hi;
    int dep_lo, dep_hi; float depth_scale;
    float *workspace; size_t workspace_bytes;
    int split_k;
    int algo;
    const float *w_winograd;
    float *pool_y; int pool_ld;
    const float *proj_w_packed; const float *proj_scale; const float *proj_shift;
    float *proj_y; int proj_ldy;
} ct_conv_desc;
int ct_conv2d(const ct_conv_desc *d, void *stream);
size_t ct_conv2d_workspace_bytes(const ct_conv_desc *d);

#define CT_MAX_FUSED_HEADS 8
typedef struct ct_heads_desc {
    const float *x; int N, H, W, Cin, ldx;
    const float *w0_winograd; const float *b0;
    int nheads;
    const float *w2; const float *b2;
    int cout[CT_MAX_FUSED_HEADS], coff[CT_MAX_FUSED_HEADS];
    float *out; int ctot;
    int sig_lo, sig_hi, dep_lo, dep_hi; float depth_scale;
} ct_heads_desc;
int ct_heads_fused(const ct_heads_desc *d, void *stream);

typedef struct ct_dcn_desc {
    const float *x; int N, H, W, Cin, ldx;
    const float *om; int ldom;
    const float *w_packed; int Cout;
    const float *scale; const float *shift;
    float *y; int ldy;
    int flags;
    float *workspace; size_t workspace_bytes;
    int split_k;
    int algo;
    int fuse_offset;
    const float *w_off_packed; const float *b_off;
    const float *up_w; int up_f; const float *up_skip; int up_lds; float *up_y; int up_ldy;
    float *om_partial; size_t om_partial_bytes;
    const float *w_off_winograd;
} ct_dcn_desc;
int ct_dcn_v2(const ct_dcn_desc *d, void *stream);
size_t ct_dcn_v2_workspace_bytes(const ct_dcn_desc *d);
size_t ct_dcn_v2_offsets_bytes(const ct_dcn_desc *d);
enum { CT_DCN_MAIN = 1,
       CT_DCN_FINISH = 2,
       CT_DCN_OFFSETS = 4     };
int ct_dcn_v2_group(const ct_dcn_desc *descs, int n, int phases, void *stream);
size_t ct_dcn_v2_group_workspace_bytes(const ct_dcn_desc *d);
int ct_dcn_v2_group_plan(const ct_dcn_desc *d, size_t *workspace_bytes, int *splits);

#define CT_DCN_BWD_INPUT 1
#define CT_DCN_BWD_OFFSET_MASK 2
#define CT_DCN_BWD_WEIGHT 4
typedef struct ct_dcn_bwd_desc {
    const float *x; int N, H, W, Cin, ldx;
    const float *om; int ldom;
    const float *gy; int Cout, ldgy;
    const float *wT_packed;
    float *gx; int ldgx;
    float *gom; int ldgom;
    float *gw; float *gb;
    float *workspace; size_t workspace_bytes;
    int flags;
} ct_dcn_bwd_desc;
int ct_dcn_v2_backward(const ct_dcn_bwd_desc *d, void *stream);
size_t ct_dcn_v2_backward_workspace_bytes(const ct_dcn_bwd_desc *d);
size_t ct_packed_dcn_weight_t_elems(int Cout, int Cin);
int ct_pack_dcn_weight_t(const float *w_oihw, float *packed, int Cout, int Cin, void *stream);

int ct_stem_forward(const float *x, const float *pre_img, const float *pre_hm, int N, int H, int W,
                    const float *w_x, const float *w_img, const float *w_hm,
                    const float *scale3, const float *shift3,
                    float *y, int ldy, void *stream);
int ct_stem_forward_parts(const float *x, const float *pre_img, const float *pre_hm, const float *add, int ldadd,
                          int N, int H, int W, const float *w_x, const float *w_img, const float *w_hm,
                          const float *scale3, const float *shift3, float *y, int ldy, void *stream);

int ct_maxpool2x2(const float *x, int N, int H, int W, int C, int ldx, float *y, int ldy, void *stream);
int ct_upsample_add(const float *x, int N, int H, int W, int C, int ldx, const float *w, int f,
                    const float *skip, int lds, float *y, int ldy, void *stream);
int ct_nchw_to_nhwc(const float *x, int N, int C, int H, int W, float *y, int ldy, void *stream);
int ct_nhwc_to_nchw(const float *x, int N, int C, int H, int W, int ldx, float *y, void *stream);

enum { CT_HEAD_REG = 0, CT_HEAD_WH, CT_HEAD_TRACKING, CT_HEAD_LTRB, CT_HEAD_LTRB_AMODAL,
       CT_HEAD_DEP, CT_HEAD_ROT, CT_HEAD_DIM, CT_HEAD_AMODEL_OFFSET, CT_HEAD_NUSCENES_ATT,
       CT_HEAD_VELOCITY, CT_NUM_HEADS };
typedef struct ct_sparse_heads_desc {
    const float *feat; int ldf;
    int nheads;
    int head[CT_NUM_HEADS];
    const float *w1[CT_NUM_HEADS], *b1[CT_NUM_HEADS], *w2[CT_NUM_HEADS], *b2[CT_NUM_HEADS];
    float depth_scale;
    int zero_tracking;
    int flip_B;
    int flip_mode[CT_NUM_HEADS];
} ct_sparse_heads_desc;
typedef struct ct_decode_desc {
    const float *hm; int B, C, h, w, K;
    const float *heads[CT_NUM_HEADS];
    float *out;
    int64_t *inds;
    void *workspace; size_t workspace_bytes;
    size_t hm_batch_stride; size_t head_batch_stride[CT_NUM_HEADS];
    int out_stride;
    float *host_out; int *done_flag; unsigned *done_counter;
    const ct_sparse_heads_desc *sparse;
} ct_decode_desc;
int ct_decode_row_floats(const ct_decode_desc *d);
size_t ct_decode_workspace_bytes(const ct_decode_desc *d);
int ct_decode(const ct_decode_desc *d, void *stream);

typedef struct ct_pose_desc {
    const float *rows; int row_floats, box_col;
    const int64_t *inds;
    int B, h, w, K, num_joints;
    const float *hps, *hm_hp, *hp_offset;
    size_t hps_batch_stride, hm_hp_batch_stride, hp_offset_batch_stride;
    float *out; int out_stride;
    void *workspace; size_t workspace_bytes;
    const float *box_wh, *box_reg, *box_ltrb;
    size_t box_wh_batch_stride, box_reg_batch_stride, box_ltrb_batch_stride;
} ct_pose_desc;
size_t ct_decode_pose_workspace_bytes(const ct_pose_desc *d);
int ct_decode_pose(const ct_pose_desc *d, void *stream);

int ct_render_pre_hm(const int *params, const int *counts, int cap, int B, int H, int W, float *out,
                     int also_flipped, void *stream);

enum { CT_FLIP_AVG = 0,
       CT_FLIP_NEG_EVEN = 1,
       CT_FLIP_JOINTS = 2,
       CT_FLIP_JOINT_OFFSETS = 3    };
typedef struct ct_flip_head {
    const float *src; float *dst;
    size_t src_batch_stride;
    int C, mode;
} ct_flip_head;
int ct_flip_merge(const ct_flip_head *heads, int nheads, const int *flip_idx, int npairs, int B, int h, int w,
                  void *stream);
int ct_flip_images(const float *src, float *dst, size_t rows, int W, void *stream);

typedef struct ct_row_layout {
    int score, cls, cts, tracking, bbox, amodel_offset;
} ct_row_layout;
typedef struct ct_track {
    float score; int cls;
    float ct[2], tracking[2], bbox[4];
    int tracking_id, age, active;
    int row;
} ct_track;
void *ct_tracker_create(float new_thresh, int max_age);
void ct_tracker_destroy(void *tracker);
void ct_tracker_reset(void *tracker);
int ct_tracker_num_tracks(void *tracker);
int ct_tracker_id_count(void *tracker);
int ct_tracker_get_tracks(void *tracker, ct_track *out, int cap);
int ct_tracker_step(void *tracker, const float *rows, int K, int F, const ct_row_layout *lay, float out_thresh,
                    const float *trans_inv, ct_track *out, int cap);
int ct_tracker_set_mode(void *tracker, int hungarian, int public_det);
int ct_tracker_init_tracks(void *tracker, const ct_track *items, int n);
int ct_tracker_step_public(void *tracker, const float *rows, int K, int F, const ct_row_layout *lay, float out_thresh,
                           const float *trans_inv, const float *public_cts, int n_public, ct_track *out, int cap);
int ct_tracker_step_dets(void *tracker, const ct_track *dets, int n, const float *public_cts, int n_public,
                         ct_track *out, int cap);
int ct_transform_points(const float *trans_inv, const float *xy, int n, float *out);
int ct_tracker_prehm_params(void *tracker, float pre_thresh, const double *trans_input, int inp_w, int inp_h,
                            int *params, int cap);

int ct_linear_assignment(const double *cost, int nr, int nc, int *rows, int *cols);

int ct_graph_begin(void *stream);
void *ct_graph_end(void *stream);
int ct_graph_launch(void *graph_exec, void *stream);
void ct_graph_destroy(void *graph_exec);
int ct_memcpy_async(void *dst, const void *src, size_t bytes, int kind , void *stream);
int ct_memset_async(void *dst, int value, size_t bytes, void *stream);
int ct_stream_synchronize(void *stream);
int ct_signal_host(int *flag, int value, void *stream);
enum { CT_FRAME_DEVICE = 0, CT_FRAME_HOST = 1, CT_FRAME_IN_PLACE = 2, CT_FRAME_UPLOADED = 3 };
typedef struct ct_prestage_desc {
    int enabled;
    int N, H, W;
    const float *w_x, *w_img, *scale3, *shift3;
    float *partial[3]; int ldp;
    int flip_B;
} ct_prestage_desc;
typedef struct ct_frame_loop_desc {
    int B, K, F;
    void *const *trackers;
    ct_row_layout layout;
    float out_thresh, pre_thresh;
    int inp_w, inp_h;
    const float *host_rows;
    float *rows_keep;
    int *blob_params, *blob_counts;
    int blob_cap;
    int nslots;
    void *graphs[3];
    float *frames[3];
    size_t frame_bytes;
    void *stream;
    ct_track *results; int results_cap;
    int *done_flag;
    ct_prestage_desc pre;
} ct_frame_loop_desc;
typedef struct ct_frame_step_args {
    int slot, frame_kind;
    const float *frame;
    const float *next_frame;
    const double *trans_input;
    const float *trans_inv;
} ct_frame_step_args;
void *ct_frame_loop_create(const ct_frame_loop_desc *d);
void ct_frame_loop_destroy(void *loop);
int ct_frame_loop_submit(void *loop, const ct_frame_step_args *a);
int ct_frame_loop_wait(void *loop);
int ct_frame_loop_finish(void *loop, const ct_frame_step_args *a, int *counts);
int ct_frame_loop_finish_submit(void *loop, const ct_frame_step_args *cur, int *counts, const ct_frame_step_args *next);
int ct_frame_loop_upload(void *loop, int slot, const float *frame);
int ct_frame_loop_prestage(void *loop, int slot);
int ct_frame_loop_pending_slot(void *loop);
int ct_frame_loop_in_flight(void *loop);
void ct_frame_loop_forget_upload(void *loop);

int ct_preprocess_image(const uint8_t *img, int h, int w, int stride, int channels, const double *trans,
                        int dst_w, int dst_h, const float *mean, const float *stdv, float *out, int flip_copy);

int ct_preprocess_lut(const float *mean, const float *stdv, int channels, float *lut_host);
int ct_preprocess_device(const uint8_t *img, int h, int w, int stride, int channels, const double *trans,
                         int dst_w, int dst_h, const float *lut, float *out, float *out_flip, void *stream);

#ifdef __cplusplus
}
#endif
#endif
```

Before: 1152 frames/s.

## Fuse decode NMS into top-k kernel and optionally render pre_hm inside stem

When the heatmap fits in LDS, the decode runs 3x3 max-pool NMS and candidate compaction inside the stage-2 top-k kernel. This removes the separate stage-1 launch and its candidate buffer. Separately, it adds an opt-in stem variant that renders the previous-frame heatmap blobs directly from the pinned parameter table, skipping the render kernel and a host-to-device copy. The fused decode puts the whole NMS on one 1024-thread block per image, which may reduce parallelism compared with the multi-block stage 1.

```diff
diff --git a/centertrack_amd/_lib.py b/centertrack_amd/_lib.py
--- a/centertrack_amd/_lib.py
+++ b/centertrack_amd/_lib.py
@@ -188,7 +188,7 @@
            'ct_memcpy_async', 'ct_memset_async', 'ct_stream_synchronize', 'ct_flip_merge', 'ct_flip_images',
            'ct_frame_loop_create', 'ct_frame_loop_destroy', 'ct_frame_loop_submit', 'ct_frame_loop_wait', 'ct_frame_loop_finish',
            'ct_frame_loop_finish_submit', 'ct_frame_loop_upload', 'ct_frame_loop_pending_slot', 'ct_frame_loop_in_flight',
-           'ct_frame_loop_forget_upload', 'ct_frame_loop_prestage', 'ct_stem_forward_parts', 'ct_signal_host']
+           'ct_frame_loop_forget_upload', 'ct_frame_loop_prestage', 'ct_stem_forward_parts', 'ct_signal_host', 'ct_stem_forward_blobs']
 
 _lib = None
 
@@ -240,6 +240,7 @@
     lib.ct_pack_dcn_weight_t.argtypes = [p, p, i, i, p]
     lib.ct_stem_forward.argtypes = [p, p, p, i, i, i, p, p, p, p, p, p, i, p]
     lib.ct_stem_forward_parts.argtypes = [p, p, p, p, i, i, i, i, p, p, p, p, p, p, i, p]
+    lib.ct_stem_forward_blobs.argtypes = [p, p, p, p, i, i, i, p, i, i, i, i, p, p, p, p, p, p, i, p]
     lib.ct_maxpool2x2.argtypes = [p, i, i, i, i, i, p, i, p]
     lib.ct_upsample_add.argtypes = [p, i, i, i, i, i, p, i, p, i, p, i, p]
     lib.ct_nchw_to_nhwc.argtypes = [p, i, i, i, i, p, i, p]
diff --git a/centertrack_amd/build.py b/centertrack_amd/build.py
--- a/centertrack_amd/build.py
+++ b/centertrack_amd/build.py
@@ -22,7 +22,7 @@
     hipcc = os.environ.get('HIPCC', '/opt/rocm/bin/hipcc')
     objdir = os.path.join(PKG, 'build')
     os.makedirs(objdir, exist_ok=True)
-    headers = [os.path.join(CSRC, 'ct_common.h'), os.path.join(CSRC, 'ksplit_core.h'),
+    headers = [os.path.join(CSRC, 'ct_common.h'), os.path.join(CSRC, 'ksplit_core.h'), os.path.join(CSRC, 'pre_hm.h'),
                os.path.join(ROOT, 'include', 'centertrack_hip.h')]
     objs = []
     procs = []
diff --git a/centertrack_amd/csrc/decode.hip b/centertrack_amd/csrc/decode.hip
--- a/centertrack_amd/csrc/decode.hip
+++ b/centertrack_amd/csrc/decode.hip
@@ -1,4 +1,5 @@
 #include "ct_common.h"
+#include <stdlib.h>
 
 namespace {
 CT_DEFINE_STAMPS(decode)
@@ -464,8 +465,90 @@
         }
 }
 
+constexpr int NMS_PIX = 16 * 1024;
+constexpr size_t NMS_LDS = (size_t)NMS_PIX * sizeof(float);
+static_assert(NMS_LDS == (size_t)SEL_U * 1024 * sizeof(unsigned long long), "the key list takes the map's place");
+
+__device__ __forceinline__ int nms_front_end(const float *hm_b, int C, int h, int w, unsigned char *smem, int *count,
+                                             unsigned long long (&keys)[SEL_U])
+{
+    float *map = reinterpret_cast<float *>(smem);
+    unsigned long long *list = reinterpret_cast<unsigned long long *>(smem);
+    const int tid = threadIdx.x, lane = tid & 63;
+    const int HW = h * w, NPIX = C * HW, nstrip = NPIX >> 3;
+    for (int i = tid * 4; i < NPIX; i += 4096)
+        *reinterpret_cast<f32x4 *>(map + i) = *reinterpret_cast<const f32x4 *>(hm_b + i);
+    __syncthreads();
+    const float NINF = -__builtin_inff();
+    float sv[16];
+#pragma unroll
+    for (int u = 0; u < 2; ++u) {
+        const int st = tid + u * 1024;
+        const bool live = st < nstrip;
+        const int f0 = live ? st * 8 : 0;
+        const int cls = f0 / HW, p0 = f0 - cls * HW;
+        const int y = p0 / w, x0 = p0 - y * w;
+        float m[8], c[8];
+#pragma unroll
+        for (int r = -1; r <= 1; ++r) {
+            const int yy = y + r;
+            const bool ok = live && yy >= 0 && yy < h;
+            const float *rp = map + (ok ? cls * HW + yy * w + x0 : 0);
+            const f32x4 a0 = *reinterpret_cast<const f32x4 *>(rp), a1 = *reinterpret_cast<const f32x4 *>(rp + 4);
+            const bool okl = ok && x0 > 0, okr = ok && x0 + 8 < w;
+            const float vl = rp[okl ? -1 : 0], vr = rp[okr ? 8 : 0];
+            float row[10];
+            row[0] = okl ? vl : NINF;
+            row[9] = okr ? vr : NINF;
+#pragma unroll
+            for (int j = 0; j < 4; ++j) { row[1 + j] = ok ? a0[j] : NINF; row[5 + j] = ok ? a1[j] : NINF; }
+#pragma unroll
+            for (int j = 0; j < 8; ++j) {
+                const float hm3 = fmaxf(fmaxf(row[j], row[j + 1]), row[j + 2]);
+                m[j] = (r == -1) ? hm3 : fmaxf(m[j], hm3);
+                if (r == 0) c[j] = row[j + 1];
+            }
+        }
+#pragma unroll
+        for (int j = 0; j < 8; ++j) {
+            const float s = (m[j] == c[j]) ? c[j] : c[j] * 0.0f;
+            sv[u * 8 + j] = live ? s : 0.0f;
+        }
+    }
+    int cnt = 0;
+#pragma unroll
+    for (int q = 0; q < 16; ++q) cnt += (sv[q] > 0.0f) ? 1 : 0;
+    int pre = cnt;
+#pragma unroll
+    for (int o = 1; o < 64; o <<= 1) {
+        const int t = __shfl_up(pre, o);
+        if (lane >= o) pre += t;
+    }
+    int base = 0;
+    if (lane == 63 && pre) base = atomicAdd(count, pre);
+    base = __shfl(base, 63) + pre - cnt;
+    __syncthreads();
+    const int n = *count;
+    if (n > SEL_U * 1024) return n;
+#pragma unroll
+    for (int q = 0; q < 16; ++q)
+        if (sv[q] > 0.0f) {
+            const unsigned flat = (unsigned)((tid + (q >> 3) * 1024) * 8 + (q & 7));
+            list[base++] = ((unsigned long long)f2ord(sv[q]) << 32) | (unsigned long long)(0xFFFFFFFFu - flat);
+        }
+    __syncthreads();
+#pragma unroll
+    for (int u = 0; u < SEL_U; ++u) {
+        const int i = tid + u * 1024;
+        keys[u] = (i < n) ? list[i] : 0ull;
+    }
+    return n;
+}
+
+template <bool FUSED>
 __global__ __launch_bounds__(1024) void decode_stage2_kernel(Stage2Args a)
 {
+    extern __shared__ __attribute__((aligned(16))) unsigned char nms_smem[];
     __shared__ unsigned hist[256];
     __shared__ unsigned long long bcast[2];
     __shared__ unsigned long long win[MAXK];
@@ -490,9 +573,9 @@
         return (k & 0xFFFFFFFF00000000ull) | (unsigned long long)(0xFFFFFFFFu - (cls * (unsigned)HW + p));
     };
     auto get = [&](int i) -> unsigned long long { return key2(i, cand[i]); };
-    const bool in_regs = M2 <= SEL_U * 1024 && NT == 1024;
+    const bool in_regs = FUSED || (M2 <= SEL_U * 1024 && NT == 1024);
     unsigned long long keys[SEL_U];
-    if (in_regs) {
+    if (!FUSED && in_regs) {
 #pragma unroll
         for (int u = 0; u < SEL_U; ++u) {
             const int i = tid + u * NT;
@@ -507,10 +590,17 @@
     bool need_sort = true;
     bool selected = false;
     if (in_regs) {
+        int rc = -2;
+        if constexpr (FUSED) {
+            const int n = nms_front_end(a.hm + (size_t)b * a.hm_bs, a.C, a.h, a.w, nms_smem, &nf, keys);
+            CT_STAMP(2);
+            if (n <= SEL_U * 1024) rc = select_topk_regs(keys, a.K, sel, filt, false);
+        } else {
 #pragma unroll
         for (int u = 0; u < SEL_U; ++u) keys[u] = key2(tid + u * NT, keys[u]);
         CT_STAMP(2);
-        const int rc = select_topk_regs(keys, a.K, sel, filt, false);
+        rc = select_topk_regs(keys, a.K, sel, filt, false);
+        }
         CT_STAMP(3);
         if (rc == a.K) {
             for (int i0 = 0; i0 < a.K; i0 += NT / 8) {
@@ -525,12 +615,13 @@
             }
             need_sort = false;
             selected = true;
-        } else if (rc == -1) {
-            if (tid == 0) total = sel.total;
+        } else if (FUSED || rc == -1) {
+            if (tid == 0) total = FUSED ? 0 : sel.total;
             selected = true;
         }
         __syncthreads();
     }
+    if constexpr (!FUSED) {
     if (!selected) {
     scan_cands(cand, M2, tid, NT, [&](int i, unsigned long long raw) {
         const unsigned long long k = key2(i, raw);
@@ -548,6 +639,7 @@
         }
     });
     __syncthreads();
+    }
     }
     if (selected && need_sort == false) {
     } else if (!selected && total >= a.K && total <= FCAP) {
@@ -902,6 +994,15 @@
     return (int)G;
 }
 
+static bool one_launch(const ct_decode_desc *d, int G)
+{
+    if (d->sparse || G > 0) return false;
+    if ((long)d->C * d->h * d->w > NMS_PIX || (d->w & 7)) return false;
+    if (((uintptr_t)d->hm & 15) || (d->hm_batch_stride & 3)) return false;
+    const char *e = getenv("CENTERTRACK_FUSED_EDGES");
+    return !(e && e[0] == '0' && e[1] == 0);
+}
+
 static size_t sparse_bytes(const ct_decode_desc *d)
 {
     if (!d->sparse) return 0;
@@ -950,8 +1051,11 @@
         attr_set = true;
     }
     if (lds1 > 96 * 1024) CT_FAIL_ARG("ct_decode: stage-1 LDS %zu too large", lds1);
-    hipLaunchKernelGGL(decode_stage1_kernel, dim3((unsigned)(d->B * d->C * nseg)), dim3(256), lds1, s, a1);
-    CT_CHECK_LAUNCH("ct_decode(stage 1)");
+    const bool one = one_launch(d, G);
+    if (!one) {
+        hipLaunchKernelGGL(decode_stage1_kernel, dim3((unsigned)(d->B * d->C * nseg)), dim3(256), lds1, s, a1);
+        CT_CHECK_LAUNCH("ct_decode(stage 1)");
+    }
     Stage2Args a2;
     a2.cand = a1.cand; a2.hm = d->hm;
     for (int i = 0; i < CT_NUM_HEADS; ++i) {
@@ -975,7 +1079,18 @@
         CT_CHECK_LAUNCH("ct_decode(stage 2a)");
         a2.cand = aa.cand2; a2.M2 = G * d->K; a2.keys_final = 1;
     }
-    hipLaunchKernelGGL(decode_stage2_kernel, dim3((unsigned)d->B), dim3(1024), 0, s, a2);
+    if (one) {
+        static bool attr2_set = false;
+        if (!attr2_set) {
+            (void)hipFuncSetAttribute(reinterpret_cast<const void *>(decode_stage2_kernel<true>),
+                                      hipFuncAttributeMaxDynamicSharedMemorySize, (int)NMS_LDS);
+            attr2_set = true;
+        }
+        hipLaunchKernelGGL(decode_stage2_kernel<true>, dim3((unsigned)d->B), dim3(1024), NMS_LDS, s, a2);
+        CT_CHECK_LAUNCH("ct_decode(one launch)");
+        return CT_OK;
+    }
+    hipLaunchKernelGGL(decode_stage2_kernel<false>, dim3((unsigned)d->B), dim3(1024), 0, s, a2);
     CT_CHECK_LAUNCH("ct_decode(stage 2)");
     if (sp) {
         SparseArgs sa;
diff --git a/centertrack_amd/csrc/elementwise.hip b/centertrack_amd/csrc/elementwise.hip
--- a/centertrack_amd/csrc/elementwise.hip
+++ b/centertrack_amd/csrc/elementwise.hip
@@ -1,4 +1,5 @@
 #include "ct_common.h"
+#include "pre_hm.h"
 
 namespace {
 
@@ -98,7 +99,7 @@
     }
 }
 
-constexpr int PHM_TW = 32, PHM_TH = 8, PHM_CAP = 256;
+constexpr int PHM_TW = 32, PHM_TH = 8;
 __global__ __launch_bounds__(256) void render_pre_hm_kernel(const int *params, const int *counts, int cap, int B,
                                                             int H, int W, float *out, int also_flipped)
 {
@@ -112,7 +113,6 @@
     const int x0 = tx * PHM_TW, y0 = ty * PHM_TH;
     const int n = min(counts[b], cap);
     const int *p = params + (size_t)b * cap * 3;
-    const int lane = threadIdx.x & 63;
     const int x = x0 + (threadIdx.x & (PHM_TW - 1)), y = y0 + (threadIdx.x / PHM_TW);
     float v = 0.0f;
     for (int c0 = 0; c0 == 0 || c0 < n; c0 += PHM_CAP) {
@@ -123,29 +123,11 @@
             const int i = i0 + threadIdx.x;
             int cx = 0, cy = 0, r = -1;
             if (i < c1) { cx = p[3 * i]; cy = p[3 * i + 1]; r = p[3 * i + 2]; }
-            const bool hit = i < c1 && r >= 0 && cx + r >= x0 && cx - r < x0 + PHM_TW && cy + r >= y0 && cy - r < y0 + PHM_TH;
-            const unsigned long long mask = __ballot(hit);
-            int base = 0;
-            if (mask) {
-                const int leader = __ffsll((long long)mask) - 1;
-                if (lane == leader) base = atomicAdd(&nblob, (int)__popcll(mask));
-                base = __shfl(base, leader);
-            }
-            if (hit) {
-                const int s = base + (int)__popcll(mask & ((1ull << lane) - 1ull));
-                blob[3 * s] = cx; blob[3 * s + 1] = cy; blob[3 * s + 2] = r;
-            }
+            phm_push(i < c1 && phm_hit(cx, cy, r, x0, x0 + PHM_TW, y0, y0 + PHM_TH), cx, cy, r, blob, &nblob);
         }
         __syncthreads();
         const int m = nblob;
-        for (int i = 0; i < m; ++i) {
-            const int cx = blob[3 * i], cy = blob[3 * i + 1], r = blob[3 * i + 2];
-            const int dx = x - cx, dy = y - cy;
-            if (dx < -r || dx > r || dy < -r || dy > r) continue;
-            const double sigma = (double)(2 * r + 1) / 6.0;
-            const double g = exp(-(double)(dx * dx + dy * dy) / (2.0 * sigma * sigma));
-            v = fmaxf(v, (float)g);
-        }
+        for (int i = 0; i < m; ++i) v = phm_splat(v, x, y, blob[3 * i], blob[3 * i + 1], blob[3 * i + 2]);
         __syncthreads();
     }
     if (x >= W || y >= H) return;
diff --git a/centertrack_amd/csrc/pre_hm.h b/centertrack_amd/csrc/pre_hm.h
--- /dev/null
+++ b/centertrack_amd/csrc/pre_hm.h
@@ -0,0 +1,34 @@
+#pragma once
+#include "ct_common.h"
+
+constexpr int PHM_CAP = 256;
+
+__device__ __forceinline__ bool phm_hit(int cx, int cy, int r, int x0, int x1, int y0, int y1)
+{
+    return r >= 0 && cx + r >= x0 && cx - r < x1 && cy + r >= y0 && cy - r < y1;
+}
+
+__device__ __forceinline__ float phm_splat(float v, int x, int y, int cx, int cy, int r)
+{
+    const int dx = x - cx, dy = y - cy;
+    if (dx < -r || dx > r || dy < -r || dy > r) return v;
+    const double sigma = (double)(2 * r + 1) / 6.0;
+    const double g = exp(-(double)(dx * dx + dy * dy) / (2.0 * sigma * sigma));
+    return fmaxf(v, (float)g);
+}
+
+__device__ __forceinline__ void phm_push(bool hit, int cx, int cy, int r, int *blob, int *nblob)
+{
+    const int lane = threadIdx.x & 63;
+    const unsigned long long mask = __ballot(hit);
+    int base = 0;
+    if (mask) {
+        const int leader = __ffsll((long long)mask) - 1;
+        if (lane == leader) base = atomicAdd(nblob, (int)__popcll(mask));
+        base = __shfl(base, leader);
+    }
+    if (hit) {
+        const int s = base + (int)__popcll(mask & ((1ull << lane) - 1ull));
+        blob[3 * s] = cx; blob[3 * s + 1] = cy; blob[3 * s + 2] = r;
+    }
+}
diff --git a/centertrack_amd/csrc/stem.hip b/centertrack_amd/csrc/stem.hip
--- a/centertrack_amd/csrc/stem.hip
+++ b/centertrack_amd/csrc/stem.hip
@@ -1,4 +1,5 @@
 #include "ct_common.h"
+#include "pre_hm.h"
 
 namespace {
 
@@ -25,11 +26,14 @@
     const float *add;
     float *y;
     int N, H, W, ldy, ldadd, tilesX, tilesY;
+    const int *blob_params;
+    const int *blob_counts;
+    int blob_cap, blob_B;
 };
 
 constexpr int ST_NWV = 10;
 
-template <int TH>
+template <int TH, bool BLOBS>
 __attribute__((amdgpu_waves_per_eu(TH == 16 ? 2 : 1)))
 __global__ __launch_bounds__(256) void stem_kernel(StemArgs a)
 {
@@ -38,6 +42,8 @@
     __shared__ __attribute__((aligned(16))) float planes[7 * ST_PS];
     __shared__ __attribute__((aligned(16))) float wl[ST_KTOT * ST_WLP];
     __shared__ int tab[ST_KTOT];
+    __shared__ int blob[BLOBS ? PHM_CAP * 3 : 1];
+    __shared__ int nblob;
     CT_STAMP_RT(0);
     CT_STAMP(1);
     CT_STAMP_HW(8);
@@ -52,11 +58,20 @@
     const int oy0 = ty * ST_TH, ox0 = tx * ST_TW;
     const size_t HW = (size_t)a.H * a.W;
 
+    [[maybe_unused]] int bl_cx = 0, bl_cy = 0, bl_r = -1, bl_n = 0;
+    [[maybe_unused]] const int *bl_p = nullptr;
+    if constexpr (BLOBS) {
+        const int b = n < a.blob_B ? n : n - a.blob_B;
+        bl_p = a.blob_params + (size_t)b * a.blob_cap * 3;
+        bl_n = min(a.blob_counts[b], a.blob_cap);
+        if (tid < bl_n) { bl_cx = bl_p[3 * tid]; bl_cy = bl_p[3 * tid + 1]; bl_r = bl_p[3 * tid + 2]; }
+    }
+
     for (int k = tid; k < ST_KTOT; k += 256) {
         const int s = (k >= 296) ? 2 : ((k >= 148) ? 1 : 0);
         const int kk = k - st_koff(s);
         const int cin = (s == 2) ? 1 : 3;
-        int off = 0;
+        int off = a.in[0] ? 0 : 3 * s * ST_PS;
         if (kk < cin * 49) {
             const int c = kk / 49, r = kk - c * 49;
             off = (3 * s + c) * ST_PS + (r / 7) * ST_PW + (r % 7);
@@ -71,6 +86,7 @@
         const float *src = a.in[s] + (size_t)n * cin * HW;
         const float *w = a.w[s];
         const int np = cin * ST_PH * 38, nw = st_k4(s) * 16;
+        if (!(BLOBS && s == 2)) {
 #pragma unroll
         for (int i = 0; i < ST_NPV; ++i) {
             const int it = tid + 256 * i;
@@ -82,6 +98,7 @@
             const float v = src[ok ? ((size_t)c * HW + (size_t)iy * a.W + ix) : 0];
             pv[i] = ok ? v : 0.0f;
         }
+        }
 #pragma unroll
         for (int i = 0; i < ST_NWV; ++i) {
             const int it = tid + 256 * i;
@@ -93,7 +110,7 @@
     };
     auto stage_store = [&](int s) {
         const int cin = (s == 2) ? 1 : 3;
-        const int np = cin * ST_PH * 38, nw = st_k4(s) * 16;
+        const int np = (BLOBS && s == 2) ? 0 : cin * ST_PH * 38, nw = st_k4(s) * 16;
 #pragma unroll
         for (int i = 0; i < ST_NPV; ++i) {
             const int it = tid + 256 * i;
@@ -131,8 +148,54 @@
         }
     }
 
+    auto render_patch = [&]() {
+        if (a.in[2]) {
+            constexpr int NPX = (ST_PH * 38 + 255) / 256;
+            const bool mir = n >= a.blob_B;
+            const int xa = mir ? a.W - 1 - (ox0 + 34) : ox0 - 3;
+            const int ya = oy0 - 3;
+            float v[NPX];
+            int rx[NPX], ry[NPX];
+#pragma unroll
+            for (int i = 0; i < NPX; ++i) {
+                const int it = tid + 256 * i;
+                const int py = it / 38, px = it - py * 38;
+                const int ix = ox0 - 3 + px;
+                ry[i] = oy0 - 3 + py;
+                rx[i] = mir ? a.W - 1 - ix : ix;
+                v[i] = 0.0f;
+            }
+            for (int c0 = 0; c0 == 0 || c0 < bl_n; c0 += PHM_CAP) {
+                const int c1 = min(bl_n, c0 + PHM_CAP);
+                if (tid == 0) nblob = 0;
+                __syncthreads();
+                {
+                    const int i = c0 + tid;
+                    int cx = bl_cx, cy = bl_cy, r = bl_r;
+                    if (c0 > 0 && i < c1) { cx = bl_p[3 * i]; cy = bl_p[3 * i + 1]; r = bl_p[3 * i + 2]; }
+                    phm_push(i < c1 && phm_hit(cx, cy, r, xa, xa + 38, ya, ya + ST_PH), cx, cy, r, blob, &nblob);
+                }
+                __syncthreads();
+                const int m = nblob;
+                for (int j = 0; j < m; ++j) {
+                    const int cx = blob[3 * j], cy = blob[3 * j + 1], r = blob[3 * j + 2];
+#pragma unroll
+                    for (int i = 0; i < NPX; ++i) v[i] = phm_splat(v[i], rx[i], ry[i], cx, cy, r);
+                }
+                __syncthreads();
+            }
+#pragma unroll
+            for (int i = 0; i < NPX; ++i) {
+                const int it = tid + 256 * i;
+                const int py = it / 38, px = it - py * 38;
+                const bool in = ry[i] >= 0 && ry[i] < a.H && rx[i] >= 0 && rx[i] < a.W;
+                if (it < ST_PH * 38) planes[6 * ST_PS + py * ST_PW + px] = in ? v[i] : 0.0f;
+            }
+        }
+    };
     const int first = a.in[0] ? 0 : (a.in[1] ? 1 : 2);
     stage_load(first);
+    if constexpr (BLOBS) render_patch();
     CT_STAMP(2);
     stage_store(first);
     __syncthreads();
@@ -199,9 +262,34 @@
     return ct_stem_forward_parts(x, pre_img, pre_hm, nullptr, 0, N, H, W, w_x, w_img, w_hm, scale3, shift3, y, ldy, stream);
 }
 
+static int stem_launch(const float *x, const float *pre_img, const float *pre_hm, const float *add, int ldadd,
+                       int N, int H, int W, const float *w_x, const float *w_img, const float *w_hm,
+                       const float *scale3, const float *shift3, float *y, int ldy, void *stream,
+                       const int *blob_params, const int *blob_counts, int blob_cap, int blob_B);
+
 extern "C" int ct_stem_forward_parts(const float *x, const float *pre_img, const float *pre_hm, const float *add, int ldadd,
                                      int N, int H, int W, const float *w_x, const float *w_img, const float *w_hm,
                                      const float *scale3, const float *shift3, float *y, int ldy, void *stream)
+{
+    return stem_launch(x, pre_img, pre_hm, add, ldadd, N, H, W, w_x, w_img, w_hm, scale3, shift3, y, ldy, stream,
+                       nullptr, nullptr, 0, 0);
+}
+
+extern "C" int ct_stem_forward_blobs(const float *x, const float *pre_img, const int *params, const int *counts, int cap,
+                                     int B, int also_flipped, const float *add, int ldadd, int N, int H, int W,
+                                     const float *w_x, const float *w_img, const float *w_hm, const float *scale3,
+                                     const float *shift3, float *y, int ldy, void *stream)
+{
+    if (!params || !counts || cap <= 0 || B <= 0) CT_FAIL_ARG("ct_stem_forward_blobs: bad blob table");
+    if (N != (also_flipped ? 2 * B : B)) CT_FAIL_ARG("ct_stem_forward_blobs: N=%d images for B=%d streams (also_flipped=%d)", N, B, also_flipped);
+    return stem_launch(x, pre_img, reinterpret_cast<const float *>(params), add, ldadd, N, H, W, w_x, w_img, w_hm, scale3,
+                       shift3, y, ldy, stream, params, counts, cap, B);
+}
+
+static int stem_launch(const float *x, const float *pre_img, const float *pre_hm, const float *add, int ldadd,
+                       int N, int H, int W, const float *w_x, const float *w_img, const float *w_hm,
+                       const float *scale3, const float *shift3, float *y, int ldy, void *stream,
+                       const int *blob_params, const int *blob_counts, int blob_cap, int blob_B)
 {
     if (!scale3 || !shift3 || !y) CT_FAIL_ARG("ct_stem_forward: null pointer");
     if (!x && !pre_img && !pre_hm) CT_FAIL_ARG("ct_stem_forward_parts: no stem selected");
@@ -212,6 +300,7 @@
     a.w[0] = w_x; a.w[1] = w_img; a.w[2] = w_hm;
     a.scale = scale3; a.shift = shift3; a.y = y; a.add = add; a.ldadd = ldadd;
     a.N = N; a.H = H; a.W = W; a.ldy = ldy;
+    a.blob_params = blob_params; a.blob_counts = blob_counts; a.blob_cap = blob_cap; a.blob_B = blob_B;
     a.tilesX = ct_cdiv(W, ST_TW);
     const long blocks8 = (long)N * a.tilesX * ct_cdiv(H, 8);
     const int want = ct_tune_get(CT_TUNE_STEM_ROWS);
@@ -219,8 +308,11 @@
     a.tilesY = ct_cdiv(H, rows16 ? 16 : 8);
     const long blocks = (long)N * a.tilesX * a.tilesY;
     if (blocks > 0x7fffffffL) CT_FAIL_ARG("ct_stem_forward: grid too large");
-    if (rows16) hipLaunchKernelGGL(stem_kernel<16>, dim3((unsigned)blocks), dim3(256), 0, (hipStream_t)stream, a);
-    else hipLaunchKernelGGL(stem_kernel<8>, dim3((unsigned)blocks), dim3(256), 0, (hipStream_t)stream, a);
+    if (blob_params) {
+        if (rows16) hipLaunchKernelGGL((stem_kernel<16, true>), dim3((unsigned)blocks), dim3(256), 0, (hipStream_t)stream, a);
+        else hipLaunchKernelGGL((stem_kernel<8, true>), dim3((unsigned)blocks), dim3(256), 0, (hipStream_t)stream, a);
+    } else if (rows16) hipLaunchKernelGGL((stem_kernel<16, false>), dim3((unsigned)blocks), dim3(256), 0, (hipStream_t)stream, a);
+    else hipLaunchKernelGGL((stem_kernel<8, false>), dim3((unsigned)blocks), dim3(256), 0, (hipStream_t)stream, a);
     CT_CHECK_LAUNCH("ct_stem_forward");
     return CT_OK;
 }
diff --git a/centertrack_amd/detector.py b/centertrack_amd/detector.py
--- a/centertrack_amd/detector.py
+++ b/centertrack_amd/detector.py
@@ -10,6 +10,10 @@
 NATIVE_LOOP = os.environ.get('CENTERTRACK_NATIVE_LOOP', '1') != '0'
 SPLIT_STEM_MAX = int(os.environ.get('CENTERTRACK_SPLIT_STEM_MAX', '0'))
 HOST_FLAG = os.environ.get('CENTERTRACK_HOST_FLAG', '1') != '0'
+
+
+def fused_stem():
+    return os.environ.get('CENTERTRACK_FUSED_STEM', '0') == '1' and os.environ.get('CENTERTRACK_FUSED_EDGES', '1') != '0'
 HOST_ROWS = os.environ.get('CENTERTRACK_HOST_ROWS', '1') != '0'
 from .image import (affine_transform, draw_umich_gaussian, gaussian_radius, get_affine_transform, make_meta)
 from .model import create_model, load_model
@@ -239,22 +243,29 @@
                                                       _lib.stream_ptr()), 'ct_flip_images')
             self.model.run_stem_partial(cur, prev, ctx['partial'][slot])
         ctx['pre_stage'] = pre_stage
+        fused = pinned_blobs = ctx['pinned_blobs'] = render and fused_stem()
+        blobs = None
+        if fused:
+            src = ctx['pc_host']
+            blobs = (src.data_ptr(), src.data_ptr() + 4 * self.B * ctx['max_blobs'] * 3, ctx['max_blobs'], self.B,
+                     1 if self.flip else 0)
 
         def device_frame(slot=0, with_copies=False):
             cur = ctx['frames'][slot]
             prev = ctx['frames'][(slot - 1) % nslots] if img_in is not None else None
-            if with_copies and render:
+            if with_copies and render and not pinned_blobs:
                 _lib.check(_lib.load().ct_memcpy_async(ctx['pc_dev'].data_ptr(), ctx['pc_host'].data_ptr(),
                                                        ctx['pc_host'].numel() * 4, 1, _lib.stream_ptr()), 'H2D')
             lib = _lib.load()
-            if render:
+            if render and not fused:
                 _lib.check(lib.ct_render_pre_hm(ctx['prm_dev'].data_ptr(), ctx['cnt_dev'].data_ptr(),
                                                 ctx['max_blobs'], self.B, H, W, hm_in.data_ptr(),
                                                 1 if self.flip else 0, _lib.stream_ptr()), 'ct_render_pre_hm')
             if self.flip and not split:
                 _lib.check(lib.ct_flip_images(cur.data_ptr(), cur[self.B:].data_ptr(), self.B * 3 * H, W,
                                               _lib.stream_ptr()), 'ct_flip_images')
-            self.model._run_plan(plan, inputs=(cur, prev, hm_in), stem_partial=ctx['partial'][slot] if split else None)
+            self.model._run_plan(plan, inputs=(cur, prev, hm_in), stem_partial=ctx['partial'][slot] if split else None,
+                                 blobs=blobs)
             if self.flip:
                 arr, n, pairs, h, w = ctx['flip_call']
                 _lib.check(lib.ct_flip_merge(arr, n, pairs.ctypes.data, len(pairs), self.B, h, w, _lib.stream_ptr()),
@@ -580,7 +591,7 @@
                     m = metas[s]
                     ch[s], _ = self.fast[s].prehm_params(opt.pre_thresh, m['trans_input'], m['inp_width'],
                                                          m['inp_height'], out=ph[s])
-                if not ctx['raw']:
+                if not ctx['raw'] and not ctx['pinned_blobs']:
                     ctx['pc_dev'].copy_(ctx['pc_host'], non_blocking=True)
             elif hm_in is not None:
                 hh = ctx['host_hm']
diff --git a/centertrack_amd/model.py b/centertrack_amd/model.py
--- a/centertrack_amd/model.py
+++ b/centertrack_amd/model.py
@@ -437,7 +437,7 @@
         if rc != 0:
             _lib.check(rc, 'stem (x / pre_img terms)')
 
-    def _run_plan(self, plan, inputs=None, stem_partial=None, launches=None):
+    def _run_plan(self, plan, inputs=None, stem_partial=None, launches=None, blobs=None):
         P = self._prepared
         lib = _lib.load()
         st = _lib.stream_ptr()
@@ -457,6 +457,21 @@
                 if inputs is not None:
                     x, img, hm = inputs
                 w = P['stem_w']
+                if blobs is not None:
+                    if hm is None:
+                        raise _lib.CTError('a blob table was given to a model without the pre_hm input')
+                    prm, cnt, cap, nb, fl = blobs
+                    part = stem_partial
+                    rc = lib.ct_stem_forward_blobs(None if part is not None else x.data_ptr(),
+                                                   None if part is not None else ops._p(img), prm, cnt, cap, nb, fl,
+                                                   part.ptr if part is not None else None, part.ld if part is not None else 0,
+                                                   x.shape[0], x.shape[2], x.shape[3],
+                                                   None if part is not None else w[0].data_ptr(),
+                                                   ops._p(w[1]) if (part is None and img is not None) else None, w[2].data_ptr(),
+                                                   P['stem_scale'].data_ptr(), P['stem_shift'].data_ptr(), y.ptr, y.ld, st)
+                    if rc != 0:
+                        _lib.check(rc, l.name)
+                    continue
                 if stem_partial is not None:
                     if hm is None:
                         raise _lib.CTError('a split stem needs the pre_hm input')
diff --git a/include/centertrack_hip.h b/include/centertrack_hip.h
--- a/include/centertrack_hip.h
+++ b/include/centertrack_hip.h
@@ -111,6 +111,10 @@
 int ct_stem_forward_parts(const float *x, const float *pre_img, const float *pre_hm, const float *add, int ldadd,
                           int N, int H, int W, const float *w_x, const float *w_img, const float *w_hm,
                           const float *scale3, const float *shift3, float *y, int ldy, void *stream);
+int ct_stem_forward_blobs(const float *x, const float *pre_img, const int *params, const int *counts, int cap, int B,
+                          int also_flipped, const float *add, int ldadd, int N, int H, int W, const float *w_x,
+                          const float *w_img, const float *w_hm, const float *scale3, const float *shift3, float *y,
+                          int ldy, void *stream);
 
 int ct_maxpool2x2(const float *x, int N, int H, int W, int C, int ldx, float *y, int ldy, void *stream);
 int ct_upsample_add(const float *x, int N, int H, int W, int C, int ldx, const float *w, int f,
```

Result: no change. 1148 frames/s (-0.3%).
